# peterrum/dealii-multigrid

Measured on AMD Instinct MI355X. Metric: DoF/s per V-cycle, 3D octant p=4, higher is better.
Workload: dtype f64; 1 GPU; 3D octant (GeometryType quadrant) HMG-global p=4 FP64, NRefGlobal=8, SmootherDegree=3, coarse solver direct, f=1, zero Dirichlet (BASELINE.json configs[2]); n_dofs=137199985, n_cells=2127189, n_levels=9, parallelism=1 GPU, chebyshev_start_vector=deal.II's (i mod 11) - mean on the local numbering, fused_transfer_bricks=33509

## Files before the change

### dealii_multigrid_amd/__init__.py

```python
from __future__ import annotations

import ctypes as C
import os

import numpy as np

_LIB_PATH = os.environ.get("MGAMD_LIBRARY") or os.path.join(os.path.dirname(os.path.abspath(__file__)), "lib", "libmgamd.so")
F64, F32 = 8, 4
AMG_MIN_SHARDED_ROWS_DEFAULT = 20000
INVALID_DOF = 0xFFFFFFFF
ALL_DIRICHLET = 0x3F


class MgamdError(RuntimeError):
    pass


class NoDeviceError(MgamdError):
    pass


def _load():
    if not os.path.exists(_LIB_PATH):
        raise MgamdError(
# ... 350 lines not shown
    def cell_slots(self):
        grp, slot = np.zeros(self.info.n_cells, np.uint8), np.zeros(self.info.n_cells, np.uint32)
        _chk(_lib.mgamd_dofs_get_cell_slots(self._h, _ptr(grp), _ptr(slot)))
        return grp, slot

    def halo_plan(self):
        sz = (C.c_uint32 * 4)()
        _chk(_lib.mgamd_dofs_halo_sizes(self._h, sz))
        npeer, nsend, nsh, nc = (int(v) for v in sz)
        plan = dict(peers=np.zeros(npeer, np.int32), peer_offset=np.zeros(npeer + 1, np.uint32), pack_idx=np.zeros(nsend, np.uint32),
                    sh_tail=np.zeros(nsh, np.uint32), sh_ptr=np.zeros(nsh + 1, np.uint32), sh_src=np.zeros(nc, np.int32),
                    sh_owner_src=np.zeros(nsh, np.int32))
        if npeer:
            _chk(_lib.mgamd_dofs_halo_get(self._h, _ptr(plan["peers"]), _ptr(plan["peer_offset"]), _ptr(plan["pack_idx"]), _ptr(plan["sh_tail"]),
                                          _ptr(plan["sh_ptr"]), _ptr(plan["sh_src"]), _ptr(plan["sh_owner_src"])))
        return plan

    def __del__(self):
        if getattr(self, "_h", None) and _lib is not None:
            _lib.mgamd_dofs_destroy(self._h)
            self._h = None


def ls_copy_indices(active: DoFs, level_dofs: DoFs, level: int):
    n = C.c_uint64()
    _chk(_lib.mgamd_ls_copy_indices(active._h, level_dofs._h, level, C.byref(n), None, None))
    g, l = np.zeros(n.value, np.uint32), np.zeros(n.value, np.uint32)
    if n.value:
        _chk(_lib.mgamd_ls_copy_indices(active._h, level_dofs._h, level, C.byref(n), _ptr(g), _ptr(l)))
    return g, l


def transfer_tables(fine: DoFs, coarse: DoFs):
    npatch = (C.c_uint64 * 3)()
    nf = (C.c_uint32 * 3)()
    _chk(_lib.mgamd_transfer_tables_info(fine._h, coarse._h, npatch, nf))
    out = []
    nc3 = (coarse.degree + 1) ** 3
    for kind in range(3):
        n = npatch[kind]
        ci = np.zeros((n, nc3), np.uint32)
        cm = np.zeros(n, np.uint16)
        fi = np.zeros((n, nf[kind] ** 3), np.uint32)
        if n:
            _chk(_lib.mgamd_transfer_tables_get(fine._h, coarse._h, kind, _ptr(ci), _ptr(cm), _ptr(fi)))
        out.append((kind, int(nf[kind]), ci, cm, fi))
    return out


class Context:
    def __init__(self, device: int = 0):
        self._h = C.c_void_p()
        _chk(_lib.mgamd_ctx_create(device, C.byref(self._h)))

    def synchronize(self):
        _chk(_lib.mgamd_ctx_synchronize(self._h))

    def stream(self) -> int:
        s = C.c_void_p()
        _chk(_lib.mgamd_ctx_stream(self._h, C.byref(s)))
        return s.value

    def kernel_profile(self, enable: bool, brick_size: int = 0):
        _chk(_lib.mgamd_ctx_kernel_profile_brick(self._h, brick_size))
        _chk(_lib.mgamd_ctx_kernel_profile(self._h, 1 if enable else 0))

    def kernel_profile_read(self):
        ms, n, b = C.c_double(), C.c_uint64(), C.c_double()
        _chk(_lib.mgamd_ctx_kernel_profile_read(self._h, C.byref(ms), C.byref(n), C.byref(b)))
        return ms.value, n.value, b.value

    def kernel_profile_bytes_moved(self):
        b = C.c_double()
        _chk(_lib.mgamd_ctx_kernel_profile_bytes_moved(self._h, C.byref(b)))
        return b.value

    def __del__(self):
        if getattr(self, "_h", None) and _lib is not None:
            _lib.mgamd_ctx_destroy(self._h)
            self._h = None


class SimGroup:

    def __init__(self, n_ranks: int):
        self.n_ranks = n_ranks
        self._h = C.c_void_p()
        _chk(_lib.mgamd_sim_group_create(n_ranks, C.byref(self._h)))

    def comm(self, rank: int) -> "Communicator":
        h = C.c_void_p()
        _chk(_lib.mgamd_comm_sim_create(self._h, rank, C.byref(h)))
        return Communicator(h, self.n_ranks, rank, self)

    def __del__(self):
        if getattr(self, "_h", None) and _lib is not None:
            _lib.mgamd_sim_group_destroy(self._h)
            self._h = None


class Communicator:
    def __init__(self, handle, n_ranks, rank, keepalive=None):
        self._h, self.n_ranks, self.rank, self._keep = handle, n_ranks, rank, keepalive

    @staticmethod
    def rccl_unique_id() -> bytes:
        buf = C.create_string_buffer(128)
        _chk(_lib.mgamd_comm_rccl_unique_id(buf))
        return buf.raw

    @staticmethod
    def rccl(ctx: "Context", n_ranks: int, rank: int, unique_id: bytes) -> "Communicator":
        h = C.c_void_p()
        _chk(_lib.mgamd_comm_rccl_create(ctx._h, n_ranks, rank, C.c_char_p(unique_id), C.byref(h)))
        return Communicator(h, n_ranks, rank)

    def subset(self, group: int) -> "Communicator":
        if group == 1:
            return self
        h = C.c_void_p()
        _chk(_lib.mgamd_comm_subset(self._h, group, C.byref(h)))
        return Communicator(h, self.n_ranks // group, self.rank // group, self)

    def allreduce_sum(self, ctx: "Context", value: float) -> float:
        r = C.c_double()
        _chk(_lib.mgamd_comm_allreduce_sum(self._h, ctx._h, C.c_double(value), C.byref(r)))
        return r.value

    def __del__(self):
        if getattr(self, "_h", None) and _lib is not None:
            _lib.mgamd_comm_destroy(self._h)
            self._h = None


class Vector:

    def __init__(self, ctx: Context, n: int, number_type: int = F64, _handle=None):
        self.ctx = ctx
        self._h = C.c_void_p()
        if _handle is not None:
            self._h = _handle
        else:
            _chk(_lib.mgamd_vec_create(ctx._h, C.c_uint64(n), number_type, C.byref(self._h)))
        sz = C.c_uint64()
        _chk(_lib.mgamd_vec_size(self._h, C.byref(sz)))
        self.n = sz.value

    def from_host(self, a):
        a = np.ascontiguousarray(a, dtype=np.float64)
        assert a.size == self.n
        _chk(_lib.mgamd_vec_from_host(self._h, _ptr(a)))
        return self

    def to_host(self):
        a = np.zeros(self.n)
        _chk(_lib.mgamd_vec_to_host(self._h, _ptr(a)))
        return a

    def set(self, value: float):
        _chk(_lib.mgamd_vec_set(self._h, C.c_double(value)))

    def copy_from(self, other: "Vector"):
        _chk(_lib.mgamd_vec_copy(self._h, other._h))

    def sadd(self, s: float, a: float, x: "Vector"):
        _chk(_lib.mgamd_vec_sadd(self._h, C.c_double(s), C.c_double(a), x._h))

    def dot(self, other: "Vector") -> float:
        r = C.c_double()
        _chk(_lib.mgamd_vec_dot(self._h, other._h, C.byref(r)))
        return r.value

    def l2_norm(self) -> float:
        r = C.c_double()
        _chk(_lib.mgamd_vec_norm2(self._h, C.byref(r)))
        return r.value

    def __del__(self):
        if getattr(self, "_h", None) and _lib is not None:
            _lib.mgamd_vec_destroy(self._h)
            self._h = None


class Operator:

    def __init__(self, ctx: Context, dofs: DoFs, number_type: int = F64, comm: "Communicator" = None):
        self.ctx, self.dofs, self.number_type, self.comm = ctx, dofs, number_type, comm
        self._h = C.c_void_p()
        if comm is None:
            _chk(_lib.mgamd_level_op_create(ctx._h, dofs._h, number_type, C.byref(self._h)))
        else:
            _chk(_lib.mgamd_level_op_create_distributed(ctx._h, dofs._h, number_type, comm._h, C.byref(self._h)))

    def dot(self, x: "Vector", y: "Vector") -> float:
        r = C.c_double()
        _chk(_lib.mgamd_level_op_dot(self._h, x._h, y._h, C.byref(r)))
        return r.value

    def n_owned(self) -> int:
        n = C.c_uint64()
        _chk(_lib.mgamd_level_op_n_owned(self._h, C.byref(n)))
        return n.value

    def m(self) -> int:
        n = C.c_uint64()
        _chk(_lib.mgamd_level_op_m(self._h, C.byref(n)))
        return n.value

    def mass_coefficient(self) -> float:
        s = C.c_double()
        _chk(_lib.mgamd_level_op_mass_coefficient(self._h, C.byref(s)))
        return s.value

    def initialize_dof_vector(self) -> Vector:
        h = C.c_void_p()
        _chk(_lib.mgamd_level_op_init_vector(self._h, C.byref(h)))
        return Vector(self.ctx, 0, _handle=h)

    def vmult(self, dst: Vector, src: Vector):
        _chk(_lib.mgamd_level_op_vmult(self._h, dst._h, src._h))

    def vmult_mass(self, dst: Vector, src: Vector):
        _chk(_lib.mgamd_level_op_vmult_mass(self._h, dst._h, src._h))

    def vmult_interface_up(self, dst: Vector, src: Vector):
        _chk(_lib.mgamd_level_op_vmult_interface_up(self._h, dst._h, src._h))

    def exchange_add_tail(self, v: Vector):
        _chk(_lib.mgamd_level_op_exchange_add_tail(self._h, v._h))

    def vmult_interface_down(self, dst: Vector, src: Vector):
        _chk(_lib.mgamd_level_op_vmult_interface_down(self._h, dst._h, src._h))

    def compute_inverse_diagonal(self, diagonal: Vector):
        _chk(_lib.mgamd_level_op_inverse_diagonal(self._h, diagonal._h))

    def rhs(self, b: Vector, kind: int = 0):
        _chk(_lib.mgamd_level_op_rhs_kind(self._h, kind, b._h))

    def rhs_boundary_flux(self, b: Vector, q):
        q = _flux_array(q)
        _chk(_lib.mgamd_level_op_rhs_boundary_flux(self._h, _ptr(q), b._h))

    def distribute(self, x: Vector, kind: int = 0):
        _chk(_lib.mgamd_level_op_distribute(self._h, kind, x._h))

    def rhs_dirichlet(self, b: Vector, g: Vector, include_mass: bool = True):
        _chk(_lib.mgamd_level_op_rhs_dirichlet(self._h, g._h, 1 if include_mass else 0, b._h))

    def distribute_values(self, x: Vector, g: Vector):
        _chk(_lib.mgamd_level_op_distribute_values(self._h, x._h, g._h))

    def get_system_matrix(self) -> "SparseMatrix":
        if self.dofs.mass_coefficient() != self.mass_coefficient():
            raise MgamdError(f"get_system_matrix: the mass coefficient of the DoFs ({self.dofs.mass_coefficient()}) was changed after this "
                             f"operator was built with {self.mass_coefficient()}; the assembled matrix would be another operator's")
        return SparseMatrix(self.ctx, self.dofs)

    def __del__(self):
        if getattr(self, "_h", None) and _lib is not None:
            _lib.mgamd_level_op_destroy(self._h)
            self._h = None


class PreconditionChebyshev:
    def __init__(self, op: Operator, degree=3, smoothing_range=20.0, eig_cg_n_iterations=20):
        self.op = op
        self._h = C.c_void_p()
        _chk(_lib.mgamd_cheb_create(op._h, degree, C.c_double(smoothing_range), eig_cg_n_iterations, C.byref(self._h)))

    def vmult(self, dst: Vector, src: Vector):
        _chk(_lib.mgamd_cheb_vmult(self._h, dst._h, src._h))

    def step(self, dst: Vector, src: Vector):
        _chk(_lib.mgamd_cheb_step(self._h, dst._h, src._h))

    def eigenvalue_estimates(self):
        lo, hi = C.c_double(), C.c_double()
        _chk(_lib.mgamd_cheb_get_eigen_estimates(self._h, C.byref(lo), C.byref(hi)))
        return lo.value, hi.value

    def __del__(self):
        if getattr(self, "_h", None) and _lib is not None:
            _lib.mgamd_cheb_destroy(self._h)
            self._h = None


class MGTwoLevelTransfer:
    def __init__(self, fine: Operator, coarse: Operator):
        self.fine, self.coarse = fine, coarse
        self._h = C.c_void_p()
        _chk(_lib.mgamd_transfer2_create(fine._h, coarse._h, C.byref(self._h)))

    def prolongate_and_add(self, dst_fine: Vector, src_coarse: Vector):
        _chk(_lib.mgamd_transfer2_prolongate_and_add(self._h, dst_fine._h, src_coarse._h))

    def restrict_and_add(self, dst_coarse: Vector, src_fine: Vector):
        _chk(_lib.mgamd_transfer2_restrict_and_add(self._h, dst_coarse._h, src_fine._h))

    def n_fused_bricks(self):
        n = C.c_uint64()
        _chk(_lib.mgamd_transfer2_n_fused_bricks(self._h, C.byref(n)))
        return n.value

    def __del__(self):
        if getattr(self, "_h", None) and _lib is not None:
            _lib.mgamd_transfer2_destroy(self._h)
            self._h = None


STAGE_NAMES = ["pre_smoother_step", "residual_step", "restriction", "coarse_solve", "prolongation", "edge_prolongation",
               "post_smoother_step", "transfer_to_mg", "transfer_to_global"]
_STAGE_CB = C.CFUNCTYPE(None, C.c_int, C.c_int, C.c_uint, C.c_void_p)


class PreconditionMG:

    def __init__(self, ctx: Context, levels, transfers, smoothers, coarse_solver="direct", nested: "PreconditionMG" = None,
                 n_cycles: int = 1, local_smoothing: "DoFs" = None, sharded_amg: "DoFs" = None,
                 amg_min_sharded_rows: int = AMG_MIN_SHARDED_ROWS_DEFAULT):
        self.ctx, self.levels, self.transfers, self.smoothers, self.nested = ctx, levels, transfers, smoothers, nested
        self.sharded_amg = sharded_amg
        n = len(levels)
        L = (C.c_void_p * n)(*[l._h for l in levels])
        T = (C.c_void_p * n)(*[(t._h if t is not None else None) for t in transfers])
        S = (C.c_void_p * n)(*[(s._h if s is not None else None) for s in smoothers])
        self._h = C.c_void_p()
        if sharded_amg is not None:
            if local_smoothing is not None or nested is not None:
                raise MgamdError("sharded_amg excludes local smoothing and a nested multigrid")
            _chk(_lib.mgamd_mg_create_sharded_amg(ctx._h, n, L, T, S, coarse_solver.encode(), sharded_amg._h, n_cycles,
                                                  C.c_uint32(amg_min_sharded_rows), C.byref(self._h)))
        elif local_smoothing is not None:
            _chk(_lib.mgamd_mg_create_local_smoothing(ctx._h, n, L, T, S, local_smoothing._h, coarse_solver.encode(), C.byref(self._h)))
        else:
            _chk(_lib.mgamd_mg_create_nested(ctx._h, n, L, T, S, coarse_solver.encode(), nested._h if nested is not None else None, n_cycles,
                                             C.byref(self._h)))
        self._cb = None

    def set_collapse(self, enable: bool) -> int:
        l = C.c_uint()
        _chk(_lib.mgamd_mg_set_collapse(self._h, 1 if enable else 0, C.byref(l)))
        return l.value

    def coarse_solver_used(self) -> str:
        buf = C.create_string_buffer(32)
        _chk(_lib.mgamd_mg_coarse_solver_used(self._h, buf))
        return buf.value.decode()

    def coarse_iterations(self) -> int:
        n = C.c_uint64()
        _chk(_lib.mgamd_mg_coarse_iterations(self._h, C.byref(n)))
        return n.value

    def amg_layout(self):
        n, info = C.c_uint32(), (C.c_uint32 * (5 * 32))()
        _chk(_lib.mgamd_mg_amg_layout(self._h, C.byref(n), info, 32))
        return [dict(global_rows=info[5 * l], owned_rows=info[5 * l + 1], ghosts=info[5 * l + 2], peers=info[5 * l + 3],
                     replicated=bool(info[5 * l + 4])) for l in range(min(n.value, 32))]

    def vmult(self, z: Vector, r: Vector):
        _chk(_lib.mgamd_mg_vcycle(self._h, z._h, r._h))

    def connect_stages(self, fn):
        if fn is None:
            self._cb = None
            _chk(_lib.mgamd_mg_set_stage_callback(self._h, None, None))
            return
        self._cb = _STAGE_CB(lambda s, st, lv, u: fn(s, bool(st), lv))
        _chk(_lib.mgamd_mg_set_stage_callback(self._h, self._cb, None))

    def stage_timing(self, enable: bool):
        _chk(_lib.mgamd_mg_stage_timing(self._h, 1 if enable else 0))

    def stage_times(self):
        n = len(self.levels)
        ms = np.zeros((9, n))
        cnt = C.c_uint64()
        _chk(_lib.mgamd_mg_stage_times(self._h, _ptr(ms), n, C.byref(cnt)))
        return ms

    def time_vcycles(self, z: Vector, r: Vector, n: int, use_graph: bool = True) -> float:
        ms = C.c_double()
        _chk(_lib.mgamd_mg_time_vcycles(self._h, z._h, r._h, n, 1 if use_graph else 0, C.byref(ms)))
        return ms.value

    def __del__(self):
        if getattr(self, "_h", None) and _lib is not None:
            _lib.mgamd_mg_destroy(self._h)
            self._h = None


class SparseMatrix:

    def __init__(self, ctx: Context, dofs: DoFs):
        self.ctx, self.dofs = ctx, dofs
        self._h = C.c_void_p()
        _chk(_lib.mgamd_matrix_create(ctx._h, dofs._h, C.byref(self._h)))
        n, nnz, lanes = C.c_uint64(), C.c_uint64(), C.c_int()
        _chk(_lib.mgamd_matrix_info(self._h, C.byref(n), C.byref(nnz), C.byref(lanes)))
        self.n_rows, self.nnz, self.lanes = n.value, nnz.value, lanes.value

    def m(self) -> int:
        return self.n_rows

    def vmult(self, dst: Vector, src: Vector):
        _chk(_lib.mgamd_matrix_vmult(self._h, dst._h, src._h))

    def time_spmv(self, mode: int, lanes: int, reps: int = 50) -> float:
        ms = C.c_double()
        _chk(_lib.mgamd_debug_matrix_time_spmv(self._h, mode, lanes, reps, C.byref(ms)))
        return ms.value

    def __del__(self):
        if getattr(self, "_h", None) and _lib is not None:
            _lib.mgamd_matrix_destroy(self._h)
            self._h = None


class PreconditionAMG:

    def __init__(self, matrix: SparseMatrix, n_cycles: int = 1):
        self.matrix, self.n_cycles = matrix, n_cycles
        self._h = C.c_void_p()
        _chk(_lib.mgamd_amg_create(matrix._h, n_cycles, C.byref(self._h)))

    def vmult(self, z: Vector, r: Vector):
        _chk(_lib.mgamd_amg_vmult(self._h, z._h, r._h))

    def layout(self):
        n, rows = C.c_uint32(), (C.c_uint32 * 32)()
        _chk(_lib.mgamd_amg_layout(self._h, C.byref(n), rows, 32))
        return [rows[l] for l in range(min(n.value, 32))]

    def __del__(self):
        if getattr(self, "_h", None) and _lib is not None:
            _lib.mgamd_amg_destroy(self._h)
            self._h = None


def solve_cg(A, preconditioner, x: Vector, b: Vector, reltol=1e-4, abstol=1e-20, maxiter=10000):
    it, res = C.c_uint(), C.c_double()
    ph = preconditioner._h if preconditioner is not None else None
    if isinstance(A, SparseMatrix):
        if preconditioner is not None and not isinstance(preconditioner, PreconditionAMG):
            raise MgamdError("solve_cg: a SparseMatrix takes a PreconditionAMG (or None)")
        _chk(_lib.mgamd_solve_cg_matrix(A._h, ph, x._h, b._h, C.c_double(reltol), C.c_double(abstol), maxiter, C.byref(it), C.byref(res)))
        return it.value, res.value
    if isinstance(preconditioner, PreconditionAMG):
        raise MgamdError("solve_cg: a PreconditionAMG goes with the SparseMatrix it was built on")
    _chk(_lib.mgamd_solve_cg(A._h, ph, x._h, b._h, C.c_double(reltol), C.c_double(abstol), maxiter, C.byref(it), C.byref(res)))
    return it.value, res.value


class TimeStepper:

    def __init__(self, op: Operator, mg: "PreconditionMG", theta: float, dt: float):
        self.op, self.mg = op, mg
        self._h = C.c_void_p()
        _chk(_lib.mgamd_time_stepper_create(op._h, mg._h if mg is not None else None, C.c_double(theta), C.c_double(dt), C.byref(self._h)))

    @staticmethod
    def mass_coefficient(theta: float, dt: float) -> float:
        return 1.0 / (theta * dt)

    def step(self, u: Vector, f_old: Vector = None, f_new: Vector = None, reltol=1e-4, abstol=1e-20, maxiter=10000, g_old: Vector = None,
             g_new: Vector = None, load: Vector = None):
        it, res = C.c_uint(), C.c_double()
        h = lambda v: v._h if v is not None else None
        if g_old is None and g_new is None and load is None:
            _chk(_lib.mgamd_time_stepper_step(self._h, u._h, h(f_old), h(f_new), C.c_double(reltol), C.c_double(abstol), maxiter,
                                              C.byref(it), C.byref(res)))
        else:
            _chk(_lib.mgamd_time_stepper_step_data(self._h, u._h, h(f_old), h(f_new), h(g_old), h(g_new), h(load), C.c_double(reltol),
                                                   C.c_double(abstol), maxiter, C.byref(it), C.byref(res)))
        return it.value, res.value

    def time(self) -> float:
        t = C.c_double()
        _chk(_lib.mgamd_time_stepper_time(self._h, C.byref(t), None))
        return t.value

    def n_steps(self) -> int:
        n = C.c_uint64()
        _chk(_lib.mgamd_time_stepper_time(self._h, None, C.byref(n)))
        return n.value

    def __del__(self):
        if getattr(self, "_h", None) and _lib is not None:
            _lib.mgamd_time_stepper_destroy(self._h)
            self._h = None


class AmgHostHierarchy:

    def __init__(self, dofs: DoFs):
        self._h = C.c_void_p()
        _chk(_lib.mgamd_debug_amg_host_create(dofs._h, C.byref(self._h)))
        n = C.c_uint32()
        _chk(_lib.mgamd_debug_amg_host_n_levels(self._h, C.byref(n)))
        self.n_levels = n.value

    def level(self, l: int):
        rows, nnz_a, cols_p, nnz_p, na, lam = C.c_uint32(), C.c_uint64(), C.c_uint32(), C.c_uint64(), C.c_uint32(), C.c_double()
        _chk(_lib.mgamd_debug_amg_host_level_info(self._h, C.c_uint32(l), C.byref(rows), C.byref(nnz_a), C.byref(cols_p), C.byref(nnz_p),
                                                 C.byref(na), C.byref(lam)))
        n, coarsest = rows.value, l + 1 == self.n_levels
        A = (np.zeros(n + 1, np.uint32), np.zeros(nnz_a.value, np.uint32), np.zeros(nnz_a.value))
        P = (np.zeros(n + 1, np.uint32), np.zeros(nnz_p.value, np.uint32), np.zeros(nnz_p.value))
        agg = np.zeros(n, np.int32)
        _chk(_lib.mgamd_debug_amg_host_level_get(self._h, C.c_uint32(l), *[_ptr(a) for a in A], *([None] * 3 if coarsest else [_ptr(a) for a in P]),
                                                None if coarsest else _ptr(agg)))
        return dict(A=A, P=None if coarsest else P, n_cols_P=cols_p.value, agg=None if coarsest else agg, n_aggregates=na.value,
                    lambda_max=lam.value)

    def __del__(self):
        if getattr(self, "_h", None) and _lib is not None:
            _lib.mgamd_debug_amg_host_destroy(self._h)
            self._h = None


class AmgShardPlans:

    def __init__(self, partition: "Partition", level: int, degree: int, max_brick: int = -1,
                 min_sharded_rows: int = AMG_MIN_SHARDED_ROWS_DEFAULT):
        self._h = C.c_void_p()
        _chk(_lib.mgamd_debug_amg_shard_create(partition._h, level, degree, max_brick, C.c_uint32(min_sharded_rows), C.byref(self._h)))
        n, ns = C.c_uint32(), C.c_uint32()
        _chk(_lib.mgamd_debug_amg_shard_n_levels(self._h, C.byref(n), C.byref(ns)))
        self.n_levels, self.n_sharded_levels, self.n_ranks = n.value, ns.value, partition.n_ranks

    def level(self, rank: int, l: int):
        info = (C.c_uint32 * 12)()
        _chk(_lib.mgamd_debug_amg_shard_level_info(self._h, rank, C.c_uint32(l), info))
        rep, ng, nr, nm, ni, ngh, nrecv, npeer, nza, nzp, nzr, rrows = (int(v) for v in info)
        out = dict(replicated=bool(rep), n_global=ng, n_rows=nr, n_mirror=nm, n_interior=ni, n_ghost=ngh, n_recv=nrecv, A=None, P=None, R=None)
        if rep:
            return out
        u32 = lambda n: np.zeros(n, np.uint32)
        out.update(rows=u32(nr), ghost=u32(nrecv), peers=np.zeros(npeer, np.int32), peer_offset=u32(npeer + 1), send_count=u32(npeer),
                   recv_count=u32(npeer), send_idx=u32(nrecv), A=(u32(nr + 1), u32(nza), np.zeros(nza)), P=(u32(nr + 1), u32(nzp), np.zeros(nzp)),
                   R=(u32(rrows + 1), u32(nzr), np.zeros(nzr)))
        _chk(_lib.mgamd_debug_amg_shard_level_get(self._h, rank, C.c_uint32(l), *[_ptr(out[k]) for k in ("rows", "ghost", "peers", "peer_offset",
                                                                                                      "send_count", "recv_count", "send_idx")],
                                                 *[_ptr(a) for a in out["A"]], *[_ptr(a) for a in out["P"]], *[_ptr(a) for a in out["R"]]))
        return out

    def __del__(self):
        if getattr(self, "_h", None) and _lib is not None:
            _lib.mgamd_debug_amg_shard_destroy(self._h)
            self._h = None


SPMV_PLAIN, SPMV_ADD, SPMV_RESID, SPMV_CHEB, SPMV_DOT = 0, 1, 2, 3, 4


def debug_csr_spmv(ctx: "Context", number_type, mode, lanes, ptr, col, val, x, y, b=None, xold=None, xold_is_y=False, dinv=None, f1=0.0,
                   f2=0.0):
    ptr, col = np.ascontiguousarray(ptr, np.uint32), np.ascontiguousarray(col, np.uint32)
    val, x, y = (np.ascontiguousarray(a, np.float64) for a in (val, x, y))
    y = y.copy()
    opt = [None if a is None else np.ascontiguousarray(a, np.float64) for a in (b, xold, dinv)]
    n_rows = len(ptr) - 1
    assert len(y) == n_rows and len(col) == len(val) == ptr[-1]
    used = C.c_int()
    _chk(_lib.mgamd_debug_csr_spmv(ctx._h, number_type, mode, lanes, C.c_uint32(n_rows), C.c_uint32(len(x)), _ptr(ptr), _ptr(col), _ptr(val),
                                   _ptr(x), _ptr(y), *[None if a is None else _ptr(a) for a in opt[:2]], 1 if xold_is_y else 0,
                                   None if opt[2] is None else _ptr(opt[2]), C.c_double(f1), C.c_double(f2), C.byref(used)))
    return y, used.value


def debug_csr_spmv_ex(ctx: "Context", mode, lanes, ptr, col, val, x, y, b=None, xold=None, xold_is_y=False, dinv=None, f1=0.0, f2=0.0,
                      max_blocks=0, number_type=F64):
    ptr, col = np.ascontiguousarray(ptr, np.uint32), np.ascontiguousarray(col, np.uint32)
    val, x, y = (np.ascontiguousarray(a, np.float64) for a in (val, x, y))
    y = y.copy()
    opt = [None if a is None else np.ascontiguousarray(a, np.float64) for a in (b, xold, dinv)]
    n_rows = len(ptr) - 1
    assert len(y) == n_rows and len(col) == len(val) == ptr[-1]
    used, blocks, dot = C.c_int(), C.c_int(), C.c_double()
    _chk(_lib.mgamd_debug_csr_spmv_ex(ctx._h, number_type, mode, lanes, C.c_uint32(n_rows), C.c_uint32(len(x)), _ptr(ptr), _ptr(col),
                                      _ptr(val), _ptr(x), _ptr(y), *[None if a is None else _ptr(a) for a in opt[:2]],
                                      1 if xold_is_y else 0, None if opt[2] is None else _ptr(opt[2]), C.c_double(f1), C.c_double(f2),
                                      max_blocks, C.byref(used), C.byref(blocks), C.byref(dot)))
    return y, used.value, blocks.value, dot.value


def csr_spmv_lanes_long(n_rows: int, nnz: int) -> int:
    lanes = C.c_int()
    _chk(_lib.mgamd_debug_csr_spmv_lanes_long(C.c_uint32(n_rows), C.c_uint64(nnz), C.byref(lanes)))
    return lanes.value


def amg_shard_match_rows(global_dofs: "DoFs", local_dofs: "DoFs"):
    rows = np.zeros(local_dofs.n_dofs, np.uint32)
    _chk(_lib.mgamd_debug_amg_shard_match_rows(global_dofs._h, local_dofs._h, _ptr(rows)))
    return rows


def csr_row_pointers(row_counts):
    counts = np.ascontiguousarray(row_counts, np.uint64)
    ptr = np.zeros(len(counts) + 1, np.uint32)
    _chk(_lib.mgamd_debug_csr_row_pointers(C.c_uint32(len(counts)), _ptr(counts), _ptr(ptr)))
    return ptr


# ... 187 lines not shown
```

### dealii_multigrid_amd/csrc/c_api_device.hip

```cpp
#include "runtime.hpp"
#include "kernels_amg.hpp"
#include <cstdio>

using namespace mgamd;

#define REQUIRE(cond)                                    \
  if (!(cond))                                           \
  throw std::invalid_argument("null or invalid argument: " #cond)

extern "C" {

int
mgamd_ctx_create(int device, mgamd_ctx **out)
{
  MGAMD_TRY
  REQUIRE(out);
  auto *c = new mgamd_ctx;
  try
    {
      c->ctx = std::make_unique<Ctx>(device);
    }
  catch (...)
    {
      delete c;
// ... 238 lines not shown
}

int
mgamd_sim_group_create(unsigned n_ranks, mgamd_sim_group **out)
{
  MGAMD_TRY
  REQUIRE(out && n_ranks > 0);
  auto *g  = new mgamd_sim_group;
  g->group = std::make_shared<SimGroup>((int)n_ranks);
  *out     = g;
  MGAMD_CATCH
}

int
mgamd_sim_group_destroy(mgamd_sim_group *g)
{
  delete g;
  return MGAMD_OK;
}

int
mgamd_comm_sim_create(mgamd_sim_group *g, unsigned rank, mgamd_comm **out)
{
  MGAMD_TRY
  REQUIRE(g && out && (int)rank < g->group->n);
  auto *c = new mgamd_comm;
  c->comm = std::make_shared<SimComm>(g->group, (int)rank);
  *out    = c;
  MGAMD_CATCH
}

int
mgamd_comm_subset(mgamd_comm *base, unsigned group, mgamd_comm **out)
{
  MGAMD_TRY
  if (!base || !base->comm || !out || group == 0)
    throw std::invalid_argument("bad argument");
  auto *c = new mgamd_comm;
  try
    {
      c->comm = std::make_shared<SubsetComm>(base->comm, (int)group);
    }
  catch (...)
    {
      delete c;
      throw;
    }
  *out = c;
  MGAMD_CATCH
}

int
mgamd_comm_destroy(mgamd_comm *c)
{
  delete c;
  return MGAMD_OK;
}

int
mgamd_comm_allreduce_sum(mgamd_comm *c, mgamd_ctx *ctx, double value, double *result)
{
  MGAMD_TRY
  REQUIRE(c && ctx && result);
  *result = c->comm->allreduce_sum_host(value, ctx->ctx->stream);
  MGAMD_CATCH
}

int
mgamd_level_op_destroy(mgamd_level_op *op)
{
  delete op;
  return MGAMD_OK;
}

int
mgamd_level_op_m(const mgamd_level_op *op, uint64_t *n)
{
  MGAMD_TRY
  REQUIRE(op && n);
  *n = op->op->n_dofs();
  MGAMD_CATCH
}

int
mgamd_level_op_mass_coefficient(const mgamd_level_op *op, double *sigma)
{
  MGAMD_TRY
  REQUIRE(op && sigma);
  *sigma = op->op->sigma;
  MGAMD_CATCH
}

int
mgamd_level_op_init_vector(const mgamd_level_op *op, mgamd_vec **out)
{
  MGAMD_TRY
  REQUIRE(op && out);
  *out = vec_create(op->op->ctx, op->op->n_dofs(), op->op->type);
  MGAMD_CATCH
}

int
mgamd_level_op_vmult(mgamd_level_op *op, mgamd_vec *dst, const mgamd_vec *src)
{
  MGAMD_TRY
  REQUIRE(op && dst && src);
  op->op->vmult(*dst, *src);
  MGAMD_CATCH
}

int
mgamd_level_op_vmult_mass(mgamd_level_op *op, mgamd_vec *dst, const mgamd_vec *src)
{
  MGAMD_TRY
  REQUIRE(op && dst && src);
  op->op->vmult_mass(*dst, *src);
  MGAMD_CATCH
}

int
mgamd_level_op_inverse_diagonal(mgamd_level_op *op, mgamd_vec *diagonal)
{
  MGAMD_TRY
  REQUIRE(op && diagonal);
  if (diagonal->type != op->op->type)
    throw std::invalid_argument("vector number type does not match the operator's");
  op->op->compute_inverse_diagonal(*diagonal);
  MGAMD_CATCH
}

int
mgamd_level_op_rhs(mgamd_level_op *op, mgamd_vec *rhs)
{
  MGAMD_TRY
  REQUIRE(op && rhs);
  op->op->rhs(*rhs);
  MGAMD_CATCH
}

int
mgamd_level_op_rhs_kind(mgamd_level_op *op, int kind, mgamd_vec *rhs)
{
  MGAMD_TRY
  REQUIRE(op && rhs);
  if (kind != 0 && kind != 1)
    throw std::invalid_argument("SimulationType kind must be 0 (Constant) or 1 (Gaussian)");
  op->op->rhs(*rhs, kind);
  MGAMD_CATCH
}

int
mgamd_level_op_rhs_boundary_flux(mgamd_level_op *op, const double q[6], mgamd_vec *rhs)
{
  MGAMD_TRY
  REQUIRE(op && q && rhs);
  op->op->rhs_boundary_flux(*rhs, q);
  MGAMD_CATCH
}

int
mgamd_level_op_distribute(mgamd_level_op *op, int kind, mgamd_vec *x)
{
  MGAMD_TRY
  REQUIRE(op && x);
  if (kind != 0 && kind != 1)
    throw std::invalid_argument("SimulationType kind must be 0 (Constant) or 1 (Gaussian)");
  op->op->distribute(*x, kind);
  MGAMD_CATCH
}

int
mgamd_level_op_rhs_dirichlet(mgamd_level_op *op, const mgamd_vec *g, int include_mass, mgamd_vec *rhs)
{
  MGAMD_TRY
  REQUIRE(op && g && rhs);
  op->op->rhs_dirichlet(*rhs, *g, include_mass != 0);
  MGAMD_CATCH
}

int
mgamd_level_op_distribute_values(mgamd_level_op *op, mgamd_vec *x, const mgamd_vec *g)
{
  MGAMD_TRY
  REQUIRE(op && x && g);
  op->op->distribute_values(*x, *g);
  MGAMD_CATCH
}

int
mgamd_level_op_debug_stamps(mgamd_level_op *op, unsigned long long *out, uint64_t max_count, uint64_t *count)
{
  MGAMD_TRY
  REQUIRE(op && out && count);
  *count = op->op->read_debug_stamps(out, max_count);
  MGAMD_CATCH
}

int
mgamd_cheb_create(mgamd_level_op *op, unsigned degree, double smoothing_range, unsigned eig_cg_n_iterations, mgamd_cheb **out)
{
  MGAMD_TRY
  REQUIRE(op && out);
  auto *h = new mgamd_cheb;
  try
    {
      h->c.reset(make_chebyshev(op->op.get(), degree, smoothing_range, eig_cg_n_iterations));
    }
  catch (...)
    {
      delete h;
      throw;
    }
  *out = h;
  MGAMD_CATCH
}

int
mgamd_cheb_destroy(mgamd_cheb *c)
{
  delete c;
  return MGAMD_OK;
}

int
mgamd_cheb_vmult(mgamd_cheb *c, mgamd_vec *dst, const mgamd_vec *src)
{
  MGAMD_TRY
  REQUIRE(c && dst && src);
  c->c->vmult(*dst, *src);
  MGAMD_CATCH
}

int
mgamd_cheb_step(mgamd_cheb *c, mgamd_vec *dst, const mgamd_vec *src)
{
  MGAMD_TRY
  REQUIRE(c && dst && src);
  c->c->step(*dst, *src);
  MGAMD_CATCH
}

int
mgamd_cheb_get_eigen_estimates(const mgamd_cheb *c, double *min_eigenvalue, double *max_eigenvalue)
{
  MGAMD_TRY
  REQUIRE(c);
  if (min_eigenvalue)
    *min_eigenvalue = c->c->min_eig;
  if (max_eigenvalue)
    *max_eigenvalue = c->c->max_eig;
  MGAMD_CATCH
}

int
mgamd_transfer2_create(mgamd_level_op *fine, mgamd_level_op *coarse, mgamd_transfer2 **out)
{
  MGAMD_TRY
  REQUIRE(fine && coarse && out);
  auto *h = new mgamd_transfer2;
  try
    {
      h->t.reset(make_transfer2(fine->op.get(), coarse->op.get()));
    }
  catch (...)
    {
      delete h;
      throw;
    }
  *out = h;
  MGAMD_CATCH
}

int
mgamd_transfer2_destroy(mgamd_transfer2 *t)
{
  delete t;
  return MGAMD_OK;
}

int
mgamd_transfer2_prolongate_and_add(mgamd_transfer2 *t, mgamd_vec *dst_fine, const mgamd_vec *src_coarse)
{
  MGAMD_TRY
  REQUIRE(t && dst_fine && src_coarse);
  t->t->prolongate_and_add(*dst_fine, *src_coarse);
  MGAMD_CATCH
}

int
mgamd_transfer2_restrict_and_add(mgamd_transfer2 *t, mgamd_vec *dst_coarse, const mgamd_vec *src_fine)
{
  MGAMD_TRY
  REQUIRE(t && dst_coarse && src_fine);
  t->t->restrict_and_add(*dst_coarse, *src_fine);
  MGAMD_CATCH
}

int
mgamd_transfer2_n_fused_bricks(const mgamd_transfer2 *t, uint64_t *n)
{
  MGAMD_TRY
  REQUIRE(t && n);
  *n = t->t->n_fused_bricks_total();
  MGAMD_CATCH
}

int
mgamd_mg_create(mgamd_ctx *ctx, unsigned n_levels, mgamd_level_op *const *levels, mgamd_transfer2 *const *transfers,
                mgamd_cheb *const *smoothers, const char *coarse_solver, mgamd_mg **out)
{
  MGAMD_TRY
  REQUIRE(ctx && levels && out && n_levels > 0 && (n_levels == 1 || (transfers && smoothers)));
  std::vector<LevelOperatorBase *> L(n_levels, nullptr);
  std::vector<Transfer2Base *>     Tr(n_levels, nullptr);
  std::vector<ChebyshevBase *>     Sm(n_levels, nullptr);
  for (unsigned l = 0; l < n_levels; ++l)
    {
      REQUIRE(levels[l]);
      L[l] = levels[l]->op.get();
      if (transfers && transfers[l])
        Tr[l] = transfers[l]->t.get();
      if (smoothers && smoothers[l])
        Sm[l] = smoothers[l]->c.get();
    }
  auto *h = new mgamd_mg;
  try
    {
      h->mg.reset(make_multigrid(ctx->ctx.get(), n_levels, L.data(), Tr.data(), Sm.data(), coarse_solver ? coarse_solver : "direct"));
    }
  catch (...)
    {
      delete h;
      throw;
    }
  *out = h;
  MGAMD_CATCH
}

int
mgamd_mg_create_nested(mgamd_ctx *ctx, unsigned n_levels, mgamd_level_op *const *levels, mgamd_transfer2 *const *transfers,
                       mgamd_cheb *const *smoothers, const char *coarse_solver, mgamd_mg *coarse_mg, unsigned n_cycles, mgamd_mg **out)
{
  MGAMD_TRY
  REQUIRE(ctx && levels && out && n_levels > 0 && (n_levels == 1 || (transfers && smoothers)));
  std::vector<LevelOperatorBase *> L(n_levels, nullptr);
  std::vector<Transfer2Base *>     Tr(n_levels, nullptr);
  std::vector<ChebyshevBase *>     Sm(n_levels, nullptr);
  for (unsigned l = 0; l < n_levels; ++l)
    {
      REQUIRE(levels[l]);
      L[l] = levels[l]->op.get();
      if (transfers && transfers[l])
        Tr[l] = transfers[l]->t.get();
      if (smoothers && smoothers[l])
        Sm[l] = smoothers[l]->c.get();
    }
  auto *h = new mgamd_mg;
  try
    {
      h->mg.reset(make_multigrid(ctx->ctx.get(), n_levels, L.data(), Tr.data(), Sm.data(), coarse_solver ? coarse_solver : "amg",
                                 coarse_mg ? coarse_mg->mg.get() : nullptr, n_cycles));
    }
  catch (...)
    {
      delete h;
      throw;
    }
  *out = h;
  MGAMD_CATCH
}

int
mgamd_mg_create_sharded_amg(mgamd_ctx *ctx, unsigned n_levels, mgamd_level_op *const *levels, mgamd_transfer2 *const *transfers,
                            mgamd_cheb *const *smoothers, const char *coarse_solver, const mgamd_dofs *global_coarse_dofs, unsigned n_cycles,
                            uint32_t min_sharded_rows, mgamd_mg **out)
{
  MGAMD_TRY
  REQUIRE(ctx && levels && out && global_coarse_dofs && n_levels > 0 && (n_levels == 1 || (transfers && smoothers)));
  if (global_coarse_dofs->halo)
    throw std::invalid_argument("mgamd_mg_create_sharded_amg: global_coarse_dofs must be the GLOBAL level (mgamd_dofs_create)");
  std::vector<LevelOperatorBase *> L(n_levels, nullptr);
  std::vector<Transfer2Base *>     Tr(n_levels, nullptr);
  std::vector<ChebyshevBase *>     Sm(n_levels, nullptr);
  for (unsigned l = 0; l < n_levels; ++l)
    {
      REQUIRE(levels[l]);
      L[l] = levels[l]->op.get();
      if (transfers && transfers[l])
        Tr[l] = transfers[l]->t.get();
      if (smoothers && smoothers[l])
        Sm[l] = smoothers[l]->c.get();
    }
  auto *h = new mgamd_mg;
  try
    {
      h->mg.reset(make_multigrid(ctx->ctx.get(), n_levels, L.data(), Tr.data(), Sm.data(), coarse_solver ? coarse_solver : "amg", nullptr,
                                 n_cycles, global_coarse_dofs->tables.get(), min_sharded_rows));
    }
  catch (...)
    {
      delete h;
      throw;
    }
  *out = h;
  MGAMD_CATCH
}

int
mgamd_mg_coarse_iterations(const mgamd_mg *mg, uint64_t *n_iterations)
{
  MGAMD_TRY
  REQUIRE(mg && n_iterations);
  *n_iterations = mg->mg->coarse_cg_iterations();
  MGAMD_CATCH
}

int
mgamd_mg_amg_layout(const mgamd_mg *mg, uint32_t *n_levels, uint32_t *info, uint32_t max_levels)
{
  MGAMD_TRY
  REQUIRE(mg && n_levels);
  std::vector<uint32_t> v;
  mg->mg->amg_layout(v);
  *n_levels = (uint32_t)(v.size() / 5);
  if (info)
    std::copy(v.begin(), v.begin() + 5 * std::min<size_t>(v.size() / 5, max_levels), info);
  MGAMD_CATCH
}

int
mgamd_mg_create_local_smoothing(mgamd_ctx *ctx, unsigned n_levels, mgamd_level_op *const *levels, mgamd_transfer2 *const *transfers,
                                mgamd_cheb *const *smoothers, const mgamd_dofs *active_mesh_dofs, const char *coarse_solver, mgamd_mg **out)
{
  MGAMD_TRY
  REQUIRE(ctx && levels && out && active_mesh_dofs && n_levels > 0 && (n_levels == 1 || (transfers && smoothers)));
  std::vector<LevelOperatorBase *> L(n_levels, nullptr);
  std::vector<Transfer2Base *>     Tr(n_levels, nullptr);
  std::vector<ChebyshevBase *>     Sm(n_levels, nullptr);
  for (unsigned l = 0; l < n_levels; ++l)
    {
      REQUIRE(levels[l]);
      L[l] = levels[l]->op.get();
      if (transfers && transfers[l])
        Tr[l] = transfers[l]->t.get();
      if (smoothers && smoothers[l])
        Sm[l] = smoothers[l]->c.get();
    }
  auto *h = new mgamd_mg;
  try
    {
      h->mg.reset(make_multigrid(ctx->ctx.get(), n_levels, L.data(), Tr.data(), Sm.data(), coarse_solver ? coarse_solver : "amg"));
      h->mg->setup_local_smoothing(*active_mesh_dofs->tables);
    }
  catch (...)
    {
      delete h;
      throw;
    }
  *out = h;
  MGAMD_CATCH
}

int
mgamd_level_op_exchange_add_tail(mgamd_level_op *op, mgamd_vec *v)
{
  MGAMD_TRY
  REQUIRE(op && v);
  op->op->exchange_add_tail(*v);
  MGAMD_CATCH
}

int
mgamd_level_op_vmult_interface_up(mgamd_level_op *op, mgamd_vec *dst, const mgamd_vec *src)
{
  MGAMD_TRY
  REQUIRE(op && dst && src);
  op->op->vmult_interface_up(*dst, *src);
  MGAMD_CATCH
}

int
mgamd_level_op_vmult_interface_down(mgamd_level_op *op, mgamd_vec *dst, const mgamd_vec *src)
{
  MGAMD_TRY
  REQUIRE(op && dst && src);
  op->op->vmult_interface_down(*dst, *src);
  MGAMD_CATCH
}

int
mgamd_mg_set_collapse(mgamd_mg *mg, int enable, unsigned *collapse_level)
{
  MGAMD_TRY
  REQUIRE(mg);
  const unsigned l = mg->mg->set_collapse(enable != 0);
  if (collapse_level)
    *collapse_level = l;
  MGAMD_CATCH
}

int
mgamd_mg_coarse_solver_used(const mgamd_mg *mg, char name[32])
{
  MGAMD_TRY
  REQUIRE(mg && name);
  std::snprintf(name, 32, "%s", mg->mg->coarse_used.c_str());
  MGAMD_CATCH
}

int
mgamd_mg_destroy(mgamd_mg *mg)
{
  delete mg;
  return MGAMD_OK;
}

int
mgamd_mg_vcycle(mgamd_mg *mg, mgamd_vec *z, const mgamd_vec *r)
{
  MGAMD_TRY
  REQUIRE(mg && z && r);
  mg->mg->vcycle(*z, *r);
  MGAMD_CATCH
}

int
mgamd_mg_set_stage_callback(mgamd_mg *mg, mgamd_stage_callback cb, void *user)
{
  MGAMD_TRY
  REQUIRE(mg);
  mg->mg->cb      = cb;
  mg->mg->cb_user = user;
  MGAMD_CATCH
}

int
mgamd_mg_stage_timing(mgamd_mg *mg, int enable)
{
  MGAMD_TRY
  if (!mg)
    throw std::invalid_argument("null argument");
  mg->mg->set_stage_timing(enable != 0);
  MGAMD_CATCH
}

int
mgamd_mg_stage_times(mgamd_mg *mg, double *ms, unsigned n_levels, uint64_t *n_records)
{
  MGAMD_TRY
  if (!mg || !ms)
    throw std::invalid_argument("null argument");
  if (n_levels != mg->mg->n_levels())
    throw std::invalid_argument("stage_times: ms must hold 9 x n_levels entries");
  const size_t n = mg->mg->read_stage_times(ms);
  if (n_records)
    *n_records = n;
  MGAMD_CATCH
}

int
mgamd_mg_time_vcycles(mgamd_mg *mg, mgamd_vec *z, const mgamd_vec *r, unsigned n, int use_graph, double *ms_per_cycle)
{
  MGAMD_TRY
  REQUIRE(mg && z && r && ms_per_cycle);
  *ms_per_cycle = mg->mg->time_vcycles(*z, *r, n, use_graph != 0);
  MGAMD_CATCH
}

int
mgamd_solve_cg(mgamd_level_op *A, mgamd_mg *preconditioner, mgamd_vec *x, const mgamd_vec *b, double reltol, double abstol,
               unsigned maxiter, unsigned *n_iterations, double *residual_norm)
{
  MGAMD_TRY
  REQUIRE(A && x && b);
  unsigned it  = 0;
  double   res = 0;
  solve_cg(*A->op, preconditioner ? preconditioner->mg.get() : nullptr, *x, *b, reltol, abstol, maxiter, it, res);
  if (n_iterations)
    *n_iterations = it;
  if (residual_norm)
    *residual_norm = res;
  MGAMD_CATCH
}

int
mgamd_time_stepper_create(mgamd_level_op *A, mgamd_mg *preconditioner, double theta, double dt, mgamd_time_stepper **out)
{
  MGAMD_TRY
  REQUIRE(A && out);
  auto ts = std::make_unique<mgamd_time_stepper>();
  ts->ts.reset(make_theta_stepper(*A->op, preconditioner ? preconditioner->mg.get() : nullptr, theta, dt));
  *out = ts.release();
  MGAMD_CATCH
}

int
mgamd_time_stepper_step(mgamd_time_stepper *ts, mgamd_vec *u, const mgamd_vec *f_old, const mgamd_vec *f_new, double reltol, double abstol,
                        unsigned maxiter, unsigned *n_iterations, double *residual_norm)
{
  MGAMD_TRY
  REQUIRE(ts && u);
  unsigned it  = 0;
  double   res = 0;
  ts->ts->step(*u, f_old, f_new, reltol, abstol, maxiter, it, res);
  if (n_iterations)
    *n_iterations = it;
// ... 322 lines not shown
```

### dealii_multigrid_amd/csrc/kernels_transfer.hpp

```cpp
#pragma once
#include "kernels_common.hpp"

namespace mgamd
{
  template <int PC, int NF>
  struct TransferGeo
  {
    static constexpr int NC    = PC + 1;
    static constexpr int NC3   = NC * NC * NC;
    static constexpr int NF3   = NF * NF * NF;
    static constexpr int LINES = NF * NF;
    static constexpr int SPW   = LINES >= 256 ? 1 : 256 / LINES;
    static constexpr int BLOCK = ((SPW * LINES + 63) / 64) * 64;
  };

  template <typename T, int PC, int NF>
  struct TransferArgs
  {
    const uint32_t *coarse_idx;
    const uint16_t *coarse_mask;
    const uint32_t *fine_idx;
    uint32_t        n_patches;
    Mats<PC, T>     m;
    T               E[NF * (PC + 1)];
    const T        *src;
    T              *dst;
  };
  static_assert(sizeof(TransferArgs<double, MAX_KERNEL_DEGREE, 2 * MAX_KERNEL_DEGREE + 1>) <= KERNARG_LIMIT,
                "TransferArgs exceeds the kernel-argument segment");

  template <typename T, int PC, int NF>
  __device__ __forceinline__ void
  fine_rmw(const TransferArgs<T, PC, NF> &args, const T *__restrict__ buf, int p0, int np, int tid)
  {
    using G           = TransferGeo<PC, NF>;
    constexpr int ITF = (G::SPW * G::NF3 + G::BLOCK - 1) / G::BLOCK;
    uint32_t      gi[ITF];
    T             val[ITF];
#pragma unroll
    for (int it = 0; it < ITF; ++it)
      {
        const int idx = tid + it * G::BLOCK;
        gi[it]        = idx < np * G::NF3 ? args.fine_idx[(size_t)p0 * G::NF3 + idx] : DEV_INVALID;
      }
#pragma unroll
    for (int it = 0; it < ITF; ++it)
      val[it] = args.dst[gi[it] != DEV_INVALID ? gi[it] : 0];
#pragma unroll
    for (int it = 0; it < ITF; ++it)
      if (gi[it] != DEV_INVALID)
        args.dst[gi[it]] = val[it] + buf[tid + it * G::BLOCK];
  }

  template <typename T, int PC, int NF, bool IDENTITY>
  __global__ void
  __launch_bounds__((TransferGeo<PC, NF>::BLOCK)) prolongate_kernel(const TransferArgs<T, PC, NF> args)
  {
    using G = TransferGeo<PC, NF>;
    extern __shared__ __align__(16) unsigned char smem_raw[];
    T *bufA = reinterpret_cast<T *>(smem_raw);
    T *bufB = bufA + G::SPW * G::NF3;

    const int tid    = threadIdx.x;
    const int p0     = blockIdx.x * G::SPW;
    const int np     = min((int)G::SPW, (int)args.n_patches - p0);
    const int sl     = tid / G::LINES;
    const int ln     = tid % G::LINES;
    const int u = ln % NF, v = ln / NF;
    const bool act = tid < G::SPW * G::LINES && sl < np;

    {
      constexpr int ITC = (G::SPW * G::NC3 + G::BLOCK - 1) / G::BLOCK;
      uint32_t      gi[ITC];
      T             val[ITC];
#pragma unroll
      for (int it = 0; it < ITC; ++it)
        {
          const int idx = tid + it * G::BLOCK;
          gi[it]        = idx < np * G::NC3 ? args.coarse_idx[(size_t)p0 * G::NC3 + idx] : DEV_INVALID;
        }
#pragma unroll
      for (int it = 0; it < ITC; ++it)
        val[it] = args.src[gi[it] != DEV_INVALID ? gi[it] : 0];
#pragma unroll
      for (int it = 0; it < ITC; ++it)
        {
          const int idx = tid + it * G::BLOCK;
          if (idx < np * G::NC3)
            bufB[(idx / G::NC3) * G::NF3 + idx % G::NC3] = gi[it] != DEV_INVALID ? val[it] : T(0);
        }
    }
    __syncthreads();
    uint32_t mask = 0;
    if (act)
      mask = args.coarse_mask[p0 + sl];
    const bool any_hanging = __syncthreads_or((int)(mask >> 3)) != 0;
    if (any_hanging)
      {
        T        *view = bufB + sl * (G::NF3 - G::NC3);
        const bool la  = act && u < G::NC && v < G::NC;
        hanging_passes<T, PC>(view, args.m, sl, u, v, la, la ? mask : 0u, false);
      }
    if (IDENTITY)
      {
        fine_rmw<T, PC, NF>(args, bufB, p0, np, tid);
        return;
      }
    if (act && u < G::NC && v < G::NC)
      {
        T in[G::NC];
#pragma unroll
        for (int b = 0; b < G::NC; ++b)
          in[b] = bufB[sl * G::NF3 + (v * G::NC + u) * G::NC + b];
#pragma unroll
        for (int a = 0; a < NF; ++a)
          {
            T s = T(0);
#pragma unroll
            for (int b = 0; b < G::NC; ++b)
              s += T(args.E[a * G::NC + b]) * in[b];
            bufA[sl * G::NF3 + (v * G::NC + u) * NF + a] = s;
          }
      }
    __syncthreads();
    if (act && v < G::NC)
      {
        T in[G::NC];
#pragma unroll
        for (int b = 0; b < G::NC; ++b)
          in[b] = bufA[sl * G::NF3 + (v * G::NC + b) * NF + u];
#pragma unroll
        for (int a = 0; a < NF; ++a)
          {
            T s = T(0);
#pragma unroll
            for (int b = 0; b < G::NC; ++b)
              s += T(args.E[a * G::NC + b]) * in[b];
            bufB[sl * G::NF3 + (v * NF + a) * NF + u] = s;
          }
      }
    __syncthreads();
    if (act)
      {
        T in[G::NC];
#pragma unroll
        for (int b = 0; b < G::NC; ++b)
          in[b] = bufB[sl * G::NF3 + (b * NF + v) * NF + u];
#pragma unroll
        for (int a = 0; a < NF; ++a)
          {
            T s = T(0);
#pragma unroll
            for (int b = 0; b < G::NC; ++b)
              s += T(args.E[a * G::NC + b]) * in[b];
            bufA[sl * G::NF3 + (a * NF + v) * NF + u] = s;
          }
      }
    __syncthreads();
    fine_rmw<T, PC, NF>(args, bufA, p0, np, tid);
  }

  template <typename T, int PC, int NF, bool IDENTITY>
  __global__ void
  __launch_bounds__((TransferGeo<PC, NF>::BLOCK)) restrict_kernel(const TransferArgs<T, PC, NF> args)
  {
    using G = TransferGeo<PC, NF>;
    extern __shared__ __align__(16) unsigned char smem_raw[];
    T *bufA = reinterpret_cast<T *>(smem_raw);
    T *bufB = bufA + G::SPW * G::NF3;

    const int tid    = threadIdx.x;
    const int p0     = blockIdx.x * G::SPW;
    const int np     = min((int)G::SPW, (int)args.n_patches - p0);
    const int sl     = tid / G::LINES;
    const int ln     = tid % G::LINES;
    const int u = ln % NF, v = ln / NF;
    const bool act = tid < G::SPW * G::LINES && sl < np;

    {
      constexpr int ITF = (G::SPW * G::NF3 + G::BLOCK - 1) / G::BLOCK;
      uint32_t      gi[ITF];
      T             val[ITF];
#pragma unroll
      for (int it = 0; it < ITF; ++it)
        {
          const int idx = tid + it * G::BLOCK;
          gi[it]        = idx < np * G::NF3 ? args.fine_idx[(size_t)p0 * G::NF3 + idx] : DEV_INVALID;
        }
#pragma unroll
      for (int it = 0; it < ITF; ++it)
        val[it] = args.src[gi[it] != DEV_INVALID ? gi[it] : 0];
#pragma unroll
      for (int it = 0; it < ITF; ++it)
        {
          const int idx = tid + it * G::BLOCK;
          if (idx < G::SPW * G::NF3)
            bufA[idx] = gi[it] != DEV_INVALID ? val[it] : T(0);
        }
    }
    __syncthreads();
    if (!IDENTITY)
      {
        if (act)
          {
            T in[NF];
#pragma unroll
            for (int a = 0; a < NF; ++a)
              in[a] = bufA[sl * G::NF3 + (a * NF + v) * NF + u];
#pragma unroll
            for (int b = 0; b < G::NC; ++b)
              {
                T s = T(0);
#pragma unroll
                for (int a = 0; a < NF; ++a)
                  s += T(args.E[a * G::NC + b]) * in[a];
                bufB[sl * G::NF3 + (b * NF + v) * NF + u] = s;
              }
          }
        __syncthreads();
        if (act && v < G::NC)
          {
            T in[NF];
#pragma unroll
            for (int a = 0; a < NF; ++a)
              in[a] = bufB[sl * G::NF3 + (v * NF + a) * NF + u];
#pragma unroll
            for (int b = 0; b < G::NC; ++b)
              {
                T s = T(0);
#pragma unroll
                for (int a = 0; a < NF; ++a)
                  s += T(args.E[a * G::NC + b]) * in[a];
                bufA[sl * G::NF3 + (v * G::NC + b) * NF + u] = s;
              }
          }
        __syncthreads();
        if (act && u < G::NC && v < G::NC)
          {
            T in[NF];
#pragma unroll
            for (int a = 0; a < NF; ++a)
              in[a] = bufA[sl * G::NF3 + (v * G::NC + u) * NF + a];
#pragma unroll
            for (int b = 0; b < G::NC; ++b)
              {
                T s = T(0);
#pragma unroll
                for (int a = 0; a < NF; ++a)
                  s += T(args.E[a * G::NC + b]) * in[a];
                bufB[sl * G::NF3 + (v * G::NC + u) * G::NC + b] = s;
              }
          }
        __syncthreads();
      }
    T *res = IDENTITY ? bufA : bufB;
    uint32_t mask = 0;
    if (act)
      mask = args.coarse_mask[p0 + sl];
    const bool any_hanging = __syncthreads_or((int)(mask >> 3)) != 0;
    if (any_hanging)
      {
        T         *view = res + sl * (G::NF3 - G::NC3);
        const bool la   = act && u < G::NC && v < G::NC;
        hanging_passes<T, PC>(view, args.m, sl, u, v, la, la ? mask : 0u, true);
      }
    {
      constexpr int ITC = (G::SPW * G::NC3 + G::BLOCK - 1) / G::BLOCK;
      uint32_t      gi[ITC];
#pragma unroll
      for (int it = 0; it < ITC; ++it)
        {
          const int idx = tid + it * G::BLOCK;
          gi[it]        = idx < np * G::NC3 ? args.coarse_idx[(size_t)p0 * G::NC3 + idx] : DEV_INVALID;
        }
#pragma unroll
      for (int it = 0; it < ITC; ++it)
        if (gi[it] != DEV_INVALID)
          {
            const int idx = tid + it * G::BLOCK;
            atomic_add(&args.dst[gi[it]], res[(idx / G::NC3) * G::NF3 + idx % G::NC3]);
          }
    }
  }

  template <typename T>
  struct PatchP1Args
  {
    const uint32_t *uniq_ptr;
    const uint32_t *uniq_idx;
    const uint16_t *loc;
    const uint16_t *coarse_mask;
    const uint32_t *fine_idx_t;
    uint32_t        n_patches, max_uniq;
    Mats<1, T>      m;
    const T        *src;
    T              *dst;
  };
  static_assert(sizeof(PatchP1Args<double>) <= KERNARG_LIMIT, "PatchP1Args exceeds the kernel-argument segment");
  constexpr int PATCH_P1_BLOCK = 256;
  constexpr int PATCH_P1_ITERS = 8;

  template <typename T>
  __global__ void
  __launch_bounds__(PATCH_P1_BLOCK) patch_p1_prolongate_kernel(const PatchP1Args<T> a)
  {
    extern __shared__ __align__(16) unsigned char smem_raw[];
    T             *U    = reinterpret_cast<T *>(smem_raw);
    const int      tid  = threadIdx.x;
    const uint32_t wg   = blockIdx.x;
    const uint32_t pch  = wg * PATCH_P1_BLOCK + tid;
    const bool     act  = pch < a.n_patches;
    const uint32_t p0   = a.uniq_ptr[wg];
    const int      nu   = (int)(a.uniq_ptr[wg + 1] - p0);
    const uint4    lw   = reinterpret_cast<const uint4 *>(a.loc)[act ? pch : 0];
    const uint32_t mask = act ? a.coarse_mask[pch] : 0u;
    uint32_t       fi[27];
#pragma unroll
    for (int t = 0; t < 27; ++t)
      fi[t] = act ? a.fine_idx_t[(size_t)t * a.n_patches + pch] : DEV_INVALID;
    T gv[PATCH_P1_ITERS];
#pragma unroll
    for (int k = 0; k < PATCH_P1_ITERS; ++k)
      {
        const int j = tid + k * PATCH_P1_BLOCK;
        gv[k]       = nu > 0 ? a.src[a.uniq_idx[p0 + (j < nu ? j : nu - 1)]] : T(0);
      }
#pragma unroll
    for (int k = 0; k < PATCH_P1_ITERS; ++k)
      {
        const int j = tid + k * PATCH_P1_BLOCK;
        if (j < nu)
          U[j] = gv[k];
      }
    __syncthreads();
    const uint32_t lw4[4] = {lw.x, lw.y, lw.z, lw.w};
    T              c[8];
#pragma unroll
    for (int i = 0; i < 8; ++i)
      {
        const uint32_t l = (lw4[i / 2] >> (16 * (i % 2))) & 0xFFFFu;
        c[i]             = (act && l != 0xFFFFu) ? U[l] : T(0);
      }
    if (mask >> 3)
      hanging_in_registers_p1<T, false>(c, mask, a.m);
    T gx[12], gy[18];
#pragma unroll
    for (int q = 0; q < 4; ++q)
      {
        gx[3 * q + 0] = c[2 * q];
        gx[3 * q + 1] = T(0.5) * (c[2 * q] + c[2 * q + 1]);
        gx[3 * q + 2] = c[2 * q + 1];
      }
#pragma unroll
    for (int z = 0; z < 2; ++z)
#pragma unroll
      for (int X = 0; X < 3; ++X)
        {
          const T y0 = gx[X + 3 * (0 + 2 * z)], y1 = gx[X + 3 * (1 + 2 * z)];
          gy[X + 3 * (0 + 3 * z)] = y0;
          gy[X + 3 * (1 + 3 * z)] = T(0.5) * (y0 + y1);
          gy[X + 3 * (2 + 3 * z)] = y1;
        }
    T oldv[27];
#pragma unroll
    for (int t = 0; t < 27; ++t)
      oldv[t] = a.dst[fi[t] != DEV_INVALID ? fi[t] : 0];
#pragma unroll
    for (int XY = 0; XY < 9; ++XY)
      {
        const T z0 = gy[XY], z1 = gy[XY + 9];
        const T f[3] = {z0, T(0.5) * (z0 + z1), z1};
#pragma unroll
        for (int Z = 0; Z < 3; ++Z)
          if (fi[XY + 9 * Z] != DEV_INVALID)
            a.dst[fi[XY + 9 * Z]] = oldv[XY + 9 * Z] + f[Z];
      }
  }

  template <typename T>
  __global__ void
  __launch_bounds__(PATCH_P1_BLOCK) patch_p1_restrict_kernel(const PatchP1Args<T> a)
  {
    extern __shared__ __align__(16) unsigned char smem_raw[];
    T             *Acc  = reinterpret_cast<T *>(smem_raw);
    const int      tid  = threadIdx.x;
    const uint32_t wg   = blockIdx.x;
    const uint32_t pch  = wg * PATCH_P1_BLOCK + tid;
    const bool     act  = pch < a.n_patches;
    const uint32_t p0   = a.uniq_ptr[wg];
    const int      nu   = (int)(a.uniq_ptr[wg + 1] - p0);
    const uint4    lw   = reinterpret_cast<const uint4 *>(a.loc)[act ? pch : 0];
    const uint32_t mask = act ? a.coarse_mask[pch] : 0u;
    uint32_t       fi[27];
#pragma unroll
    for (int t = 0; t < 27; ++t)
      fi[t] = act ? a.fine_idx_t[(size_t)t * a.n_patches + pch] : DEV_INVALID;
    T r[27];
#pragma unroll
    for (int t = 0; t < 27; ++t)
      r[t] = a.src[fi[t] != DEV_INVALID ? fi[t] : 0];
#pragma unroll
    for (int t = 0; t < 27; ++t)
      if (fi[t] == DEV_INVALID)
        r[t] = T(0);
    for (int j = tid; j < nu; j += PATCH_P1_BLOCK)
      Acc[j] = T(0);
    T gy[18], gx[12], c[8];
#pragma unroll
    for (int XY = 0; XY < 9; ++XY)
      {
        gy[XY]     = r[XY] + T(0.5) * r[XY + 9];
        gy[XY + 9] = T(0.5) * r[XY + 9] + r[XY + 18];
      }
#pragma unroll
    for (int z = 0; z < 2; ++z)
#pragma unroll
      for (int X = 0; X < 3; ++X)
        {
          const T y0 = gy[X + 3 * (0 + 3 * z)], y1 = gy[X + 3 * (1 + 3 * z)], y2 = gy[X + 3 * (2 + 3 * z)];
          gx[X + 3 * (0 + 2 * z)] = y0 + T(0.5) * y1;
          gx[X + 3 * (1 + 2 * z)] = T(0.5) * y1 + y2;
        }
#pragma unroll
    for (int q = 0; q < 4; ++q)
      {
        c[2 * q]     = gx[3 * q] + T(0.5) * gx[3 * q + 1];
        c[2 * q + 1] = T(0.5) * gx[3 * q + 1] + gx[3 * q + 2];
      }
    if (mask >> 3)
      hanging_in_registers_p1<T, true>(c, mask, a.m);
    __syncthreads();
    const uint32_t lw4[4] = {lw.x, lw.y, lw.z, lw.w};
    if (act)
      {
#pragma unroll
        for (int i = 0; i < 8; ++i)
          {
            const uint32_t l = (lw4[i / 2] >> (16 * (i % 2))) & 0xFFFFu;
            if (l != 0xFFFFu)
              atomic_add(&Acc[l], c[i]);
          }
      }
    __syncthreads();
    for (int j = tid; j < nu; j += PATCH_P1_BLOCK)
      atomic_add(&a.dst[a.uniq_idx[p0 + j]], Acc[j]);
  }

  template <int P, int B>
  struct BrickTransferGeo
  {
    static constexpr int NF    = P * B + 1;
    static constexpr int BC    = B / 2;
    static constexpr int NC    = P * BC + 1;
    static constexpr int NF3   = NF * NF * NF;
    static constexpr int NC3   = NC * NC * NC;
    static constexpr int BLOCK = 256;
    static constexpr int LDS = NF3;
  };

  template <typename T, int P>
  struct BrickTransferArgs
  {
    const uint32_t *slot;
    const uint32_t *interior_base;
    const uint16_t *shell_pos;
    const uint32_t *coarse_idx;
    const uint32_t *own_shell;
    uint32_t        n_bricks;
    T               E[(2 * P + 1) * (P + 1)];
    const T        *src;
    T              *dst;
  };
  static_assert(sizeof(BrickTransferArgs<double, MAX_KERNEL_DEGREE>) <= KERNARG_LIMIT, "BrickTransferArgs exceeds the kernel-argument segment");

  template <typename T, int P, int B>
  __global__ void
  __launch_bounds__(256, 4) brick_prolongate_kernel(const BrickTransferArgs<T, P> args)
  {
    using G  = BrickTransferGeo<P, B>;
    using LG = Geo<P, B>;
    extern __shared__ __align__(16) unsigned char smem_raw[];
    T *buf = reinterpret_cast<T *>(smem_raw);
    constexpr int NC = G::NC, NF = G::NF, BLOCK = G::BLOCK;
    const int      tid   = threadIdx.x;
    const uint32_t brick = xcd_contiguous(blockIdx.x, gridDim.x);
    const uint32_t slot  = args.slot[brick];

    constexpr int  NI_P  = LG::NI > 0 ? LG::NI : 1;
    constexpr int  NIN_P = LG::N_INT > 0 ? LG::N_INT : 1;
    constexpr int  ITI_P = (NIN_P + BLOCK - 1) / BLOCK;
    constexpr int  ITS_P = (LG::N_SHELL + BLOCK - 1) / BLOCK;
    const uint32_t ibase = LG::N_INT > 0 ? args.interior_base[slot] : 0u;
    T              ival[ITI_P];
    uint32_t       sgi_p[ITS_P];
    T              sval_p[ITS_P];
    if (LG::N_INT > 0)
      {
#pragma unroll
        for (int it = 0; it < ITI_P; ++it)
          {
            const int i = tid + it * BLOCK;
            ival[it]    = NT_LOAD(&args.dst[ibase + (i < NIN_P ? i : 0)]);
          }
      }
#pragma unroll
    for (int it = 0; it < ITS_P; ++it)
      {
        const int s = tid + it * BLOCK;
        sgi_p[it]   = s < LG::N_SHELL ? NT_LOAD(&args.own_shell[(size_t)brick * LG::N_SHELL + s]) : DEV_INVALID;
      }
#pragma unroll
    for (int it = 0; it < ITS_P; ++it)
      sval_p[it] = args.dst[sgi_p[it] != DEV_INVALID ? sgi_p[it] : 0];

    {
      constexpr int ITC = (G::NC3 + BLOCK - 1) / BLOCK;
      uint32_t      gi[ITC];
      T             val[ITC];
#pragma unroll
      for (int it = 0; it < ITC; ++it)
        {
          const int idx = tid + it * BLOCK;
          gi[it]        = idx < G::NC3 ? NT_LOAD(&args.coarse_idx[(size_t)brick * G::NC3 + idx]) : DEV_INVALID;
        }
#pragma unroll
      for (int it = 0; it < ITC; ++it)
        val[it] = args.src[gi[it] != DEV_INVALID ? gi[it] : 0];
#pragma unroll
      for (int it = 0; it < ITC; ++it)
        {
          const int idx = tid + it * BLOCK;
          if (idx < G::NC3)
            {
              const int x = idx % NC, y = (idx / NC) % NC, z = idx / (NC * NC);
              buf[(z * NF + y) * NF + x] = gi[it] != DEV_INVALID ? val[it] : T(0);
            }
        }
    }
    __syncthreads();
    T in[NC], out[NF];
    for (int l = tid; l < NC * NC; l += BLOCK)
      {
        const int base = (l / NC) * NF + l % NC;
#pragma unroll
        for (int i = 0; i < NC; ++i)
          in[i] = buf[base + i * NF * NF];
        line_embed<T, P, G::BC>(args.E, in, out);
#pragma unroll
        for (int i = 0; i < NF; ++i)
          buf[base + i * NF * NF] = out[i];
      }
    __syncthreads();
    for (int l = tid; l < NC * NF; l += BLOCK)
      {
        const int base = (l / NC) * NF * NF + l % NC;
#pragma unroll
        for (int i = 0; i < NC; ++i)
          in[i] = buf[base + i * NF];
        line_embed<T, P, G::BC>(args.E, in, out);
#pragma unroll
        for (int i = 0; i < NF; ++i)
          buf[base + i * NF] = out[i];
      }
    __syncthreads();
    for (int l = tid; l < NF * NF; l += BLOCK)
      {
        const int base = l * NF;
#pragma unroll
        for (int i = 0; i < NC; ++i)
          in[i] = buf[base + i];
        line_embed<T, P, G::BC>(args.E, in, out);
#pragma unroll
        for (int i = 0; i < NF; ++i)
          buf[base + i] = out[i];
      }
    __syncthreads();
    if (LG::N_INT > 0)
      {
#pragma unroll
        for (int it = 0; it < ITI_P; ++it)
          {
            const int i = tid + it * BLOCK;
            if (i < NIN_P)
              {
                const int x = i % NI_P, y = (i / NI_P) % NI_P, z = i / (NI_P * NI_P);
                NT_STORE(ival[it] + buf[((z + 1) * NF + (y + 1)) * NF + x + 1], &args.dst[ibase + i]);
              }
          }
      }
#pragma unroll
    for (int it = 0; it < ITS_P; ++it)
      if (sgi_p[it] != DEV_INVALID)
        args.dst[sgi_p[it]] = sval_p[it] + buf[args.shell_pos[tid + it * BLOCK]];
  }

  template <typename T, int P, int B>
  __global__ void
  __launch_bounds__(256) brick_restrict_kernel(const BrickTransferArgs<T, P> args)
  {
    using G  = BrickTransferGeo<P, B>;
    using LG = Geo<P, B>;
    extern __shared__ __align__(16) unsigned char smem_raw[];
    T *buf = reinterpret_cast<T *>(smem_raw);
    constexpr int NC = G::NC, NF = G::NF, BLOCK = G::BLOCK;
    const int      tid   = threadIdx.x;
    const uint32_t brick = xcd_contiguous(blockIdx.x, gridDim.x);
    const uint32_t slot  = args.slot[brick];

    if (LG::N_INT > 0)
      {
        constexpr int  NI_  = LG::NI > 0 ? LG::NI : 1;
        constexpr int  NIN_ = LG::N_INT > 0 ? LG::N_INT : 1;
        constexpr int  ITI  = (NIN_ + BLOCK - 1) / BLOCK;
        const uint32_t base = args.interior_base[slot];
        T              val[ITI];
#pragma unroll
        for (int it = 0; it < ITI; ++it)
          {
            const int i = tid + it * BLOCK;
            val[it]     = NT_LOAD(&args.src[base + (i < NIN_ ? i : 0)]);
          }
#pragma unroll
        for (int it = 0; it < ITI; ++it)
          {
            const int i = tid + it * BLOCK;
            if (i < NIN_)
              {
                const int x = i % NI_, y = (i / NI_) % NI_, z = i / (NI_ * NI_);
                buf[((z + 1) * NF + (y + 1)) * NF + x + 1] = val[it];
              }
          }
      }
    {
      constexpr int ITS = (LG::N_SHELL + BLOCK - 1) / BLOCK;
      uint32_t      gi[ITS];
      T             val[ITS];
#pragma unroll
      for (int it = 0; it < ITS; ++it)
        {
          const int s = tid + it * BLOCK;
          gi[it]      = s < LG::N_SHELL ? NT_LOAD(&args.own_shell[(size_t)brick * LG::N_SHELL + s]) : DEV_INVALID;
        }
#pragma unroll
      for (int it = 0; it < ITS; ++it)
        val[it] = args.src[gi[it] != DEV_INVALID ? gi[it] : 0];
#pragma unroll
      for (int it = 0; it < ITS; ++it)
        if (tid + it * BLOCK < LG::N_SHELL)
          buf[args.shell_pos[tid + it * BLOCK]] = gi[it] != DEV_INVALID ? val[it] : T(0);
    }
    constexpr int ITC_R = (G::NC3 + BLOCK - 1) / BLOCK;
    uint32_t      cgi[ITC_R];
    T             cold[ITC_R];
    bool          cinner[ITC_R];
#pragma unroll
    for (int it = 0; it < ITC_R; ++it)
      {
        const int idx = tid + it * BLOCK;
        cgi[it]       = idx < G::NC3 ? NT_LOAD(&args.coarse_idx[(size_t)brick * G::NC3 + idx]) : DEV_INVALID;
        const int x = idx % NC, y = (idx / NC) % NC, z = idx / (NC * NC);
        cinner[it] = x > 0 && y > 0 && z > 0 && x < NC - 1 && y < NC - 1 && z < NC - 1;
      }
#pragma unroll
    for (int it = 0; it < ITC_R; ++it)
      cold[it] = args.dst[(cgi[it] != DEV_INVALID && cinner[it]) ? cgi[it] : 0];
    __syncthreads();
    T in[NF], out[NC];
    for (int l = tid; l < NF * NF; l += BLOCK)
      {
        const int base = l * NF;
#pragma unroll
        for (int i = 0; i < NF; ++i)
          in[i] = buf[base + i];
        line_embed_T<T, P, G::BC>(args.E, in, out);
#pragma unroll
        for (int i = 0; i < NC; ++i)
          buf[base + i] = out[i];
      }
    __syncthreads();
    for (int l = tid; l < NC * NF; l += BLOCK)
      {
        const int base = (l / NC) * NF * NF + l % NC;
#pragma unroll
        for (int i = 0; i < NF; ++i)
          in[i] = buf[base + i * NF];
        line_embed_T<T, P, G::BC>(args.E, in, out);
#pragma unroll
        for (int i = 0; i < NC; ++i)
          buf[base + i * NF] = out[i];
      }
    __syncthreads();
    for (int l = tid; l < NC * NC; l += BLOCK)
      {
        const int base = (l / NC) * NF + l % NC;
#pragma unroll
        for (int i = 0; i < NF; ++i)
          in[i] = buf[base + i * NF * NF];
        line_embed_T<T, P, G::BC>(args.E, in, out);
#pragma unroll
        for (int i = 0; i < NC; ++i)
          buf[base + i * NF * NF] = out[i];
      }
    __syncthreads();
#pragma unroll
    for (int it = 0; it < ITC_R; ++it)
      if (cgi[it] != DEV_INVALID)
        {
          const int idx = tid + it * BLOCK;
          const int x = idx % NC, y = (idx / NC) % NC, z = idx / (NC * NC);
          const T   v = buf[(z * NF + y) * NF + x];
          if (cinner[it])
            args.dst[cgi[it]] = cold[it] + v;
          else
            atomic_add(&args.dst[cgi[it]], v);
        }
  }

  template <typename T, int P, int B>
  __global__ void
  __launch_bounds__(256, 3) brick_restrict_persistent_kernel(const BrickTransferArgs<T, P> args)
  {
    using G  = BrickTransferGeo<P, B>;
    using LG = Geo<P, B>;
    static_assert(LG::N_INT > 0, "bricks with interior nodes");
    extern __shared__ __align__(16) unsigned char smem_raw[];
    T *buf = reinterpret_cast<T *>(smem_raw);
    constexpr int NC = G::NC, NF = G::NF, BLOCK = G::BLOCK;
    constexpr int NI = LG::NI, NIN = LG::N_INT;
    constexpr int ITI = (NIN + BLOCK - 1) / BLOCK, ITS = (LG::N_SHELL + BLOCK - 1) / BLOCK, ITC = (G::NC3 + BLOCK - 1) / BLOCK;
    const int      tid = threadIdx.x;
    const uint32_t n = args.n_bricks, w = blockIdx.x, stride = gridDim.x;
    if (w >= n)
      return;
    int  spos[ITS], cpos[ITC];
    bool cinner[ITC];
#pragma unroll
    for (int it = 0; it < ITS; ++it)
      spos[it] = tid + it * BLOCK < LG::N_SHELL ? (int)args.shell_pos[tid + it * BLOCK] : -1;
#pragma unroll
    for (int it = 0; it < ITC; ++it)
      {
        const int idx = tid + it * BLOCK;
        const int x = idx % NC, y = (idx / NC) % NC, z = idx / (NC * NC);
        cinner[it] = x > 0 && y > 0 && z > 0 && x < NC - 1 && y < NC - 1 && z < NC - 1;
        cpos[it]   = idx < G::NC3 ? (z * NF + y) * NF + x : -1;
      }
    auto load_tables = [&](uint32_t v, uint32_t &base, uint32_t(&gi)[ITS], uint32_t(&cgi)[ITC]) {
      const uint32_t brick = xcd_contiguous(v, n);
      base                 = args.interior_base[args.slot[brick]];
#pragma unroll
      for (int it = 0; it < ITS; ++it)
        gi[it] = spos[it] >= 0 ? NT_LOAD(&args.own_shell[(size_t)brick * LG::N_SHELL + tid + it * BLOCK]) : DEV_INVALID;
#pragma unroll
      for (int it = 0; it < ITC; ++it)
        cgi[it] = cpos[it] >= 0 ? NT_LOAD(&args.coarse_idx[(size_t)brick * G::NC3 + tid + it * BLOCK]) : DEV_INVALID;
    };
    auto load_values = [&](uint32_t base, const uint32_t(&gi)[ITS], const uint32_t(&cgi)[ITC], T(&val)[ITI], T(&sval)[ITS], T(&cold)[ITC]) {
#pragma unroll
      for (int it = 0; it < ITI; ++it)
        val[it] = NT_LOAD(&args.src[base + (uint32_t)(tid + it * BLOCK < NIN ? tid + it * BLOCK : 0)]);
#pragma unroll
      for (int it = 0; it < ITS; ++it)
        sval[it] = args.src[gi[it] != DEV_INVALID ? gi[it] : 0];
#pragma unroll
      for (int it = 0; it < ITC; ++it)
        cold[it] = args.dst[(cgi[it] != DEV_INVALID && cinner[it]) ? cgi[it] : 0];
    };
    uint32_t base, gi[ITS], cgi[ITC];
    T        val[ITI], sval[ITS], cold[ITC];
    load_tables(w, base, gi, cgi);
    load_values(base, gi, cgi, val, sval, cold);
    for (uint32_t v = w;;)
      {
        const uint32_t vn       = v + stride;
        const bool     has_next = vn < n;
        {
          int x = tid % NI + 1, y = (tid / NI) % NI + 1, z = tid / (NI * NI) + 1;
#pragma unroll
          for (int it = 0; it < ITI; ++it)
            {
              if ((it + 1) * BLOCK <= NIN || tid + it * BLOCK < NIN)
                buf[(z * NF + y) * NF + x] = val[it];
              constexpr int DZ = BLOCK / (NI * NI), DY = (BLOCK % (NI * NI)) / NI, DX = BLOCK % NI;
              x += DX;
              if (x > NI)
                {
                  x -= NI;
                  ++y;
                }
              y += DY;
              if (y > NI)
                {
                  y -= NI;
                  ++z;
                }
              z += DZ;
            }
        }
#pragma unroll
        for (int it = 0; it < ITS; ++it)
          if (spos[it] >= 0)
            buf[spos[it]] = gi[it] != DEV_INVALID ? sval[it] : T(0);
        uint32_t basen = base, gin[ITS], cgn[ITC];
        if (has_next)
          load_tables(vn, basen, gin, cgn);
        __syncthreads();
        T in[NF], out[NC];
        for (int l = tid; l < NF * NF; l += BLOCK)
          {
            const int b0 = l * NF;
#pragma unroll
            for (int i = 0; i < NF; ++i)
              in[i] = buf[b0 + i];
            line_embed_T<T, P, G::BC>(args.E, in, out);
#pragma unroll
            for (int i = 0; i < NC; ++i)
              buf[b0 + i] = out[i];
          }
        __syncthreads();
        for (int l = tid; l < NC * NF; l += BLOCK)
          {
            const int b0 = (l / NC) * NF * NF + l % NC;
#pragma unroll
            for (int i = 0; i < NF; ++i)
              in[i] = buf[b0 + i * NF];
            line_embed_T<T, P, G::BC>(args.E, in, out);
#pragma unroll
            for (int i = 0; i < NC; ++i)
              buf[b0 + i * NF] = out[i];
          }
        __syncthreads();
        for (int l = tid; l < NC * NC; l += BLOCK)
          {
            const int b0 = (l / NC) * NF + l % NC;
#pragma unroll
            for (int i = 0; i < NF; ++i)
              in[i] = buf[b0 + i * NF * NF];
            line_embed_T<T, P, G::BC>(args.E, in, out);
#pragma unroll
            for (int i = 0; i < NC; ++i)
              buf[b0 + i * NF * NF] = out[i];
          }
        __syncthreads();
        T valn[ITI], svaln[ITS], coldn[ITC];
        if (has_next)
          load_values(basen, gin, cgn, valn, svaln, coldn);
#pragma unroll
        for (int it = 0; it < ITC; ++it)
          if (cgi[it] != DEV_INVALID)
            {
              const T r = buf[cpos[it]];
              if (cinner[it])
                args.dst[cgi[it]] = cold[it] + r;
              else
                atomic_add(&args.dst[cgi[it]], r);
            }
        if (!has_next)
          break;
        v    = vn;
        base = basen;
#pragma unroll
        for (int it = 0; it < ITS; ++it)
          {
            gi[it]   = gin[it];
            sval[it] = svaln[it];
          }
#pragma unroll
        for (int it = 0; it < ITC; ++it)
          {
            cgi[it]  = cgn[it];
            cold[it] = coldn[it];
          }
#pragma unroll
        for (int it = 0; it < ITI; ++it)
          val[it] = valn[it];
        __syncthreads();
      }
  }

}
```

### dealii_multigrid_amd/csrc/runtime.hip

```cpp
#include "runtime.hpp"
#include "level_operator.hpp"
#include "amg.hpp"
#include "amg_shard.hpp"

#include <chrono>
#include <cmath>
#include <mutex>
#include <set>
#include <unordered_map>
#include <cstring>
#include <type_traits>

namespace mgamd
{
  Ctx::Ctx(int dev)
    : device(dev)
  {
    int        count = 0;
    hipError_t e     = hipGetDeviceCount(&count);
    if (e != hipSuccess || count == 0)
      throw NoDeviceError("no HIP device available: this library has no CPU fallback");
    if (dev < 0 || dev >= count)
      throw std::invalid_argument("device index out of range");
    HIP_CHECK(hipSetDevice(dev));
// ... 425 lines not shown
              hipLaunchKernelGGL(vec_sadd_kernel<T>, g, 256, 0, ctx->stream, d.p, T(beta), T(1), z.p, n);
            }
        }
      if (!alphas.empty())
        {
          betas.resize(alphas.size(), 0.0);
          max_eig = lanczos_max_eigenvalue(alphas, betas, &min_eig);
        }
      else
        min_eig = max_eig = 1.0;
      max_eig *= 1.2;
      const double a = smoothing_range > 1.0 ? max_eig / smoothing_range : std::min(0.9 * max_eig, min_eig);
      delta          = 0.5 * (max_eig - a);
      theta          = 0.5 * (max_eig + a);
      ctx->sync();
    }

    void
    vmult_raw(T *S, T *Tb, const T *b)
    {
      Ctx         *ctx = lop->ctx;
      const size_t n   = lop->n_dofs();
      T           *cur = (degree % 2 == 1) ? S : Tb;
      T           *oth = (cur == S) ? Tb : S;
      const bool passes = degree >= 2 && std::fabs(delta) >= 1e-40;
      if (!passes)
        hipLaunchKernelGGL(vec_scaled_product_kernel<T>, grid_for(n), 256, 0, ctx->stream, cur, T(1.0 / theta), dinv.p, b, n);
      if (passes)
        {
          double rhok = delta / theta, sigma = theta / delta;
          for (unsigned j = 0; j + 1 < degree; ++j)
            {
              const double rhokp = 1.0 / (2.0 * sigma - rhok);
              const double f1 = rhokp * rhok, f2 = 2.0 * rhokp / delta;
              rhok = rhokp;
              if (j < 2)
                lop->cheb_raw(oth, j == 0 ? nullptr : cur, nullptr, b, dinv.p, f1, f2, (int)j + 1, 1.0 / theta);
              else
                lop->cheb_raw(oth, cur, oth, b, dinv.p, f1, f2);
              std::swap(cur, oth);
            }
        }
      if (cur != S)
        hipLaunchKernelGGL((vec_copy_kernel<T, T>), grid_for(n), 256, 0, ctx->stream, S, cur, n);
    }

    T *
    step_raw(T *X, T *O, const T *b, const FusedTransferHost<T> *prolongate = nullptr, double *out_wide = nullptr)
    {
      const bool wide_in_pass = out_wide && degree >= 2 && std::fabs(delta) >= 1e-40 && sizeof(T) == 4;
      T *cur = X, *oth = O;
      if (prolongate)
        lop->cheb_prolongate_raw(oth, cur, b, dinv.p, 1.0 / theta, *prolongate);
      else
        lop->cheb_raw(oth, cur, nullptr, b, dinv.p, 0.0, 1.0 / theta);
      std::swap(cur, oth);
      if (degree >= 2 && std::fabs(delta) >= 1e-40)
        {
          double rhok = delta / theta, sigma = theta / delta;
          for (unsigned j = 0; j + 1 < degree; ++j)
            {
              const double rhokp = 1.0 / (2.0 * sigma - rhok);
              const double f1 = rhokp * rhok, f2 = 2.0 * rhokp / delta;
              rhok = rhokp;
              const bool last = j + 2 == degree;
              lop->cheb_raw(oth, cur, oth, b, dinv.p, f1, f2, 0, 0.0, (last && wide_in_pass) ? out_wide : nullptr);
              std::swap(cur, oth);
            }
        }
      if (out_wide && !wide_in_pass)
        hipLaunchKernelGGL((vec_copy_kernel<double, T>), grid_for(lop->n_dofs()), 256, 0, lop->ctx->stream, out_wide, cur, lop->n_dofs());
      return out_wide ? nullptr : cur;
    }

    void
    vmult(mgamd_vec &dst, const mgamd_vec &src) override
    {
      if (dst.n != lop->n_dofs() || src.n != lop->n_dofs() || dst.data == src.data)
        throw std::invalid_argument("PreconditionChebyshev::vmult: bad vectors");
      vmult_raw(dst.as<T>(), tmp.p, src.as<T>());
    }
    void
    step(mgamd_vec &dst, const mgamd_vec &src) override
    {
      if (dst.n != lop->n_dofs() || src.n != lop->n_dofs() || dst.data == src.data)
        throw std::invalid_argument("PreconditionChebyshev::step: bad vectors");
      T *res = step_raw(dst.as<T>(), tmp.p, src.as<T>());
      if (res != dst.as<T>())
        hipLaunchKernelGGL((vec_copy_kernel<T, T>), grid_for(dst.n), 256, 0, lop->ctx->stream, dst.as<T>(), res, dst.n);
    }
  };

  ChebyshevBase *
  make_chebyshev(LevelOperatorBase *op, unsigned degree, double smoothing_range, unsigned eig_cg_n_iterations)
  {
    if (degree < 1)
      throw std::invalid_argument("SmootherDegree must be >= 1");
    if (op->type == MGAMD_F64)
      return new Chebyshev<double>(static_cast<LevelOperator<double> *>(op), degree, smoothing_range, eig_cg_n_iterations);
    return new Chebyshev<float>(static_cast<LevelOperator<float> *>(op), degree, smoothing_range, eig_cg_n_iterations);
  }

  template <typename T>
  struct Transfer2 : Transfer2Base
  {
    struct GroupD
    {
      int                 kind = 0, nf = 2;
      size_t              n_patches = 0;
      DBuf<uint32_t>      coarse_idx, fine_idx, fine_idx_restrict;
      DBuf<uint16_t>      coarse_mask;
      std::vector<double> E;
      DBuf<uint32_t> p1_uniq_ptr, p1_uniq_idx, p1_fine_t, p1_fine_t_restrict;
      DBuf<uint16_t> p1_loc;
      uint32_t       p1_max_uniq = 0;
      void
      build_p1(const std::vector<uint32_t> &cidx, const std::vector<uint32_t> &fidx, const std::vector<uint32_t> *fidx_restrict)
      {
        const size_t          np = n_patches, nwg = (np + PATCH_P1_BLOCK - 1) / PATCH_P1_BLOCK;
        std::vector<uint32_t> ptr(nwg + 1, 0), idx, tmp;
        std::vector<uint16_t> l(np * 8, 0xFFFFu);
        for (size_t w = 0; w < nwg; ++w)
          {
            const size_t a = w * PATCH_P1_BLOCK, b = std::min(np, a + PATCH_P1_BLOCK);
            tmp.clear();
            for (size_t i = a * 8; i < b * 8; ++i)
              if (cidx[i] != INVALID_DOF)
                tmp.push_back(cidx[i]);
            std::sort(tmp.begin(), tmp.end());
            tmp.erase(std::unique(tmp.begin(), tmp.end()), tmp.end());
            for (size_t i = a * 8; i < b * 8; ++i)
              if (cidx[i] != INVALID_DOF)
                l[i] = (uint16_t)(std::lower_bound(tmp.begin(), tmp.end(), cidx[i]) - tmp.begin());
            idx.insert(idx.end(), tmp.begin(), tmp.end());
            ptr[w + 1]  = (uint32_t)idx.size();
            p1_max_uniq = std::max<uint32_t>(p1_max_uniq, (uint32_t)tmp.size());
          }
        if (idx.empty())
          idx.push_back(0);
        auto transpose = [&](const std::vector<uint32_t> &f) {
          std::vector<uint32_t> t(f.size());
          for (size_t q = 0; q < np; ++q)
            for (int k = 0; k < 27; ++k)
              t[(size_t)k * np + q] = f[q * 27 + k];
          return t;
        };
        p1_uniq_ptr.upload(ptr);
        p1_uniq_idx.upload(idx);
        p1_loc.upload(l);
        p1_fine_t.upload(transpose(fidx));
        if (fidx_restrict)
          p1_fine_t_restrict.upload(transpose(*fidx_restrict));
      }
    };
    struct BrickD
    {
      int            B = 2, fine_group = 0;
      size_t         n_bricks = 0;
      size_t         n_unfused = 0;
      bool           fused = false;
      DBuf<uint32_t> slot, coarse_idx, own_shell, own_shell_restrict;
    };
    FusedTransferHost<T> fused;
    DBuf<uint32_t>       fused_flags;
    DBuf<uint32_t>       fused_coarse_idx;
    DBuf<uint8_t>        fused_tail_flags;
    DBuf<uint32_t>       fused_tail_chunks;
    size_t               n_fused_bricks = 0;
    bool
    fused_ready() const
    {
      return fused.group >= 0 && n_fused_bricks > 0;
    }
    uint64_t
    n_fused_bricks_total() const override
    {
      return fused_ready() ? n_fused_bricks : 0;
    }
    GroupD                               grp[3];
    std::vector<std::unique_ptr<BrickD>> bricks;
    LevelOperator<T>                    *fop = nullptr, *cop = nullptr;
    int                                  pc = 1, pf = 1;
    Ctx                                 *ctx = nullptr;
    FE1D                                 fec;

    Transfer2(LevelOperator<T> *f, LevelOperator<T> *c)
      : fec(c->tables->p)
    {
      fine   = f;
      coarse = c;
      fop    = f;
      cop    = c;
      ctx    = f->ctx;
      int fuse_group = -1;
      if (!getenv("MGAMD_NO_FUSED_TRANSFER") && !f->tables->has_robin() && f->tables->tria != c->tables->tria && f->tables->p == c->tables->p &&
          !f->tables->ls_level && !c->tables->ls_level && fused_transfer_supported(f->tables->p))
        for (size_t gi = 0; gi < f->tables->groups.size(); ++gi)
          {
            const SlotGroup &g = f->tables->groups[gi];
            if (persistent_lattice(g.N) && !g.constrained_group && g.n_slots() > 0)
              fuse_group = (int)gi;
          }
      TransferTables tt(*f->tables, *c->tables, true, fuse_group);
      const uint32_t copy_lo = f->tables->n_interior + f->tables->n_tail_owned, copy_hi = f->tables->n_interior + f->tables->n_tail;
      auto           owned_only = [&](std::vector<uint32_t> v) {
        for (uint32_t &i : v)
          if (i != INVALID_DOF && i >= copy_lo && i < copy_hi)
            i = INVALID_DOF;
        return v;
      };
      for (const BrickTransferGroup &bg : tt.bricks)
        {
          auto d        = std::make_unique<BrickD>();
          d->B          = bg.B;
          d->fine_group = bg.fine_group;
          d->n_bricks   = bg.n_bricks();
          d->n_unfused  = bg.fused ? bg.n_unfused : bg.n_bricks();
          d->fused      = bg.fused;
          if (bg.fused && bg.n_bricks() > bg.n_unfused)
            {
              const SlotGroup &fg  = f->tables->groups[bg.fine_group];
              const size_t     ns  = fg.n_slots(), nsh = (size_t)fg.n_shell, nc3 = (size_t)bg.Nc * bg.Nc * bg.Nc;
              if (2 * ((nsh + 255) / 256) > 15)
                throw std::runtime_error("fused transfer: shell too large for the flag word");
              std::vector<uint32_t> fl(ns * 256, 0);
              std::vector<uint32_t> ci(ns * nc3, INVALID_DOF);
              for (size_t q = bg.n_unfused; q < bg.n_bricks(); ++q)
                {
                  const size_t sl = bg.slot[q];
                  for (size_t t = 0; t < 256; ++t)
                    fl[sl * 256 + t] = 0x8000u;
                  for (size_t t = 0; t < nsh; ++t)
                    fl[sl * 256 + t % 256] |= (uint32_t)(bg.shell_flags[q * nsh + t] & 3u) << (2 * (t / 256));
                  std::copy(bg.coarse_idx.begin() + q * nc3, bg.coarse_idx.begin() + (q + 1) * nc3, ci.begin() + sl * nc3);
                  for (size_t t = 0; t < nc3; ++t)
                    if (bg.coarse_idx[q * nc3 + t] == INVALID_DOF)
                      fl[sl * 256 + t % 256] |= 1u << (16 + t / 256);
                }
              fused_flags.upload(fl);
              fused_coarse_idx.upload(ci);
              fused_tail_flags.upload(tt.tail_owned_by_fused);
              fused.group      = bg.fine_group;
              fused.flags      = fused_flags.p;
              fused.coarse_idx = fused_coarse_idx.p;
              fused.nc3        = (uint32_t)nc3;
              fused.E          = fec.embedding(1, f->tables->p);
              fused.tail_flags = fused_tail_flags.p;
              n_fused_bricks   = bg.n_bricks() - bg.n_unfused;
              if (!f->halo && !f->tables->n_edge)
                {
                  std::vector<uint32_t> runs = tt.residual_tail_runs, chunks;
                  if (f->tables->n_dofs > f->tables->n_interior + f->tables->n_tail)
                    {
                      runs.push_back(f->tables->n_tail);
                      runs.push_back(f->tables->n_dofs - f->tables->n_interior);
                    }
                  for (size_t k = 0; k + 1 < runs.size(); k += 2)
                    for (uint32_t b0 = runs[k]; b0 < runs[k + 1]; b0 += TAIL_CHUNK)
                      {
                        chunks.push_back(b0);
                        chunks.push_back(std::min(runs[k + 1], b0 + TAIL_CHUNK));
                      }
                  fused.n_tail_chunks = (uint32_t)(chunks.size() / 2);
                  if (chunks.empty())
                    chunks.push_back(0);
                  fused_tail_chunks.upload(chunks);
                  fused.tail_chunks = fused_tail_chunks.p;
                }
            }
          d->slot.upload(bg.slot);
          d->coarse_idx.upload(bg.coarse_idx);
          d->own_shell.upload(bg.own_shell);
          if (copy_hi > copy_lo)
            d->own_shell_restrict.upload(owned_only(bg.own_shell));
          bricks.push_back(std::move(d));
        }
      pc = tt.pc;
      pf = tt.pf;
      for (int k = 0; k < 3; ++k)
        {
          grp[k].kind      = k;
          grp[k].nf        = tt.groups[k].nf;
          grp[k].n_patches = tt.groups[k].n_patches();
          if (grp[k].n_patches)
            {
              grp[k].coarse_idx.upload(tt.groups[k].coarse_idx);
              grp[k].coarse_mask.upload(tt.groups[k].coarse_mask);
              grp[k].fine_idx.upload(tt.groups[k].fine_idx);
              if (copy_hi > copy_lo)
                grp[k].fine_idx_restrict.upload(owned_only(tt.groups[k].fine_idx));
              if (k == 1 && tt.pc == 1 && grp[k].nf == 3)
                {
                  if (copy_hi > copy_lo)
                    {
                      const std::vector<uint32_t> fr = owned_only(tt.groups[k].fine_idx);
                      grp[k].build_p1(tt.groups[k].coarse_idx, tt.groups[k].fine_idx, &fr);
                    }
                  else
                    grp[k].build_p1(tt.groups[k].coarse_idx, tt.groups[k].fine_idx, nullptr);
                }
            }
          grp[k].E = fec.embedding(k, pf);
        }
    }

    template <int PC, int NF, bool IDENTITY>
    void
    launch(const GroupD &g, const T *src, T *dst, bool prolongate)
    {
      using G = TransferGeo<PC, NF>;
      TransferArgs<T, PC, NF> a;
      a.coarse_idx  = g.coarse_idx.p;
      a.coarse_mask = g.coarse_mask.p;
      a.fine_idx    = (!prolongate && g.fine_idx_restrict.p) ? g.fine_idx_restrict.p : g.fine_idx.p;
      a.n_patches   = (uint32_t)g.n_patches;
      const int n   = PC + 1;
      for (int i = 0; i < n * n; ++i)
        {
          a.m.M[i] = a.m.K[i] = 0.0;
          a.m.I0[i]           = fec.I[0][i];
          a.m.I1[i]           = fec.I[1][i];
        }
      if ((int)g.E.size() != NF * n)
        throw std::runtime_error("transfer: embedding size mismatch");
      for (int i = 0; i < NF * n; ++i)
        a.E[i] = g.E[i];
      a.src            = src;
      a.dst            = dst;
      const size_t lds = 2 * (size_t)G::SPW * G::NF3 * sizeof(T);
      const int    grid = (int)((g.n_patches + G::SPW - 1) / G::SPW);
      if (prolongate)
        launch_lds(ctx, ctx->stream, prolongate_kernel<T, PC, NF, IDENTITY>, grid, G::BLOCK, lds, a);
      else
        launch_lds(ctx, ctx->stream, restrict_kernel<T, PC, NF, IDENTITY>, grid, G::BLOCK, lds, a);
      HIP_CHECK(hipGetLastError());
    }

    void
    launch_p1(const GroupD &g, const T *src, T *dst, bool prolongate)
    {
      PatchP1Args<T> a;
      a.uniq_ptr    = g.p1_uniq_ptr.p;
      a.uniq_idx    = g.p1_uniq_idx.p;
      a.loc         = g.p1_loc.p;
      a.coarse_mask = g.coarse_mask.p;
      a.fine_idx_t  = (!prolongate && g.p1_fine_t_restrict.p) ? g.p1_fine_t_restrict.p : g.p1_fine_t.p;
      a.n_patches   = (uint32_t)g.n_patches;
      a.max_uniq    = g.p1_max_uniq;
      for (int i = 0; i < 4; ++i)
        {
          a.m.M[i] = a.m.K[i] = 0.0;
          a.m.I0[i]           = fec.I[0][i];
          a.m.I1[i]           = fec.I[1][i];
        }
      a.src = src;
      a.dst = dst;
      const int    grid = (int)((g.n_patches + PATCH_P1_BLOCK - 1) / PATCH_P1_BLOCK);
      const size_t lds  = (size_t)std::max<uint32_t>(g.p1_max_uniq, 1) * sizeof(T);
      if (prolongate)
        hipLaunchKernelGGL(patch_p1_prolongate_kernel<T>, grid, PATCH_P1_BLOCK, lds, ctx->stream, a);
      else
        hipLaunchKernelGGL(patch_p1_restrict_kernel<T>, grid, PATCH_P1_BLOCK, lds, ctx->stream, a);
      HIP_CHECK(hipGetLastError());
    }

    template <int P, int B>
    void
    launch_brick(const BrickD &b, const T *src, T *dst, bool prolongate, size_t n_launch)
    {
      if (n_launch == 0)
        return;
      using G = BrickTransferGeo<P, B>;
      BrickTransferArgs<T, P> a;
      const GroupDev<T>      &fg = *fop->groups[b.fine_group];
      a.slot          = b.slot.p;
      a.interior_base = fg.interior_base.p;
      a.shell_pos     = fg.shell_pos.p;
      a.coarse_idx    = b.coarse_idx.p;
      a.own_shell     = (!prolongate && b.own_shell_restrict.p) ? b.own_shell_restrict.p : b.own_shell.p;
      a.n_bricks      = (uint32_t)n_launch;
      const std::vector<double> E = fec.embedding(1, P);
      for (int i = 0; i < (2 * P + 1) * (P + 1); ++i)
        a.E[i] = E[i];
      a.src            = src;
      a.dst            = dst;
      const size_t lds = (size_t)G::LDS * sizeof(T);
      if (prolongate)
        launch_lds(ctx, ctx->stream, brick_prolongate_kernel<T, P, B>, (int)n_launch, G::BLOCK, lds, a);
      else if constexpr (persistent_lattice(G::NF))
        launch_persistent(ctx, ctx->stream, brick_restrict_persistent_kernel<T, P, B>, (int)n_launch, 3, G::BLOCK, lds, a);
      else
        launch_lds(ctx, ctx->stream, brick_restrict_kernel<T, P, B>, (int)n_launch, G::BLOCK, lds, a);
      HIP_CHECK(hipGetLastError());
    }

    void
    run(const T *src, T *dst, bool prolongate, bool skip_fused = false)
    {
      for (auto &b : bricks)
        {
          const size_t nb = skip_fused ? b->n_unfused : b->n_bricks;
          if (!dispatch_degree(pc, [&](auto P) {
                if (!dispatch_brick_size<P(), 2, 4, 8, 16>(b->B, [&](auto B) { launch_brick<P(), B()>(*b, src, dst, prolongate, nb); }))
                  throw std::runtime_error("brick transfer: unsupported brick size");
              }))
            throw std::runtime_error("brick transfer: degree not instantiated");
        }
      for (int k = 0; k < 3; ++k)
        {
          const GroupD &g = grp[k];
          if (!g.n_patches)
            continue;
          const int key = pc * 100 + g.nf;
          if (k == 0)
            {
              if (!dispatch_degree(pc, [&](auto P) { launch<P(), P() + 1, true>(g, src, dst, prolongate); }))
                throw std::runtime_error("transfer: degree not instantiated");
            }
          else
            switch (key)
              {
                case 103:
                  if (g.p1_uniq_ptr.p)
                    launch_p1(g, src, dst, prolongate);
                  else
                    launch<1, 3, false>(g, src, dst, prolongate);
                  break;
                case 104:
                  launch<1, 4, false>(g, src, dst, prolongate);
                  break;
                case 205:
                  launch<2, 5, false>(g, src, dst, prolongate);
                  break;
                case 206:
                  launch<2, 6, false>(g, src, dst, prolongate);
                  break;
                case 307:
                  launch<3, 7, false>(g, src, dst, prolongate);
                  break;
                case 308:
                  launch<3, 8, false>(g, src, dst, prolongate);
                  break;
                case 409:
                  launch<4, 9, false>(g, src, dst, prolongate);
                  break;
                case 511:
                  launch<5, 11, false>(g, src, dst, prolongate);
                  break;
                case 613:
                  launch<6, 13, false>(g, src, dst, prolongate);
                  break;
                case 715:
                  launch<7, 15, false>(g, src, dst, prolongate);
                  break;
                default:
                  throw std::runtime_error("transfer: (coarse degree, fine patch) combination not instantiated");
              }
        }
    }

    void
    residual_restrict_raw(T *dst_coarse, T *t, const T *b, const T *x)
    {
      FusedTransferHost<T> f = fused;
      f.coarse               = dst_coarse;
      Epilogue<T> e{t, x, nullptr, b, nullptr, T(0), T(0), T(0)};
      fop->template apply<MODE_RESIDUAL_RESTRICT>(x, e, false, 0, 0, &f);
    }
    void
    restrict_unfused_raw(T *dst_coarse, const T *src_fine)
    {
      run(src_fine, dst_coarse, false, true);
      finish_restriction(dst_coarse);
    }
    void
    prolongate_unfused_raw(T *dst_fine, const T *src_coarse)
    {
      run(src_coarse, dst_fine, true, true);
      if (fop->halo)
        fop->import_from_owner_raw(dst_fine + fop->tables->n_interior);
    }
    void
    prolongate_raw(T *dst_fine, const T *src_coarse)
    {
      run(src_coarse, dst_fine, true);
      if (fop->halo)
        fop->import_from_owner_raw(dst_fine + fop->tables->n_interior);
    }
    void
    restrict_raw(T *dst_coarse, const T *src_fine)
    {
      run(src_fine, dst_coarse, false);
      finish_restriction(dst_coarse);
    }
    void
    finish_restriction(T *dst_coarse)
    {
      if (auto *sc = dynamic_cast<SubsetComm *>(cop->comm.get()))
        {
          auto     *sf = dynamic_cast<SubsetComm *>(fop->comm.get());
          const int gf = sf ? sf->group : (fop->comm ? 1 : sc->group);
          if (gf != sc->group)
            {
              if (gf != 1)
                throw std::runtime_error("restriction between two rank-subset tiers of different group sizes is not supported");
              sc->replica_sum(dst_coarse, cop->n_dofs(), (int)sizeof(T), ctx->stream);
            }
        }
      if (cop->halo)
        cop->exchange_add_raw(dst_coarse + cop->tables->n_interior);
      else if (fop->comm)
        fop->comm->allreduce_sum(dst_coarse, cop->n_dofs(), (int)sizeof(T), ctx->stream);
    }
    void
    prolongate_and_add(mgamd_vec &dst, const mgamd_vec &src) override
    {
      if (dst.n != fine->n_dofs() || src.n != coarse->n_dofs())
        throw std::invalid_argument("prolongate_and_add: vector size mismatch");
      prolongate_raw(dst.as<T>(), src.as<T>());
    }
    void
    restrict_and_add(mgamd_vec &dst, const mgamd_vec &src) override
    {
      if (dst.n != coarse->n_dofs() || src.n != fine->n_dofs())
        throw std::invalid_argument("restrict_and_add: vector size mismatch");
      restrict_raw(dst.as<T>(), src.as<T>());
    }
  };

  Transfer2Base *
  make_transfer2(LevelOperatorBase *fine, LevelOperatorBase *coarse)
  {
    if (fine->type != coarse->type)
      throw std::invalid_argument("transfer: level number types differ");
    if (fine->type == MGAMD_F64)
      return new Transfer2<double>(static_cast<LevelOperator<double> *>(fine), static_cast<LevelOperator<double> *>(coarse));
    return new Transfer2<float>(static_cast<LevelOperator<float> *>(fine), static_cast<LevelOperator<float> *>(coarse));
  }

  int
  csr_spmv_lanes(uint32_t n_rows, size_t nnz)
  {
    const double avg = n_rows ? (double)nnz / n_rows : 0.0;
    return avg <= 6 ? 4 : (avg <= 24 ? 8 : (avg <= 64 ? 16 : 32));
  }
  int
  csr_spmv_lanes_long(uint32_t n_rows, size_t nnz)
  {
    const double avg       = n_rows ? (double)nnz / n_rows : 0.0;
    const char  *e         = getenv("MGAMD_SPMV_WAVE_MIN_MEAN_ROW");
    const double threshold = e ? atof(e) : CSR_SPMV_WAVE_MIN_MEAN_ROW;
    return avg > threshold ? 64 : csr_spmv_lanes(n_rows, nnz);
  }

  template <typename F>
  void
  dispatch_spmv(int mode, int lanes, F &&f)
  {
    auto with_lanes = [&](auto mode_tag) {
      switch (lanes)
        {
          case 4:
            f(mode_tag, std::integral_constant<int, 4>());
            break;
          case 8:
            f(mode_tag, std::integral_constant<int, 8>());
            break;
          case 16:
            f(mode_tag, std::integral_constant<int, 16>());
            break;
          case 32:
            f(mode_tag, std::integral_constant<int, 32>());
            break;
          case 64:
            f(mode_tag, std::integral_constant<int, 64>());
            break;
          default:
            throw std::invalid_argument("csr_spmv: lanes must be 4, 8, 16, 32 or 64");
        }
    };
    switch (mode)
      {
        case SPMV_PLAIN:
          with_lanes(std::integral_constant<int, SPMV_PLAIN>());
          break;
        case SPMV_ADD:
          with_lanes(std::integral_constant<int, SPMV_ADD>());
          break;
        case SPMV_RESID:
          with_lanes(std::integral_constant<int, SPMV_RESID>());
          break;
        case SPMV_CHEB:
          with_lanes(std::integral_constant<int, SPMV_CHEB>());
          break;
        case SPMV_DOT:
          with_lanes(std::integral_constant<int, SPMV_DOT>());
          break;
        default:
          throw std::invalid_argument("csr_spmv: unknown mode");
      }
  }

  template <typename T>
  int
  launch_csr_spmv(hipStream_t stream, int mode, int lanes, uint32_t n_rows, const uint32_t *ptr, const uint32_t *col, const T *val, const T *x,
                  T *y, const T *b, const T *xold, const T *dinv, double f1, double f2, double *partial, int max_blocks)
  {
    if (!n_rows)
      return 0;
    if (mode == SPMV_DOT && !partial)
      throw std::invalid_argument("csr_spmv: SPMV_DOT needs the buffer of the block partials");
    int grid = 0;
    dispatch_spmv(mode, lanes, [&](auto mode_tag, auto lanes_tag) {
      constexpr int MODE  = decltype(mode_tag)::value;
      constexpr int LANES = decltype(lanes_tag)::value;
      if constexpr ((MODE == SPMV_DOT || LANES == 64) && !std::is_same<T, double>::value)
        throw std::invalid_argument("csr_spmv: SPMV_DOT and 64 lanes per row are FP64 only");
      else
        {
          size_t g = std::min<size_t>(((size_t)n_rows * LANES + 255) / 256, MODE == SPMV_DOT ? 1024 : 4096);
          if (max_blocks > 0)
            g = std::min<size_t>(g, (size_t)max_blocks);
          grid = (int)g;
          if constexpr (LANES == 64)
            hipLaunchKernelGGL((csr_spmv_wave_kernel<T, MODE>), grid, 256, 0, stream, n_rows, ptr, col, val, x, y, b, xold, dinv, T(f1), T(f2),
                               partial);
          else
            hipLaunchKernelGGL((csr_spmv_kernel<T, MODE, LANES>), grid, 256, 0, stream, n_rows, ptr, col, val, x, y, b, xold, dinv, T(f1),
                               T(f2), partial);
        }
    });
    HIP_CHECK(hipGetLastError());
    return grid;
  }
  template int
  launch_csr_spmv<double>(hipStream_t, int, int, uint32_t, const uint32_t *, const uint32_t *, const double *, const double *, double *,
                          const double *, const double *, const double *, double, double, double *, int);
  template int
  launch_csr_spmv<float>(hipStream_t, int, int, uint32_t, const uint32_t *, const uint32_t *, const float *, const float *, float *,
                         const float *, const float *, const float *, double, double, double *, int);

  template <typename T>
  void
  launch_csr_spmv_range(hipStream_t stream, int mode, int lanes, uint32_t row_begin, uint32_t row_end, const uint32_t *ptr, const uint32_t *col,
                        const T *val, const T *x, T *y, const T *b, const T *xold, const T *dinv, double f1, double f2)
  {
    if (row_end <= row_begin)
      return;
    if (mode == SPMV_DOT || lanes == 64)
      throw std::invalid_argument("csr_spmv: a range of rows has neither SPMV_DOT nor 64 lanes per row");
    const uint32_t n_rows = row_end - row_begin;
    dispatch_spmv(mode, lanes, [&](auto mode_tag, auto lanes_tag) {
      constexpr int MODE  = decltype(mode_tag)::value;
      constexpr int LANES = decltype(lanes_tag)::value;
      if constexpr (MODE != SPMV_DOT && LANES != 64)
        {
          const int grid = (int)std::min<size_t>(((size_t)n_rows * LANES + 255) / 256, 4096);
          hipLaunchKernelGGL((csr_spmv_range_kernel<T, MODE, LANES>), grid, 256, 0, stream, row_begin, row_end, ptr, col, val, x, y, b, xold,
                             dinv, T(f1), T(f2));
        }
    });
    HIP_CHECK(hipGetLastError());
  }

  template <typename T>
  struct AmgCycle
  {
    struct Mat
    {
      DBuf<uint32_t> ptr, col;
      DBuf<T>        val;
      uint32_t       n_rows = 0, n_cols = 0;
      int            lanes  = 8;
      void
      upload(const CSR &A)
      {
        n_rows = A.n_rows;
        n_cols = A.n_cols;
        ptr.upload(A.ptr);
        col.upload(A.col.empty() ? std::vector<uint32_t>(1, 0) : A.col);
        std::vector<T> v(std::max<size_t>(A.val.size(), 1), T(0));
        std::copy(A.val.begin(), A.val.end(), v.begin());
        val.upload(v);
      }
    };
    struct Lvl
    {
      std::shared_ptr<Mat>  A;
      Mat                   P, R;
      DBuf<T>               dinv, x, b, r, t, send;
      DBuf<uint32_t>        send_idx;
      double                theta = 1, delta = 0;
      uint32_t              n = 0, n_int = 0, n_recv = 0, n_global = 0, n_owned = 0, n_ghost = 0;
      bool                  replicated = true;
      std::vector<int>      peers;
      std::vector<uint32_t> peer_offset;
    };
    Ctx                              *ctx = nullptr;
    LevelOperator<T>                 *op0 = nullptr;
    std::shared_ptr<Comm>             comm;
    std::vector<std::unique_ptr<Lvl>> lv;
    DBuf<double>                      coarse_inv;
    unsigned                          degree  = 2;
    bool                              overlap = true;
    bool                              long_rows = false;
    std::shared_ptr<Mat>              shared0;
    DBuf<uint32_t> in_amg, in_geo, out_amg, out_geo;
    uint32_t       n_in = 0, n_out = 0;

    int
    lanes_for(const CSR &M) const
    {
      return long_rows ? csr_spmv_lanes_long(M.n_rows, M.nnz()) : csr_spmv_lanes(M.n_rows, M.nnz());
    }
    AmgHierarchyHost
    build_hierarchy(CSR A0)
    {
      if (const char *e = getenv("MGAMD_AMG_SMOOTHER_DEGREE"))
        degree = std::max(1, atoi(e));
      AmgHierarchyHost H = build_smoothed_aggregation(std::move(A0));
      if (H.levels.back().A.n_rows > 4096)
        throw std::runtime_error("AMG: coarsening stalled at " + std::to_string(H.levels.back().A.n_rows) + " rows");
      coarse_inv.upload(H.coarse_inv);
      return H;
    }
    void
    add_level(const AmgLevelHost &G, const AmgShardLevel *P, bool last)
    {
      const bool whole = !P || P->replicated;
      auto       L     = std::make_unique<Lvl>();
      L->n_global = L->n = L->n_int = L->n_owned = G.A.n_rows;
      if (P)
        {
          L->replicated  = P->replicated;
          L->n_global    = P->n_global;
          L->n           = P->n_rows;
          L->n_int       = P->replicated ? P->n_rows : P->launch_interior();
          L->n_recv      = P->n_recv;
          L->n_owned     = P->n_owned();
          L->n_ghost     = P->n_ghost;
          L->peers       = P->peers;
          L->peer_offset = P->peer_offset;
        }
      if (lv.empty() && shared0)
        L->A = shared0;
      else
        {
          L->A = std::make_shared<Mat>();
          L->A->upload(whole ? G.A : P->A);
          L->A->lanes = lanes_for(G.A);
        }
      if (!last)
        {
          L->P.upload(whole ? G.P : P->P);
          L->R.upload(whole ? G.R : P->R);
          L->P.lanes = lanes_for(G.P);
          L->R.lanes = lanes_for(G.R);
        }
      std::vector<T> d(std::max<uint32_t>(L->n, 1), T(1));
      for (uint32_t i = 0; i < L->n; ++i)
        d[i] = (T)G.dinv[whole ? i : P->rows[i]];
// ... 1227 lines not shown
```

### dealii_multigrid_amd/csrc/runtime.hpp

```cpp
#pragma once
#include "api_common.hpp"
#include "comm.hpp"

#include <hip/hip_runtime.h>

#include <functional>
#include <map>
#include <sstream>

namespace mgamd
{
#define HIP_CHECK(expr)                                                                                       \
  do                                                                                                          \
    {                                                                                                         \
      hipError_t e_ = (expr);                                                                                 \
      if (e_ != hipSuccess)                                                                                   \
        {                                                                                                     \
          std::ostringstream os_;                                                                             \
          os_ << "HIP error " << hipGetErrorString(e_) << " at " << __FILE__ << ":" << __LINE__ << ": " #expr; \
          throw std::runtime_error(os_.str());                                                                \
        }                                                                                                     \
    }                                                                                                         \
  while (0)

  struct Ctx
  {
    int         device = 0;
    hipStream_t stream = nullptr;
    int         n_cu   = 256;
    double     *d_partial = nullptr;
    double     *d_result  = nullptr;
    double     *h_result  = nullptr;
    double     *d_cg      = nullptr;
    bool                                           profile = false;
    int                                            prof_brick = 0;
    std::vector<std::pair<hipEvent_t, hipEvent_t>> prof_events;
    size_t                                         prof_used  = 0;
    double                                         prof_bytes = 0.0;
    double                                         prof_bytes_moved = 0.0;
    double                                         prof_ms_accum = 0.0;
    uint64_t                                       prof_n_accum  = 0;

    hipStream_t             side = nullptr;
    std::vector<hipEvent_t> sync_events;
    size_t                  sync_next = 0;

    explicit Ctx(int dev);
    ~Ctx();
    void
    sync()
    {
      HIP_CHECK(hipStreamSynchronize(stream));
    }
    void
    order_after(hipStream_t to, hipStream_t from)
    {
      hipEvent_t e = sync_events[sync_next];
      sync_next    = (sync_next + 1) % sync_events.size();
      HIP_CHECK(hipEventRecord(e, from));
      HIP_CHECK(hipStreamWaitEvent(to, e, 0));
    }
    void
    harvest_profile();
  };

  template <typename T>
  struct DBuf
  {
    T     *p = nullptr;
    size_t n = 0;
    DBuf() = default;
    DBuf(const DBuf &) = delete;
    DBuf &
    operator=(const DBuf &) = delete;
    ~DBuf()
    {
      if (p)
        (void)hipFree(p);
    }
    void
    alloc(size_t count)
    {
      if (p)
        (void)hipFree(p);
      p = nullptr;
      n = count;
      if (count)
        HIP_CHECK(hipMalloc((void **)&p, count * sizeof(T)));
    }
    void
    upload(const std::vector<T> &h)
    {
      alloc(h.size());
      if (n)
        HIP_CHECK(hipMemcpy(p, h.data(), n * sizeof(T), hipMemcpyHostToDevice));
    }
    void
    zero(hipStream_t s)
    {
      if (n)
        HIP_CHECK(hipMemsetAsync(p, 0, n * sizeof(T), s));
    }
  };
}

struct mgamd_ctx
{
  std::unique_ptr<mgamd::Ctx> ctx;
};

struct mgamd_vec
{
  mgamd::Ctx *ctx  = nullptr;
  size_t      n    = 0;
  int         type = MGAMD_F64;
  void       *data = nullptr;
  ~mgamd_vec();
  template <typename T>
  T *
  as()
  {
    check<T>();
    return static_cast<T *>(data);
  }
  template <typename T>
  const T *
  as() const
  {
    check<T>();
    return static_cast<const T *>(data);
  }
  template <typename T>
  void
  check() const
  {
    if ((int)sizeof(T) != type)
      throw std::invalid_argument("vector number type does not match the operator's");
  }
};

namespace mgamd
{
  mgamd_vec *
  vec_create(Ctx *ctx, size_t n, int type);

  void
  vec_set(mgamd_vec &v, double value);
  void
  vec_copy(mgamd_vec &dst, const mgamd_vec &src);
  void
  vec_sadd(mgamd_vec &y, double s, double a, const mgamd_vec &x);
  double
  vec_dot(const mgamd_vec &x, const mgamd_vec &y);

  struct LevelOperatorBase
  {
    Ctx                         *ctx  = nullptr;
    int                          type = MGAMD_F64;
    std::shared_ptr<LevelTables> tables;
    std::shared_ptr<Tria>        tria;
    std::shared_ptr<Comm>        comm;
    std::shared_ptr<HaloPlan>    halo_plan;
    double sigma = 0.0;
    void
    refuse_singular(const char *who) const
    {
      if (tables->dirichlet_faces == 0 && sigma == 0.0 && !tables->has_robin())
        throw std::invalid_argument(std::string(who) + ": refused, the operator is singular: dirichlet_faces mask 0 (no Dirichlet face) with "
                                    "mass coefficient sigma = 0 and no convective face has the constants in its kernel, and no mean-value "
                                    "projection is built");
    }
    virtual ~LevelOperatorBase() = default;
    virtual double
    dot(const mgamd_vec &x, const mgamd_vec &y) = 0;
    virtual void
    exchange_add_tail(mgamd_vec &v) = 0;
    uint64_t
    n_dofs_owned() const
    {
      return (uint64_t)tables->n_interior + tables->n_tail_owned + tables->n_dirichlet_owned + tables->n_hanging_owned;
    }
    uint32_t
    n_dofs() const
    {
      return tables->n_dofs;
    }
    size_t
    n_dot() const
    {
      return comm ? (size_t)tables->n_interior + tables->n_tail_owned : (size_t)n_dofs();
    }
    virtual void
    vmult(mgamd_vec &dst, const mgamd_vec &src) = 0;
    virtual void
    vmult_mass(mgamd_vec &dst, const mgamd_vec &src) = 0;
    virtual void
    compute_inverse_diagonal(mgamd_vec &d) = 0;
    virtual void
    vmult_interface_up(mgamd_vec &dst, const mgamd_vec &src) = 0;
    virtual void
    vmult_interface_down(mgamd_vec &dst, const mgamd_vec &src) = 0;
    virtual size_t
    read_debug_stamps(unsigned long long *out, size_t max_count) = 0;
    void
    rhs(mgamd_vec &b, int kind = 0);
    void
    rhs_boundary_flux(mgamd_vec &b, const double q[6]);
    void
    distribute(mgamd_vec &x, int kind);
    virtual void
    rhs_dirichlet(mgamd_vec &rhs, const mgamd_vec &g, bool include_mass) = 0;
    virtual void
    distribute_values(mgamd_vec &x, const mgamd_vec &g) = 0;

  private:
    virtual void
    distribute_values_core(mgamd_vec &x, const mgamd_vec &g) = 0;
    void
    upload_load(mgamd_vec &b, const std::vector<double> &h);
  };

  struct ChebyshevBase
  {
    virtual ~ChebyshevBase() = default;
    LevelOperatorBase *op = nullptr;
    unsigned           degree = 3;
    double             min_eig = 0, max_eig = 0, theta = 1, delta = 0;
    virtual void
    vmult(mgamd_vec &dst, const mgamd_vec &src) = 0;
    virtual void
    step(mgamd_vec &dst, const mgamd_vec &src) = 0;
  };

  struct Transfer2Base
  {
    virtual ~Transfer2Base() = default;
    LevelOperatorBase *fine = nullptr, *coarse = nullptr;
    virtual void
    prolongate_and_add(mgamd_vec &dst_fine, const mgamd_vec &src_coarse) = 0;
    virtual void
    restrict_and_add(mgamd_vec &dst_coarse, const mgamd_vec &src_fine) = 0;
    virtual uint64_t
    n_fused_bricks_total() const = 0;
  };

  struct MultigridBase
  {
    virtual ~MultigridBase() = default;
    Ctx                 *ctx = nullptr;
    mgamd_stage_callback cb  = nullptr;
    void                *cb_user = nullptr;
    virtual void
    vcycle(mgamd_vec &z, const mgamd_vec &r) = 0;
    virtual double
    time_vcycles(mgamd_vec &z, const mgamd_vec &r, unsigned n, bool use_graph) = 0;
    virtual unsigned
    n_levels() const = 0;
    virtual void
    setup_local_smoothing(const LevelTables &active) = 0;
    virtual unsigned
    set_collapse(bool on) = 0;
    std::string coarse_used;
    int         number_type = MGAMD_F64;
    virtual LevelOperatorBase *
    finest_operator() const = 0;
    virtual const LevelTables *
    outer_tables() const = 0;
    virtual void
    vcycle_level_raw(void *z, const void *r) = 0;
    virtual void
    amg_layout(std::vector<uint32_t> &out) const = 0;
    virtual uint64_t
    coarse_cg_iterations() const = 0;

    struct StageRecord
    {
      int        stage;
      unsigned   level;
      hipEvent_t e0, e1;
    };
    bool                     stage_timing = false;
    std::vector<StageRecord> stage_records;
    size_t                   stage_used = 0;
    void
    set_stage_timing(bool on)
    {
      ctx->sync();
      stage_timing = on;
      stage_used   = 0;
    }
    size_t
    read_stage_times(double *ms)
    {
      ctx->sync();
      for (size_t i = 0; i < stage_used; ++i)
        {
          float t = 0;
          HIP_CHECK(hipEventElapsedTime(&t, stage_records[i].e0, stage_records[i].e1));
          ms[(size_t)stage_records[i].stage * n_levels() + stage_records[i].level] += t;
        }
      const size_t n = stage_used;
      stage_used     = 0;
      return n;
    }
    void
    release_stage_records()
    {
      for (auto &r : stage_records)
        {
          (void)hipEventDestroy(r.e0);
          (void)hipEventDestroy(r.e1);
        }
      stage_records.clear();
    }
  };

  LevelOperatorBase *
  make_level_operator(Ctx *ctx, const mgamd_dofs *dofs, int type, std::shared_ptr<Comm> comm = nullptr);
  ChebyshevBase *
  make_chebyshev(LevelOperatorBase *op, unsigned degree, double smoothing_range, unsigned eig_cg_n_iterations);
  Transfer2Base *
  make_transfer2(LevelOperatorBase *fine, LevelOperatorBase *coarse);
  MultigridBase *
  make_multigrid(Ctx *ctx, unsigned n_levels, LevelOperatorBase *const *levels, Transfer2Base *const *transfers,
                 ChebyshevBase *const *smoothers, const std::string &coarse_solver, MultigridBase *nested = nullptr,
                 unsigned n_cycles = 1, const LevelTables *amg_global = nullptr, uint32_t amg_min_sharded_rows = 0);
  void
  solve_cg(LevelOperatorBase &A, MultigridBase *M, mgamd_vec &x, const mgamd_vec &b, double reltol, double abstol, unsigned maxiter,
           unsigned &n_iterations, double &residual);
  struct ThetaStepperBase
  {
    virtual ~ThetaStepperBase() = default;
    double   theta = 1, dt = 0, t = 0;
    uint64_t n_steps = 0;
    virtual void
    step(mgamd_vec &u, const mgamd_vec *f_old, const mgamd_vec *f_new, double reltol, double abstol, unsigned maxiter, unsigned &n_iterations,
         double &residual) = 0;
    virtual void
    step_data(mgamd_vec &u, const mgamd_vec *f_old, const mgamd_vec *f_new, const mgamd_vec *g_old, const mgamd_vec *g_new, const mgamd_vec *load,
              double reltol, double abstol, unsigned maxiter, unsigned &n_iterations, double &residual) = 0;
  };
  ThetaStepperBase *
  make_theta_stepper(LevelOperatorBase &A, MultigridBase *M, double theta, double dt);
  int
  csr_spmv_lanes(uint32_t n_rows, size_t nnz);
  constexpr double CSR_SPMV_WAVE_MIN_MEAN_ROW = 144.0;
  int
  csr_spmv_lanes_long(uint32_t n_rows, size_t nnz);
  template <typename T>
  int
  launch_csr_spmv(hipStream_t stream, int mode, int lanes, uint32_t n_rows, const uint32_t *ptr, const uint32_t *col, const T *val, const T *x,
                  T *y, const T *b, const T *xold, const T *dinv, double f1, double f2, double *partial = nullptr, int max_blocks = 0);

  struct AssembledMatrixBase
  {
    virtual ~AssembledMatrixBase() = default;
    Ctx     *ctx    = nullptr;
    uint32_t n_rows = 0;
    uint64_t nnz    = 0;
    int      lanes  = 0;
    virtual void
    vmult(mgamd_vec &dst, const mgamd_vec &src) = 0;
    virtual double
    time_spmv(int mode, int lanes, unsigned reps) = 0;
  };
  struct AmgPreconditionerBase
  {
    virtual ~AmgPreconditionerBase() = default;
    virtual void
    vmult(mgamd_vec &z, const mgamd_vec &r) = 0;
    virtual void
    layout(std::vector<uint32_t> &rows_per_level) const = 0;
  };
  std::shared_ptr<AssembledMatrixBase>
  make_assembled_matrix(Ctx *ctx, const mgamd_dofs *dofs);
  AmgPreconditionerBase *
  make_amg_preconditioner(const std::shared_ptr<AssembledMatrixBase> &A, unsigned n_cycles);
  void
  solve_cg_matrix(AssembledMatrixBase &A, AmgPreconditionerBase *M, mgamd_vec &x, const mgamd_vec &b, double reltol, double abstol,
                  unsigned maxiter, unsigned &n_iterations, double &residual);
}

struct mgamd_level_op
{
  std::unique_ptr<mgamd::LevelOperatorBase> op;
};
struct mgamd_cheb
{
  std::unique_ptr<mgamd::ChebyshevBase> c;
};
struct mgamd_transfer2
{
  std::unique_ptr<mgamd::Transfer2Base> t;
};
struct mgamd_mg
{
  std::unique_ptr<mgamd::MultigridBase> mg;
};
struct mgamd_time_stepper
{
  std::unique_ptr<mgamd::ThetaStepperBase> ts;
};
struct mgamd_matrix
{
  std::shared_ptr<mgamd::AssembledMatrixBase> A;
};
struct mgamd_amg
{
  std::unique_ptr<mgamd::AmgPreconditionerBase> P;
};
```

### include/mgamd.h

```cpp
#ifndef MGAMD_H
#define MGAMD_H

#include <stddef.h>
#include <stdint.h>

#ifdef __cplusplus
extern "C" {
#endif

#define MGAMD_OK 0
#define MGAMD_ERR 1
#define MGAMD_ERR_NO_DEVICE 2
#define MGAMD_ERR_INVALID 3

#define MGAMD_INVALID_DOF 0xFFFFFFFFu

typedef struct mgamd_ctx       mgamd_ctx;
typedef struct mgamd_tria      mgamd_tria;
typedef struct mgamd_dofs      mgamd_dofs;
typedef struct mgamd_vec       mgamd_vec;
typedef struct mgamd_level_op  mgamd_level_op;
typedef struct mgamd_cheb      mgamd_cheb;
typedef struct mgamd_transfer2 mgamd_transfer2;
typedef struct mgamd_mg        mgamd_mg;
typedef struct mgamd_matrix    mgamd_matrix;
typedef struct mgamd_amg       mgamd_amg;
typedef struct mgamd_partition mgamd_partition;
typedef struct mgamd_comm      mgamd_comm;
typedef struct mgamd_sim_group mgamd_sim_group;

const char *mgamd_last_error(void);
const char *mgamd_version(void);


int mgamd_tria_create(const char *geometry, unsigned n_ref_global, unsigned n_ref_local, mgamd_tria **out);
int mgamd_tria_create_from_leaves(uint64_t n_leaves, const uint8_t *level, const uint32_t *i, const uint32_t *j, const uint32_t *k,
                                  mgamd_tria **out);
int mgamd_tria_coarsen(const mgamd_tria *fine, mgamd_tria **out);
int mgamd_tria_destroy(mgamd_tria *t);
int mgamd_tria_info(const mgamd_tria *t, uint64_t *n_cells, uint32_t *n_levels, uint64_t *n_cells_hn);
int mgamd_tria_get_cells(const mgamd_tria *t, uint8_t *level, uint32_t *i, uint32_t *j, uint32_t *k, uint16_t *mask);

int mgamd_tria_set_coefficient(mgamd_tria *t, const double *a);
int mgamd_tria_get_coefficient(const mgamd_tria *t, double *a);
int mgamd_tria_has_coefficient(const mgamd_tria *t, int *has);

int mgamd_tria_set_dirichlet_faces(mgamd_tria *t, unsigned mask);
int mgamd_tria_get_dirichlet_faces(const mgamd_tria *t, unsigned *mask);
int mgamd_tria_set_robin_coefficients(mgamd_tria *t, const double beta[6]);
int mgamd_tria_get_robin_coefficients(const mgamd_tria *t, double beta[6]);

typedef struct
{
  uint32_t degree;
  uint64_t n_cells;
  uint32_t n_dofs;
  uint32_t n_interior;
  uint32_t n_tail;
  uint32_t n_dirichlet;
  uint32_t n_hanging;
  uint32_t n_groups;
  uint32_t group_B[8];
  uint64_t group_slots[8];
  uint32_t n_tail_owned, n_dirichlet_owned, n_hanging_owned;
  uint32_t n_peers;
  uint32_t n_halo_send;
  uint32_t n_edge;
  uint64_t group_halo_slots[8];
} mgamd_dofs_info_t;

int mgamd_dofs_create(const mgamd_tria *t, int degree, int max_brick, mgamd_dofs **out);
int mgamd_dofs_destroy(mgamd_dofs *d);
int mgamd_dofs_info(const mgamd_dofs *d, mgamd_dofs_info_t *info);
int mgamd_dofs_get_cell_slots(const mgamd_dofs *d, uint8_t *group, uint32_t *slot);
int mgamd_dofs_get_keys(const mgamd_dofs *d, int32_t *keys);
int mgamd_dofs_get_cell_dofs(const mgamd_dofs *d, uint32_t *out);
int mgamd_dofs_rhs_constant(const mgamd_dofs *d, double *out);
int mgamd_dofs_rhs(const mgamd_dofs *d, int kind, double *out);
int mgamd_dofs_distribute(const mgamd_dofs *d, int kind, double *x);
int mgamd_dofs_dirichlet_faces(const mgamd_dofs *d, unsigned *mask);
int mgamd_dofs_rhs_boundary_flux(const mgamd_dofs *d, const double q[6], double *out);
int mgamd_dofs_robin_coefficients(const mgamd_dofs *d, double beta[6]);
int mgamd_dofs_robin_faces(const mgamd_dofs *d, uint64_t *n_faces, uint32_t *idx, uint8_t *flags, double *scale);
int mgamd_dofs_rhs_dirichlet(const mgamd_dofs *d, const double *g, int include_mass, double *out);
int mgamd_dofs_distribute_values(const mgamd_dofs *d, const double *g, double *x);
int mgamd_dofs_dirichlet_face_values(const mgamd_dofs *d, const double v[6], double *g);
int mgamd_dofs_dirichlet_cells(const mgamd_dofs *d, uint64_t *n_cells, uint32_t *idx, uint16_t *mask, double *scale);
int mgamd_dofs_node_positions(const mgamd_dofs *d, double *xyz);
int mgamd_dofs_set_mass_coefficient(mgamd_dofs *d, double sigma);
int mgamd_dofs_mass_coefficient(const mgamd_dofs *d, double *sigma);
int mgamd_dofs_coefficient_range(const mgamd_dofs *d, double *min, double *max);

int mgamd_dofs_matrix(const mgamd_dofs *d, uint64_t *nnz, uint32_t *row_ptr, uint32_t *col, double *val);
int mgamd_dofs_amg_setup_info(const mgamd_dofs *d, uint32_t *n_levels, uint32_t *rows, uint64_t *nnz, uint32_t max_levels);

int mgamd_tria_level_mesh(const mgamd_tria *fine, unsigned level, mgamd_tria **out);
int mgamd_dofs_create_level(const mgamd_tria *level_mesh, int degree, int max_brick, mgamd_dofs **out);
int mgamd_ls_copy_indices(const mgamd_dofs *active_mesh_dofs, const mgamd_dofs *level_dofs, unsigned level, uint64_t *count,
                          uint32_t *global_idx, uint32_t *level_idx);

int mgamd_partition_create(const mgamd_tria *const *trias, unsigned n_levels, unsigned n_ranks, double hanging_weight,
                           mgamd_partition **out);
int mgamd_partition_create_ex(const mgamd_tria *const *trias, unsigned n_levels, unsigned n_ranks, double hanging_weight,
                              uint64_t min_root_cells, mgamd_partition **out);
int mgamd_partition_create_tiered(const mgamd_tria *const *trias, unsigned n_levels, unsigned n_ranks, double hanging_weight,
                                  uint64_t min_root_cells, unsigned group, uint64_t min_sub_root_cells, mgamd_partition **out);
int mgamd_partition_tiers(const mgamd_partition *p, unsigned *sub_root_level, unsigned *group);
int mgamd_partition_destroy(mgamd_partition *p);
int mgamd_partition_statistics(const mgamd_partition *p, double stats[5]);
int mgamd_partition_info(const mgamd_partition *p, unsigned *root_level, unsigned *n_ranks);
int mgamd_partition_get_owner(const mgamd_partition *p, unsigned level, uint16_t *owner);
int mgamd_dofs_create_local(const mgamd_partition *p, unsigned level, unsigned rank, int degree, int max_brick, mgamd_dofs **out);

int mgamd_dofs_halo_sizes(const mgamd_dofs *d, uint32_t sizes[4]);
int mgamd_dofs_halo_get(const mgamd_dofs *d, int32_t *peers, uint32_t *peer_offset, uint32_t *pack_idx, uint32_t *sh_tail,
                        uint32_t *sh_ptr, int32_t *sh_src, int32_t *sh_owner_src);

int mgamd_transfer_tables_info(const mgamd_dofs *fine, const mgamd_dofs *coarse, uint64_t n_patches[3], uint32_t nf[3]);
int mgamd_transfer_tables_get(const mgamd_dofs *fine, const mgamd_dofs *coarse, int kind, uint32_t *coarse_idx,
                              uint16_t *coarse_mask, uint32_t *fine_idx);


#define MGAMD_DIRECT_COARSE_MAX_DOFS 4096u

int mgamd_level_plan(const char *type, unsigned n_meshes, unsigned degree, unsigned max_levels, unsigned *n_levels, unsigned *mesh_index,
                     unsigned *degrees, int *local_smoothing);

#define MGAMD_COARSE_PLAIN 0
#define MGAMD_COARSE_NESTED 1
#define MGAMD_COARSE_SHARDED_AMG 2
int mgamd_coarse_plan(const char *coarse_name, uint64_t n_level0_dofs_global, int level0_distributed, int sharded_amg_requested, int *plan);

int mgamd_partition_defaults(unsigned n_ranks, unsigned p_low, unsigned *group, uint64_t *min_root_cells, uint64_t *min_sub_root_cells);

int mgamd_ctx_create(int device, mgamd_ctx **out);
int mgamd_ctx_destroy(mgamd_ctx *ctx);
int mgamd_ctx_synchronize(mgamd_ctx *ctx);
int mgamd_ctx_stream(mgamd_ctx *ctx, void **stream);

int mgamd_comm_rccl_unique_id(char id[128]);
int mgamd_comm_rccl_create(mgamd_ctx *ctx, unsigned n_ranks, unsigned rank, const char id[128], mgamd_comm **out);
int mgamd_sim_group_create(unsigned n_ranks, mgamd_sim_group **out);
int mgamd_sim_group_destroy(mgamd_sim_group *g);
int mgamd_comm_sim_create(mgamd_sim_group *g, unsigned rank, mgamd_comm **out);
int mgamd_comm_subset(mgamd_comm *base, unsigned group, mgamd_comm **out);
int mgamd_comm_destroy(mgamd_comm *c);
int mgamd_comm_allreduce_sum(mgamd_comm *c, mgamd_ctx *ctx, double value, double *result);

#define MGAMD_F64 8
#define MGAMD_F32 4

int mgamd_vec_create(mgamd_ctx *ctx, uint64_t n, int number_type, mgamd_vec **out);
int mgamd_vec_destroy(mgamd_vec *v);
int mgamd_vec_size(const mgamd_vec *v, uint64_t *n);
int mgamd_vec_from_host(mgamd_vec *v, const double *src);
int mgamd_vec_to_host(const mgamd_vec *v, double *dst);
int mgamd_vec_set(mgamd_vec *v, double value);
int mgamd_vec_copy(mgamd_vec *dst, const mgamd_vec *src);
int mgamd_vec_axpy(mgamd_vec *y, double a, const mgamd_vec *x);
int mgamd_vec_sadd(mgamd_vec *y, double s, double a, const mgamd_vec *x);
int mgamd_vec_dot(const mgamd_vec *x, const mgamd_vec *y, double *result);
int mgamd_vec_norm2(const mgamd_vec *x, double *result);

int mgamd_level_op_create(mgamd_ctx *ctx, const mgamd_dofs *dofs, int number_type, mgamd_level_op **out);
int mgamd_level_op_create_distributed(mgamd_ctx *ctx, const mgamd_dofs *dofs, int number_type, mgamd_comm *comm, mgamd_level_op **out);
int mgamd_level_op_destroy(mgamd_level_op *op);
int mgamd_level_op_dot(mgamd_level_op *op, const mgamd_vec *x, const mgamd_vec *y, double *result);
int mgamd_level_op_exchange_add_tail(mgamd_level_op *op, mgamd_vec *v);
int mgamd_level_op_n_owned(const mgamd_level_op *op, uint64_t *n);
int mgamd_level_op_m(const mgamd_level_op *op, uint64_t *n);
int mgamd_level_op_mass_coefficient(const mgamd_level_op *op, double *sigma);
int mgamd_level_op_init_vector(const mgamd_level_op *op, mgamd_vec **out);
int mgamd_level_op_vmult(mgamd_level_op *op, mgamd_vec *dst, const mgamd_vec *src);
int mgamd_level_op_vmult_mass(mgamd_level_op *op, mgamd_vec *dst, const mgamd_vec *src);
int mgamd_level_op_inverse_diagonal(mgamd_level_op *op, mgamd_vec *diagonal);
int mgamd_level_op_rhs(mgamd_level_op *op, mgamd_vec *rhs);
int mgamd_level_op_rhs_kind(mgamd_level_op *op, int kind, mgamd_vec *rhs);
int mgamd_level_op_rhs_boundary_flux(mgamd_level_op *op, const double q[6], mgamd_vec *rhs);
int mgamd_level_op_distribute(mgamd_level_op *op, int kind, mgamd_vec *x);
int mgamd_level_op_rhs_dirichlet(mgamd_level_op *op, const mgamd_vec *g, int include_mass, mgamd_vec *rhs);
int mgamd_level_op_distribute_values(mgamd_level_op *op, mgamd_vec *x, const mgamd_vec *g);

int mgamd_cheb_create(mgamd_level_op *op, unsigned degree, double smoothing_range, unsigned eig_cg_n_iterations,
                      mgamd_cheb **out);
int mgamd_cheb_destroy(mgamd_cheb *c);
int mgamd_cheb_vmult(mgamd_cheb *c, mgamd_vec *dst, const mgamd_vec *src);
int mgamd_cheb_step(mgamd_cheb *c, mgamd_vec *dst, const mgamd_vec *src);
int mgamd_cheb_get_eigen_estimates(const mgamd_cheb *c, double *min_eigenvalue, double *max_eigenvalue);

int mgamd_transfer2_create(mgamd_level_op *fine, mgamd_level_op *coarse, mgamd_transfer2 **out);
int mgamd_transfer2_destroy(mgamd_transfer2 *t);
int mgamd_transfer2_prolongate_and_add(mgamd_transfer2 *t, mgamd_vec *dst_fine, const mgamd_vec *src_coarse);
int mgamd_transfer2_restrict_and_add(mgamd_transfer2 *t, mgamd_vec *dst_coarse, const mgamd_vec *src_fine);
int mgamd_transfer2_n_fused_bricks(const mgamd_transfer2 *t, uint64_t *n);

int mgamd_mg_create(mgamd_ctx *ctx, unsigned n_levels, mgamd_level_op *const *levels, mgamd_transfer2 *const *transfers,
                    mgamd_cheb *const *smoothers, const char *coarse_solver, mgamd_mg **out);
int mgamd_mg_create_nested(mgamd_ctx *ctx, unsigned n_levels, mgamd_level_op *const *levels, mgamd_transfer2 *const *transfers,
                           mgamd_cheb *const *smoothers, const char *coarse_solver, mgamd_mg *coarse_mg, unsigned n_cycles,
                           mgamd_mg **out);
int mgamd_mg_coarse_solver_used(const mgamd_mg *mg, char name[32]);
#define MGAMD_AMG_MIN_SHARDED_ROWS_DEFAULT 20000u
int mgamd_mg_create_sharded_amg(mgamd_ctx *ctx, unsigned n_levels, mgamd_level_op *const *levels, mgamd_transfer2 *const *transfers,
                                mgamd_cheb *const *smoothers, const char *coarse_solver, const mgamd_dofs *global_coarse_dofs,
                                unsigned n_cycles, uint32_t min_sharded_rows, mgamd_mg **out);
int mgamd_mg_coarse_iterations(const mgamd_mg *mg, uint64_t *n_iterations);
int mgamd_mg_amg_layout(const mgamd_mg *mg, uint32_t *n_levels, uint32_t *info, uint32_t max_levels);
int mgamd_mg_create_local_smoothing(mgamd_ctx *ctx, unsigned n_levels, mgamd_level_op *const *levels, mgamd_transfer2 *const *transfers,
                                    mgamd_cheb *const *smoothers, const mgamd_dofs *active_mesh_dofs, const char *coarse_solver,
                                    mgamd_mg **out);
int mgamd_level_op_vmult_interface_up(mgamd_level_op *op, mgamd_vec *dst, const mgamd_vec *src);
int mgamd_level_op_vmult_interface_down(mgamd_level_op *op, mgamd_vec *dst, const mgamd_vec *src);
int mgamd_mg_set_collapse(mgamd_mg *mg, int enable, unsigned *collapse_level);
int mgamd_mg_destroy(mgamd_mg *mg);
int mgamd_mg_vcycle(mgamd_mg *mg, mgamd_vec *z, const mgamd_vec *r);
typedef void (*mgamd_stage_callback)(int stage, int start, unsigned level, void *user);
int mgamd_mg_set_stage_callback(mgamd_mg *mg, mgamd_stage_callback cb, void *user);
int mgamd_mg_stage_timing(mgamd_mg *mg, int enable);
int mgamd_mg_stage_times(mgamd_mg *mg, double *ms, unsigned n_levels, uint64_t *n_records);
int mgamd_mg_time_vcycles(mgamd_mg *mg, mgamd_vec *z, const mgamd_vec *r, unsigned n, int use_graph, double *ms_per_cycle);

int mgamd_solve_cg(mgamd_level_op *A, mgamd_mg *preconditioner, mgamd_vec *x, const mgamd_vec *b, double reltol, double abstol,
                   unsigned maxiter, unsigned *n_iterations, double *residual_norm);

typedef struct mgamd_time_stepper mgamd_time_stepper;
int mgamd_time_stepper_create(mgamd_level_op *A, mgamd_mg *preconditioner, double theta, double dt, mgamd_time_stepper **out);
int mgamd_time_stepper_step(mgamd_time_stepper *ts, mgamd_vec *u, const mgamd_vec *f_old, const mgamd_vec *f_new, double reltol,
                            double abstol, unsigned maxiter, unsigned *n_iterations, double *residual_norm);
int mgamd_time_stepper_step_data(mgamd_time_stepper *ts, mgamd_vec *u, const mgamd_vec *f_old, const mgamd_vec *f_new,
                                 const mgamd_vec *g_old, const mgamd_vec *g_new, const mgamd_vec *load, double reltol, double abstol,
                                 unsigned maxiter, unsigned *n_iterations, double *residual_norm);
int  mgamd_time_stepper_time(const mgamd_time_stepper *ts, double *t, uint64_t *n_steps);
void mgamd_time_stepper_destroy(mgamd_time_stepper *ts);

int mgamd_matrix_create(mgamd_ctx *ctx, const mgamd_dofs *dofs, mgamd_matrix **out);
int mgamd_matrix_destroy(mgamd_matrix *A);
int mgamd_matrix_info(const mgamd_matrix *A, uint64_t *n_rows, uint64_t *nnz, int *lanes);
int mgamd_matrix_vmult(mgamd_matrix *A, mgamd_vec *dst, const mgamd_vec *src);
int mgamd_amg_create(mgamd_matrix *A, unsigned n_cycles, mgamd_amg **out);
int mgamd_amg_destroy(mgamd_amg *P);
int mgamd_amg_vmult(mgamd_amg *P, mgamd_vec *z, const mgamd_vec *r);
int mgamd_amg_layout(const mgamd_amg *P, uint32_t *n_levels, uint32_t *rows, uint32_t max_levels);
int mgamd_solve_cg_matrix(mgamd_matrix *A, mgamd_amg *preconditioner, mgamd_vec *x, const mgamd_vec *b, double reltol, double abstol,
                          unsigned maxiter, unsigned *n_iterations, double *residual_norm);

#ifdef __cplusplus
}
#endif
#endif
```

Before: 15.57 billion DoF/s.

## Merge transfer kernel launches into planned multi-member stages per level

Turns the per-variant prolongation and restriction kernels (identity patch, general patch, P1 patch, bricks) into device body functions. A stage kernel dispatches to them by block-index ranges, and a launch plan is precomputed once per direction and fused mode. Small groups share one merged launch, while large brick groups and persistent bricks keep their own launches. The aim is fewer kernel launches and less tail idle time across the transfer stages. The cost is a fixed 256-thread block for patch kernels, which can lower occupancy for small patch sizes, and larger kernel argument structs. A launch-plan query API is also exposed.

```diff
diff --git a/dealii_multigrid_amd/__init__.py b/dealii_multigrid_amd/__init__.py
--- a/dealii_multigrid_amd/__init__.py
+++ b/dealii_multigrid_amd/__init__.py
@@ -676,6 +676,16 @@
         n = C.c_uint64()
         _chk(_lib.mgamd_transfer2_n_fused_bricks(self._h, C.byref(n)))
         return n.value
+
+    MEMBERS = ("identity", "patch", "patch_p1", "bricks", "bricks17")
+
+    def launch_plan(self, prolongate: bool, skip_fused: bool = False):
+        n, cap = C.c_uint32(), 8
+        buf = (C.c_uint32 * (cap * len(self.MEMBERS)))()
+        _chk(_lib.mgamd_transfer2_launch_plan(self._h, C.c_int(int(prolongate)), C.c_int(int(skip_fused)), C.byref(n), buf, C.c_uint32(cap)))
+        assert n.value <= cap
+        k = len(self.MEMBERS)
+        return [{m: buf[l * k + i] for i, m in enumerate(self.MEMBERS) if buf[l * k + i]} for l in range(n.value)]
 
     def __del__(self):
         if getattr(self, "_h", None) and _lib is not None:
diff --git a/dealii_multigrid_amd/csrc/c_api_device.hip b/dealii_multigrid_amd/csrc/c_api_device.hip
--- a/dealii_multigrid_amd/csrc/c_api_device.hip
+++ b/dealii_multigrid_amd/csrc/c_api_device.hip
@@ -564,6 +564,16 @@
   MGAMD_TRY
   REQUIRE(t && n);
   *n = t->t->n_fused_bricks_total();
+  MGAMD_CATCH
+}
+
+int
+mgamd_transfer2_launch_plan(const mgamd_transfer2 *t, int prolongate, int skip_fused, uint32_t *n_launches, uint32_t *members,
+                            uint32_t max_launches)
+{
+  MGAMD_TRY
+  REQUIRE(t && n_launches);
+  *n_launches = t->t->launch_plan(prolongate != 0, skip_fused != 0, members, members ? max_launches : 0);
   MGAMD_CATCH
 }
 
diff --git a/dealii_multigrid_amd/csrc/kernels_transfer.hpp b/dealii_multigrid_amd/csrc/kernels_transfer.hpp
--- a/dealii_multigrid_amd/csrc/kernels_transfer.hpp
+++ b/dealii_multigrid_amd/csrc/kernels_transfer.hpp
@@ -11,27 +11,21 @@
     static constexpr int NF3   = NF * NF * NF;
     static constexpr int LINES = NF * NF;
     static constexpr int SPW   = LINES >= 256 ? 1 : 256 / LINES;
-    static constexpr int BLOCK = ((SPW * LINES + 63) / 64) * 64;
+    static constexpr int BLOCK = 256;
+    static_assert(SPW * LINES <= BLOCK, "a patch line per thread");
   };
 
-  template <typename T, int PC, int NF>
-  struct TransferArgs
+  struct PatchTables
   {
     const uint32_t *coarse_idx;
     const uint16_t *coarse_mask;
     const uint32_t *fine_idx;
     uint32_t        n_patches;
-    Mats<PC, T>     m;
-    T               E[NF * (PC + 1)];
-    const T        *src;
-    T              *dst;
   };
-  static_assert(sizeof(TransferArgs<double, MAX_KERNEL_DEGREE, 2 * MAX_KERNEL_DEGREE + 1>) <= KERNARG_LIMIT,
-                "TransferArgs exceeds the kernel-argument segment");
 
   template <typename T, int PC, int NF>
   __device__ __forceinline__ void
-  fine_rmw(const TransferArgs<T, PC, NF> &args, const T *__restrict__ buf, int p0, int np, int tid)
+  fine_rmw(const PatchTables &t, T *dst, const T *__restrict__ buf, int p0, int np, int tid)
   {
     using G           = TransferGeo<PC, NF>;
     constexpr int ITF = (G::SPW * G::NF3 + G::BLOCK - 1) / G::BLOCK;
@@ -41,29 +35,29 @@
     for (int it = 0; it < ITF; ++it)
       {
         const int idx = tid + it * G::BLOCK;
-        gi[it]        = idx < np * G::NF3 ? args.fine_idx[(size_t)p0 * G::NF3 + idx] : DEV_INVALID;
+        gi[it]        = idx < np * G::NF3 ? t.fine_idx[(size_t)p0 * G::NF3 + idx] : DEV_INVALID;
       }
 #pragma unroll
     for (int it = 0; it < ITF; ++it)
-      val[it] = args.dst[gi[it] != DEV_INVALID ? gi[it] : 0];
+      val[it] = dst[gi[it] != DEV_INVALID ? gi[it] : 0];
 #pragma unroll
     for (int it = 0; it < ITF; ++it)
       if (gi[it] != DEV_INVALID)
-        args.dst[gi[it]] = val[it] + buf[tid + it * G::BLOCK];
-  }
-
-  template <typename T, int PC, int NF, bool IDENTITY>
-  __global__ void
-  __launch_bounds__((TransferGeo<PC, NF>::BLOCK)) prolongate_kernel(const TransferArgs<T, PC, NF> args)
+        dst[gi[it]] = val[it] + buf[tid + it * G::BLOCK];
+  }
+
+
+  template <typename T, int PC, int NF, bool IDENTITY, typename A>
+  __device__ __forceinline__ void
+  prolongate_body(const A &args, const PatchTables &t, const uint32_t block, unsigned char *smem_raw)
   {
     using G = TransferGeo<PC, NF>;
-    extern __shared__ __align__(16) unsigned char smem_raw[];
     T *bufA = reinterpret_cast<T *>(smem_raw);
     T *bufB = bufA + G::SPW * G::NF3;
 
     const int tid    = threadIdx.x;
-    const int p0     = blockIdx.x * G::SPW;
-    const int np     = min((int)G::SPW, (int)args.n_patches - p0);
+    const int p0     = (int)block * G::SPW;
+    const int np     = min((int)G::SPW, (int)t.n_patches - p0);
     const int sl     = tid / G::LINES;
     const int ln     = tid % G::LINES;
     const int u = ln % NF, v = ln / NF;
@@ -77,7 +71,7 @@
       for (int it = 0; it < ITC; ++it)
         {
           const int idx = tid + it * G::BLOCK;
-          gi[it]        = idx < np * G::NC3 ? args.coarse_idx[(size_t)p0 * G::NC3 + idx] : DEV_INVALID;
+          gi[it]        = idx < np * G::NC3 ? t.coarse_idx[(size_t)p0 * G::NC3 + idx] : DEV_INVALID;
         }
 #pragma unroll
       for (int it = 0; it < ITC; ++it)
@@ -93,7 +87,7 @@
     __syncthreads();
     uint32_t mask = 0;
     if (act)
-      mask = args.coarse_mask[p0 + sl];
+      mask = t.coarse_mask[p0 + sl];
     const bool any_hanging = __syncthreads_or((int)(mask >> 3)) != 0;
     if (any_hanging)
       {
@@ -103,7 +97,7 @@
       }
     if (IDENTITY)
       {
-        fine_rmw<T, PC, NF>(args, bufB, p0, np, tid);
+        fine_rmw<T, PC, NF>(t, args.dst, bufB, p0, np, tid);
         return;
       }
     if (act && u < G::NC && v < G::NC)
@@ -157,21 +151,20 @@
           }
       }
     __syncthreads();
-    fine_rmw<T, PC, NF>(args, bufA, p0, np, tid);
-  }
-
-  template <typename T, int PC, int NF, bool IDENTITY>
-  __global__ void
-  __launch_bounds__((TransferGeo<PC, NF>::BLOCK)) restrict_kernel(const TransferArgs<T, PC, NF> args)
+    fine_rmw<T, PC, NF>(t, args.dst, bufA, p0, np, tid);
+  }
+
+  template <typename T, int PC, int NF, bool IDENTITY, typename A>
+  __device__ __forceinline__ void
+  restrict_body(const A &args, const PatchTables &t, const uint32_t block, unsigned char *smem_raw)
   {
     using G = TransferGeo<PC, NF>;
-    extern __shared__ __align__(16) unsigned char smem_raw[];
     T *bufA = reinterpret_cast<T *>(smem_raw);
     T *bufB = bufA + G::SPW * G::NF3;
 
     const int tid    = threadIdx.x;
-    const int p0     = blockIdx.x * G::SPW;
-    const int np     = min((int)G::SPW, (int)args.n_patches - p0);
+    const int p0     = (int)block * G::SPW;
+    const int np     = min((int)G::SPW, (int)t.n_patches - p0);
     const int sl     = tid / G::LINES;
     const int ln     = tid % G::LINES;
     const int u = ln % NF, v = ln / NF;
@@ -185,7 +178,7 @@
       for (int it = 0; it < ITF; ++it)
         {
           const int idx = tid + it * G::BLOCK;
-          gi[it]        = idx < np * G::NF3 ? args.fine_idx[(size_t)p0 * G::NF3 + idx] : DEV_INVALID;
+          gi[it]        = idx < np * G::NF3 ? t.fine_idx[(size_t)p0 * G::NF3 + idx] : DEV_INVALID;
         }
 #pragma unroll
       for (int it = 0; it < ITF; ++it)
@@ -256,7 +249,7 @@
     T *res = IDENTITY ? bufA : bufB;
     uint32_t mask = 0;
     if (act)
-      mask = args.coarse_mask[p0 + sl];
+      mask = t.coarse_mask[p0 + sl];
     const bool any_hanging = __syncthreads_or((int)(mask >> 3)) != 0;
     if (any_hanging)
       {
@@ -271,7 +264,7 @@
       for (int it = 0; it < ITC; ++it)
         {
           const int idx = tid + it * G::BLOCK;
-          gi[it]        = idx < np * G::NC3 ? args.coarse_idx[(size_t)p0 * G::NC3 + idx] : DEV_INVALID;
+          gi[it]        = idx < np * G::NC3 ? t.coarse_idx[(size_t)p0 * G::NC3 + idx] : DEV_INVALID;
         }
 #pragma unroll
       for (int it = 0; it < ITC; ++it)
@@ -283,47 +276,40 @@
     }
   }
 
-  template <typename T>
-  struct PatchP1Args
+  struct PatchP1Tables
   {
     const uint32_t *uniq_ptr;
     const uint32_t *uniq_idx;
     const uint16_t *loc;
     const uint16_t *coarse_mask;
     const uint32_t *fine_idx_t;
-    uint32_t        n_patches, max_uniq;
-    Mats<1, T>      m;
-    const T        *src;
-    T              *dst;
+    uint32_t        n_patches;
   };
-  static_assert(sizeof(PatchP1Args<double>) <= KERNARG_LIMIT, "PatchP1Args exceeds the kernel-argument segment");
   constexpr int PATCH_P1_BLOCK = 256;
   constexpr int PATCH_P1_ITERS = 8;
 
-  template <typename T>
-  __global__ void
-  __launch_bounds__(PATCH_P1_BLOCK) patch_p1_prolongate_kernel(const PatchP1Args<T> a)
-  {
-    extern __shared__ __align__(16) unsigned char smem_raw[];
+  template <typename T, typename A>
+  __device__ __forceinline__ void
+  patch_p1_prolongate_body(const A &a, const PatchP1Tables &g, const uint32_t wg, unsigned char *smem_raw)
+  {
     T             *U    = reinterpret_cast<T *>(smem_raw);
     const int      tid  = threadIdx.x;
-    const uint32_t wg   = blockIdx.x;
     const uint32_t pch  = wg * PATCH_P1_BLOCK + tid;
-    const bool     act  = pch < a.n_patches;
-    const uint32_t p0   = a.uniq_ptr[wg];
-    const int      nu   = (int)(a.uniq_ptr[wg + 1] - p0);
-    const uint4    lw   = reinterpret_cast<const uint4 *>(a.loc)[act ? pch : 0];
-    const uint32_t mask = act ? a.coarse_mask[pch] : 0u;
+    const bool     act  = pch < g.n_patches;
+    const uint32_t p0   = g.uniq_ptr[wg];
+    const int      nu   = (int)(g.uniq_ptr[wg + 1] - p0);
+    const uint4    lw   = reinterpret_cast<const uint4 *>(g.loc)[act ? pch : 0];
+    const uint32_t mask = act ? g.coarse_mask[pch] : 0u;
     uint32_t       fi[27];
 #pragma unroll
     for (int t = 0; t < 27; ++t)
-      fi[t] = act ? a.fine_idx_t[(size_t)t * a.n_patches + pch] : DEV_INVALID;
+      fi[t] = act ? g.fine_idx_t[(size_t)t * g.n_patches + pch] : DEV_INVALID;
     T gv[PATCH_P1_ITERS];
 #pragma unroll
     for (int k = 0; k < PATCH_P1_ITERS; ++k)
       {
         const int j = tid + k * PATCH_P1_BLOCK;
-        gv[k]       = nu > 0 ? a.src[a.uniq_idx[p0 + (j < nu ? j : nu - 1)]] : T(0);
+        gv[k]       = nu > 0 ? a.src[g.uniq_idx[p0 + (j < nu ? j : nu - 1)]] : T(0);
       }
 #pragma unroll
     for (int k = 0; k < PATCH_P1_ITERS; ++k)
@@ -377,24 +363,22 @@
       }
   }
 
-  template <typename T>
-  __global__ void
-  __launch_bounds__(PATCH_P1_BLOCK) patch_p1_restrict_kernel(const PatchP1Args<T> a)
-  {
-    extern __shared__ __align__(16) unsigned char smem_raw[];
+  template <typename T, typename A>
+  __device__ __forceinline__ void
+  patch_p1_restrict_body(const A &a, const PatchP1Tables &g, const uint32_t wg, unsigned char *smem_raw)
+  {
     T             *Acc  = reinterpret_cast<T *>(smem_raw);
     const int      tid  = threadIdx.x;
-    const uint32_t wg   = blockIdx.x;
     const uint32_t pch  = wg * PATCH_P1_BLOCK + tid;
-    const bool     act  = pch < a.n_patches;
-    const uint32_t p0   = a.uniq_ptr[wg];
-    const int      nu   = (int)(a.uniq_ptr[wg + 1] - p0);
-    const uint4    lw   = reinterpret_cast<const uint4 *>(a.loc)[act ? pch : 0];
-    const uint32_t mask = act ? a.coarse_mask[pch] : 0u;
+    const bool     act  = pch < g.n_patches;
+    const uint32_t p0   = g.uniq_ptr[wg];
+    const int      nu   = (int)(g.uniq_ptr[wg + 1] - p0);
+    const uint4    lw   = reinterpret_cast<const uint4 *>(g.loc)[act ? pch : 0];
+    const uint32_t mask = act ? g.coarse_mask[pch] : 0u;
     uint32_t       fi[27];
 #pragma unroll
     for (int t = 0; t < 27; ++t)
-      fi[t] = act ? a.fine_idx_t[(size_t)t * a.n_patches + pch] : DEV_INVALID;
+      fi[t] = act ? g.fine_idx_t[(size_t)t * g.n_patches + pch] : DEV_INVALID;
     T r[27];
 #pragma unroll
     for (int t = 0; t < 27; ++t)
@@ -443,7 +427,7 @@
       }
     __syncthreads();
     for (int j = tid; j < nu; j += PATCH_P1_BLOCK)
-      atomic_add(&a.dst[a.uniq_idx[p0 + j]], Acc[j]);
+      atomic_add(&a.dst[g.uniq_idx[p0 + j]], Acc[j]);
   }
 
   template <int P, int B>
@@ -473,24 +457,32 @@
   };
   static_assert(sizeof(BrickTransferArgs<double, MAX_KERNEL_DEGREE>) <= KERNARG_LIMIT, "BrickTransferArgs exceeds the kernel-argument segment");
 
-  template <typename T, int P, int B>
-  __global__ void
-  __launch_bounds__(256, 4) brick_prolongate_kernel(const BrickTransferArgs<T, P> args)
+  struct BrickTables
+  {
+    const uint32_t *slot, *interior_base;
+    const uint16_t *shell_pos;
+    const uint32_t *coarse_idx, *own_shell;
+    uint32_t        n_bricks;
+    uint32_t        B;
+  };
+
+  template <typename T, int P, int B, typename A>
+  __device__ __forceinline__ void
+  brick_prolongate_body(const A &args, const BrickTables &t, const uint32_t block, const uint32_t nblocks, unsigned char *smem_raw)
   {
     using G  = BrickTransferGeo<P, B>;
     using LG = Geo<P, B>;
-    extern __shared__ __align__(16) unsigned char smem_raw[];
     T *buf = reinterpret_cast<T *>(smem_raw);
     constexpr int NC = G::NC, NF = G::NF, BLOCK = G::BLOCK;
     const int      tid   = threadIdx.x;
-    const uint32_t brick = xcd_contiguous(blockIdx.x, gridDim.x);
-    const uint32_t slot  = args.slot[brick];
+    const uint32_t brick = xcd_contiguous(block, nblocks);
+    const uint32_t slot  = t.slot[brick];
 
     constexpr int  NI_P  = LG::NI > 0 ? LG::NI : 1;
     constexpr int  NIN_P = LG::N_INT > 0 ? LG::N_INT : 1;
     constexpr int  ITI_P = (NIN_P + BLOCK - 1) / BLOCK;
     constexpr int  ITS_P = (LG::N_SHELL + BLOCK - 1) / BLOCK;
-    const uint32_t ibase = LG::N_INT > 0 ? args.interior_base[slot] : 0u;
+    const uint32_t ibase = LG::N_INT > 0 ? t.interior_base[slot] : 0u;
     T              ival[ITI_P];
     uint32_t       sgi_p[ITS_P];
     T              sval_p[ITS_P];
@@ -507,7 +499,7 @@
     for (int it = 0; it < ITS_P; ++it)
       {
         const int s = tid + it * BLOCK;
-        sgi_p[it]   = s < LG::N_SHELL ? NT_LOAD(&args.own_shell[(size_t)brick * LG::N_SHELL + s]) : DEV_INVALID;
+        sgi_p[it]   = s < LG::N_SHELL ? NT_LOAD(&t.own_shell[(size_t)brick * LG::N_SHELL + s]) : DEV_INVALID;
       }
 #pragma unroll
     for (int it = 0; it < ITS_P; ++it)
@@ -521,7 +513,7 @@
       for (int it = 0; it < ITC; ++it)
         {
           const int idx = tid + it * BLOCK;
-          gi[it]        = idx < G::NC3 ? NT_LOAD(&args.coarse_idx[(size_t)brick * G::NC3 + idx]) : DEV_INVALID;
+          gi[it]        = idx < G::NC3 ? NT_LOAD(&t.coarse_idx[(size_t)brick * G::NC3 + idx]) : DEV_INVALID;
         }
 #pragma unroll
       for (int it = 0; it < ITC; ++it)
@@ -591,28 +583,27 @@
 #pragma unroll
     for (int it = 0; it < ITS_P; ++it)
       if (sgi_p[it] != DEV_INVALID)
-        args.dst[sgi_p[it]] = sval_p[it] + buf[args.shell_pos[tid + it * BLOCK]];
-  }
-
-  template <typename T, int P, int B>
-  __global__ void
-  __launch_bounds__(256) brick_restrict_kernel(const BrickTransferArgs<T, P> args)
+        args.dst[sgi_p[it]] = sval_p[it] + buf[t.shell_pos[tid + it * BLOCK]];
+  }
+
+  template <typename T, int P, int B, typename A>
+  __device__ __forceinline__ void
+  brick_restrict_body(const A &args, const BrickTables &t, const uint32_t block, const uint32_t nblocks, unsigned char *smem_raw)
   {
     using G  = BrickTransferGeo<P, B>;
     using LG = Geo<P, B>;
-    extern __shared__ __align__(16) unsigned char smem_raw[];
     T *buf = reinterpret_cast<T *>(smem_raw);
     constexpr int NC = G::NC, NF = G::NF, BLOCK = G::BLOCK;
     const int      tid   = threadIdx.x;
-    const uint32_t brick = xcd_contiguous(blockIdx.x, gridDim.x);
-    const uint32_t slot  = args.slot[brick];
+    const uint32_t brick = xcd_contiguous(block, nblocks);
+    const uint32_t slot  = t.slot[brick];
 
     if (LG::N_INT > 0)
       {
         constexpr int  NI_  = LG::NI > 0 ? LG::NI : 1;
         constexpr int  NIN_ = LG::N_INT > 0 ? LG::N_INT : 1;
         constexpr int  ITI  = (NIN_ + BLOCK - 1) / BLOCK;
-        const uint32_t base = args.interior_base[slot];
+        const uint32_t base = t.interior_base[slot];
         T              val[ITI];
 #pragma unroll
         for (int it = 0; it < ITI; ++it)
@@ -639,7 +630,7 @@
       for (int it = 0; it < ITS; ++it)
         {
           const int s = tid + it * BLOCK;
-          gi[it]      = s < LG::N_SHELL ? NT_LOAD(&args.own_shell[(size_t)brick * LG::N_SHELL + s]) : DEV_INVALID;
+          gi[it]      = s < LG::N_SHELL ? NT_LOAD(&t.own_shell[(size_t)brick * LG::N_SHELL + s]) : DEV_INVALID;
         }
 #pragma unroll
       for (int it = 0; it < ITS; ++it)
@@ -647,7 +638,7 @@
 #pragma unroll
       for (int it = 0; it < ITS; ++it)
         if (tid + it * BLOCK < LG::N_SHELL)
-          buf[args.shell_pos[tid + it * BLOCK]] = gi[it] != DEV_INVALID ? val[it] : T(0);
+          buf[t.shell_pos[tid + it * BLOCK]] = gi[it] != DEV_INVALID ? val[it] : T(0);
     }
     constexpr int ITC_R = (G::NC3 + BLOCK - 1) / BLOCK;
     uint32_t      cgi[ITC_R];
@@ -657,7 +648,7 @@
     for (int it = 0; it < ITC_R; ++it)
       {
         const int idx = tid + it * BLOCK;
-        cgi[it]       = idx < G::NC3 ? NT_LOAD(&args.coarse_idx[(size_t)brick * G::NC3 + idx]) : DEV_INVALID;
+        cgi[it]       = idx < G::NC3 ? NT_LOAD(&t.coarse_idx[(size_t)brick * G::NC3 + idx]) : DEV_INVALID;
         const int x = idx % NC, y = (idx / NC) % NC, z = idx / (NC * NC);
         cinner[it] = x > 0 && y > 0 && z > 0 && x < NC - 1 && y < NC - 1 && z < NC - 1;
       }
@@ -878,4 +869,139 @@
       }
   }
 
+  constexpr int TM_PATCH   = 1;
+  constexpr int TM_IDENT   = 2;
+  constexpr int TM_P1      = 4;
+  constexpr int TM_BRICKS  = 8;
+  constexpr int TM_BRICK17 = 16;
+  constexpr int MAX_STAGE_BRICK_GROUPS = 4;
+
+  template <typename T, int PC, int NF>
+  struct TransferStageArgs
+  {
+    uint32_t      end_patch, end_p1, end_brick[MAX_STAGE_BRICK_GROUPS];
+    PatchTables   patch, ident;
+    PatchP1Tables p1;
+    BrickTables   brick[MAX_STAGE_BRICK_GROUPS];
+    Mats<PC, T>   m;
+    T             E[NF * (PC + 1)];
+    const T      *src;
+    T            *dst;
+  };
+  static_assert(sizeof(TransferStageArgs<double, MAX_KERNEL_DEGREE, 2 * MAX_KERNEL_DEGREE + 1>) <= KERNARG_LIMIT,
+                "TransferStageArgs exceeds the kernel-argument segment");
+
+  template <int PC, int B>
+  constexpr bool
+  stage_has_brick(int members)
+  {
+    return PC * B + 1 <= 17 && (members & (PC * B + 1 == 17 ? TM_BRICK17 : TM_BRICKS)) != 0;
+  }
+
+  template <typename A>
+  __device__ __forceinline__ BrickTables
+  stage_brick_group(const A &a, const uint32_t b, uint32_t &lo, uint32_t &hi)
+  {
+    BrickTables t = a.brick[0];
+    lo            = a.end_p1;
+    hi            = a.end_brick[0];
+#pragma unroll
+    for (int k = 1; k < MAX_STAGE_BRICK_GROUPS; ++k)
+      if (b >= a.end_brick[k - 1])
+        {
+          t  = a.brick[k];
+          lo = a.end_brick[k - 1];
+          hi = a.end_brick[k];
+        }
+    return t;
+  }
+
+  template <typename T, int PC, int B, int MEMBERS, bool PROLONGATE, typename A>
+  __device__ __forceinline__ void
+  stage_brick_size(const A &a, const BrickTables &t, const uint32_t block, const uint32_t nblocks, unsigned char *smem_raw)
+  {
+    if constexpr (stage_has_brick<PC, B>(MEMBERS))
+      if (t.B == B)
+        {
+          if constexpr (PROLONGATE)
+            brick_prolongate_body<T, PC, B>(a, t, block, nblocks, smem_raw);
+          else
+            brick_restrict_body<T, PC, B>(a, t, block, nblocks, smem_raw);
+        }
+  }
+  template <typename T, int PC, int MEMBERS, bool PROLONGATE, typename A>
+  __device__ __forceinline__ void
+  stage_brick_body(const A &a, const BrickTables &t, const uint32_t block, const uint32_t nblocks, unsigned char *smem_raw)
+  {
+    stage_brick_size<T, PC, 2, MEMBERS, PROLONGATE>(a, t, block, nblocks, smem_raw);
+    stage_brick_size<T, PC, 4, MEMBERS, PROLONGATE>(a, t, block, nblocks, smem_raw);
+    stage_brick_size<T, PC, 8, MEMBERS, PROLONGATE>(a, t, block, nblocks, smem_raw);
+    stage_brick_size<T, PC, 16, MEMBERS, PROLONGATE>(a, t, block, nblocks, smem_raw);
+  }
+
+  template <typename T, int PC, int NF, int MEMBERS>
+  __global__ void
+  __launch_bounds__(256, (MEMBERS == TM_BRICK17 ? 4 : 1)) prolongate_stage_kernel(const TransferStageArgs<T, PC, NF> a)
+  {
+    static_assert(!(MEMBERS & (TM_BRICKS | TM_BRICK17 | TM_IDENT)) || NF == 2 * PC + 1, "bricks and identity patches: h-transfers");
+    static_assert(!(MEMBERS & TM_P1) || (PC == 1 && NF == 3), "the register patches are the h-patches of p = 1");
+    extern __shared__ __align__(16) unsigned char smem_raw[];
+    const uint32_t b = blockIdx.x;
+    if constexpr ((MEMBERS & TM_PATCH) != 0)
+      if (b < a.end_patch)
+        {
+          prolongate_body<T, PC, NF, false>(a, a.patch, b, smem_raw);
+          return;
+        }
+    if constexpr ((MEMBERS & TM_P1) != 0)
+      if (b < a.end_p1)
+        {
+          patch_p1_prolongate_body<T>(a, a.p1, b - a.end_patch, smem_raw);
+          return;
+        }
+    if constexpr ((MEMBERS & (TM_BRICKS | TM_BRICK17)) != 0)
+      if (b < a.end_brick[MAX_STAGE_BRICK_GROUPS - 1])
+        {
+          uint32_t          lo, hi;
+          const BrickTables t = stage_brick_group(a, b, lo, hi);
+          stage_brick_body<T, PC, MEMBERS, true>(a, t, b - lo, hi - lo, smem_raw);
+          return;
+        }
+    if constexpr ((MEMBERS & TM_IDENT) != 0)
+      prolongate_body<T, PC, PC + 1, true>(a, a.ident, b - a.end_brick[MAX_STAGE_BRICK_GROUPS - 1], smem_raw);
+  }
+
+  template <typename T, int PC, int NF, int MEMBERS>
+  __global__ void
+  __launch_bounds__(256) restrict_stage_kernel(const TransferStageArgs<T, PC, NF> a)
+  {
+    static_assert(!(MEMBERS & (TM_BRICKS | TM_IDENT)) || NF == 2 * PC + 1, "bricks and identity patches: h-transfers");
+    static_assert(!(MEMBERS & TM_P1) || (PC == 1 && NF == 3), "the register patches are the h-patches of p = 1");
+    static_assert(!(MEMBERS & TM_BRICK17), "17-point bricks: the persistent kernel");
+    extern __shared__ __align__(16) unsigned char smem_raw[];
+    const uint32_t b = blockIdx.x;
+    if constexpr ((MEMBERS & TM_PATCH) != 0)
+      if (b < a.end_patch)
+        {
+          restrict_body<T, PC, NF, false>(a, a.patch, b, smem_raw);
+          return;
+        }
+    if constexpr ((MEMBERS & TM_P1) != 0)
+      if (b < a.end_p1)
+        {
+          patch_p1_restrict_body<T>(a, a.p1, b - a.end_patch, smem_raw);
+          return;
+        }
+    if constexpr ((MEMBERS & TM_BRICKS) != 0)
+      if (b < a.end_brick[MAX_STAGE_BRICK_GROUPS - 1])
+        {
+          uint32_t          lo, hi;
+          const BrickTables t = stage_brick_group(a, b, lo, hi);
+          stage_brick_body<T, PC, MEMBERS, false>(a, t, b - lo, hi - lo, smem_raw);
+          return;
+        }
+    if constexpr ((MEMBERS & TM_IDENT) != 0)
+      restrict_body<T, PC, PC + 1, true>(a, a.ident, b - a.end_brick[MAX_STAGE_BRICK_GROUPS - 1], smem_raw);
+  }
+
 }
diff --git a/dealii_multigrid_amd/csrc/runtime.hip b/dealii_multigrid_amd/csrc/runtime.hip
--- a/dealii_multigrid_amd/csrc/runtime.hip
+++ b/dealii_multigrid_amd/csrc/runtime.hip
@@ -751,74 +751,52 @@
             }
           grp[k].E = fec.embedding(k, pf);
         }
-    }
-
-    template <int PC, int NF, bool IDENTITY>
-    void
-    launch(const GroupD &g, const T *src, T *dst, bool prolongate)
-    {
-      using G = TransferGeo<PC, NF>;
-      TransferArgs<T, PC, NF> a;
-      a.coarse_idx  = g.coarse_idx.p;
-      a.coarse_mask = g.coarse_mask.p;
-      a.fine_idx    = (!prolongate && g.fine_idx_restrict.p) ? g.fine_idx_restrict.p : g.fine_idx.p;
-      a.n_patches   = (uint32_t)g.n_patches;
-      const int n   = PC + 1;
-      for (int i = 0; i < n * n; ++i)
-        {
-          a.m.M[i] = a.m.K[i] = 0.0;
-          a.m.I0[i]           = fec.I[0][i];
-          a.m.I1[i]           = fec.I[1][i];
-        }
-      if ((int)g.E.size() != NF * n)
-        throw std::runtime_error("transfer: embedding size mismatch");
-      for (int i = 0; i < NF * n; ++i)
-        a.E[i] = g.E[i];
-      a.src            = src;
-      a.dst            = dst;
-      const size_t lds = 2 * (size_t)G::SPW * G::NF3 * sizeof(T);
-      const int    grid = (int)((g.n_patches + G::SPW - 1) / G::SPW);
-      if (prolongate)
-        launch_lds(ctx, ctx->stream, prolongate_kernel<T, PC, NF, IDENTITY>, grid, G::BLOCK, lds, a);
+      plan_stages();
+    }
+
+    struct StageLaunch
+    {
+      std::function<void(const T *, T *)> launch;
+      uint32_t                            members[MGAMD_TRANSFER_N_MEMBERS] = {};
+    };
+    std::vector<StageLaunch> stages[2][2];
+
+    unsigned
+    launch_plan(bool prolongate, bool skip_fused, uint32_t *members, unsigned max_launches) const override
+    {
+      const std::vector<StageLaunch> &st = stages[prolongate][skip_fused];
+      for (size_t l = 0; l < st.size() && l < max_launches; ++l)
+        std::copy(st[l].members, st[l].members + MGAMD_TRANSFER_N_MEMBERS, members + l * MGAMD_TRANSFER_N_MEMBERS);
+      return (unsigned)st.size();
+    }
+
+    template <int PC, int NF, int MEMBERS, bool prolongate>
+    void
+    add_stage(bool skip_fused, const TransferStageArgs<T, PC, NF> &args, size_t lds, const uint32_t (&members)[MGAMD_TRANSFER_N_MEMBERS])
+    {
+      const int grid = (int)args.end_brick[MAX_STAGE_BRICK_GROUPS - 1] + (int)((args.ident.n_patches + TransferGeo<PC, PC + 1>::SPW - 1) / TransferGeo<PC, PC + 1>::SPW);
+      if (grid == 0)
+        return;
+      StageLaunch s;
+      std::copy(members, members + MGAMD_TRANSFER_N_MEMBERS, s.members);
+      void (*kern)(TransferStageArgs<T, PC, NF>) = nullptr;
+      if constexpr (prolongate)
+        kern = prolongate_stage_kernel<T, PC, NF, MEMBERS>;
       else
-        launch_lds(ctx, ctx->stream, restrict_kernel<T, PC, NF, IDENTITY>, grid, G::BLOCK, lds, a);
-      HIP_CHECK(hipGetLastError());
-    }
-
-    void
-    launch_p1(const GroupD &g, const T *src, T *dst, bool prolongate)
-    {
-      PatchP1Args<T> a;
-      a.uniq_ptr    = g.p1_uniq_ptr.p;
-      a.uniq_idx    = g.p1_uniq_idx.p;
-      a.loc         = g.p1_loc.p;
-      a.coarse_mask = g.coarse_mask.p;
-      a.fine_idx_t  = (!prolongate && g.p1_fine_t_restrict.p) ? g.p1_fine_t_restrict.p : g.p1_fine_t.p;
-      a.n_patches   = (uint32_t)g.n_patches;
-      a.max_uniq    = g.p1_max_uniq;
-      for (int i = 0; i < 4; ++i)
-        {
-          a.m.M[i] = a.m.K[i] = 0.0;
-          a.m.I0[i]           = fec.I[0][i];
-          a.m.I1[i]           = fec.I[1][i];
-        }
-      a.src = src;
-      a.dst = dst;
-      const int    grid = (int)((g.n_patches + PATCH_P1_BLOCK - 1) / PATCH_P1_BLOCK);
-      const size_t lds  = (size_t)std::max<uint32_t>(g.p1_max_uniq, 1) * sizeof(T);
-      if (prolongate)
-        hipLaunchKernelGGL(patch_p1_prolongate_kernel<T>, grid, PATCH_P1_BLOCK, lds, ctx->stream, a);
-      else
-        hipLaunchKernelGGL(patch_p1_restrict_kernel<T>, grid, PATCH_P1_BLOCK, lds, ctx->stream, a);
-      HIP_CHECK(hipGetLastError());
+        kern = restrict_stage_kernel<T, PC, NF, MEMBERS>;
+      s.launch = [this, a = args, kern, grid, lds](const T *src, T *dst) mutable {
+        a.src = src;
+        a.dst = dst;
+        launch_lds(ctx, ctx->stream, kern, grid, 256, lds, a);
+        HIP_CHECK(hipGetLastError());
+      };
+      stages[prolongate][skip_fused].push_back(std::move(s));
     }
 
     template <int P, int B>
     void
-    launch_brick(const BrickD &b, const T *src, T *dst, bool prolongate, size_t n_launch)
-    {
-      if (n_launch == 0)
-        return;
+    add_persistent_restriction(bool skip_fused, const BrickD &b, size_t n, const std::vector<double> &E)
+    {
       using G = BrickTransferGeo<P, B>;
       BrickTransferArgs<T, P> a;
       const GroupDev<T>      &fg = *fop->groups[b.fine_group];
@@ -826,86 +804,229 @@
       a.interior_base = fg.interior_base.p;
       a.shell_pos     = fg.shell_pos.p;
       a.coarse_idx    = b.coarse_idx.p;
-      a.own_shell     = (!prolongate && b.own_shell_restrict.p) ? b.own_shell_restrict.p : b.own_shell.p;
-      a.n_bricks      = (uint32_t)n_launch;
-      const std::vector<double> E = fec.embedding(1, P);
+      a.own_shell     = b.own_shell_restrict.p ? b.own_shell_restrict.p : b.own_shell.p;
+      a.n_bricks      = (uint32_t)n;
       for (int i = 0; i < (2 * P + 1) * (P + 1); ++i)
         a.E[i] = E[i];
-      a.src            = src;
-      a.dst            = dst;
-      const size_t lds = (size_t)G::LDS * sizeof(T);
-      if (prolongate)
-        launch_lds(ctx, ctx->stream, brick_prolongate_kernel<T, P, B>, (int)n_launch, G::BLOCK, lds, a);
-      else if constexpr (persistent_lattice(G::NF))
-        launch_persistent(ctx, ctx->stream, brick_restrict_persistent_kernel<T, P, B>, (int)n_launch, 3, G::BLOCK, lds, a);
-      else
-        launch_lds(ctx, ctx->stream, brick_restrict_kernel<T, P, B>, (int)n_launch, G::BLOCK, lds, a);
-      HIP_CHECK(hipGetLastError());
-    }
-
-    void
-    run(const T *src, T *dst, bool prolongate, bool skip_fused = false)
-    {
-      for (auto &b : bricks)
-        {
-          const size_t nb = skip_fused ? b->n_unfused : b->n_bricks;
-          if (!dispatch_degree(pc, [&](auto P) {
-                if (!dispatch_brick_size<P(), 2, 4, 8, 16>(b->B, [&](auto B) { launch_brick<P(), B()>(*b, src, dst, prolongate, nb); }))
-                  throw std::runtime_error("brick transfer: unsupported brick size");
-              }))
-            throw std::runtime_error("brick transfer: degree not instantiated");
-        }
-      for (int k = 0; k < 3; ++k)
-        {
-          const GroupD &g = grp[k];
-          if (!g.n_patches)
-            continue;
-          const int key = pc * 100 + g.nf;
-          if (k == 0)
+      StageLaunch s;
+      s.members[MGAMD_TRANSFER_MEMBER_BRICKS17] = (uint32_t)n;
+      s.launch = [this, a, n](const T *src, T *dst) mutable {
+        a.src = src;
+        a.dst = dst;
+        launch_persistent(ctx, ctx->stream, brick_restrict_persistent_kernel<T, P, B>, (int)n, 3, G::BLOCK, (size_t)G::LDS * sizeof(T), a);
+        HIP_CHECK(hipGetLastError());
+      };
+      stages[0][skip_fused].push_back(std::move(s));
+    }
+
+    template <int PC, int NF, bool prolongate>
+    void
+    plan_stage(bool skip_fused)
+    {
+      using A = TransferStageArgs<T, PC, NF>;
+      constexpr int n = PC + 1;
+      const bool    h = pf == pc;
+      A             a{};
+      for (int i = 0; i < n * n; ++i)
+        {
+          a.m.M[i] = a.m.K[i] = 0.0;
+          a.m.I0[i]           = fec.I[0][i];
+          a.m.I1[i]           = fec.I[1][i];
+        }
+      const std::vector<double> &E = grp[h ? 1 : 2].E;
+      if ((int)E.size() != NF * n)
+        throw std::runtime_error("transfer: embedding size mismatch");
+      for (int i = 0; i < NF * n; ++i)
+        a.E[i] = E[i];
+      auto patch_tables = [&](const GroupD &g) {
+        return PatchTables{g.coarse_idx.p, g.coarse_mask.p, (!prolongate && g.fine_idx_restrict.p) ? g.fine_idx_restrict.p : g.fine_idx.p, (uint32_t)g.n_patches};
+      };
+      auto set_ends = [](A &s, uint32_t e) {
+        s.end_patch = s.end_p1 = e;
+        for (uint32_t &b : s.end_brick)
+          b = e;
+      };
+      using GP = TransferGeo<PC, NF>;
+      if (!h)
+        {
+          if (grp[0].n_patches || grp[1].n_patches || !bricks.empty())
+            throw std::runtime_error("transfer: h-patches in a p-transfer");
+          if constexpr (NF != 2 * PC + 1 || 2 * PC <= MAX_KERNEL_DEGREE)
             {
-              if (!dispatch_degree(pc, [&](auto P) { launch<P(), P() + 1, true>(g, src, dst, prolongate); }))
-                throw std::runtime_error("transfer: degree not instantiated");
+              uint32_t members[MGAMD_TRANSFER_N_MEMBERS] = {};
+              a.patch                                    = patch_tables(grp[2]);
+              members[MGAMD_TRANSFER_MEMBER_PATCH]       = (uint32_t)((grp[2].n_patches + GP::SPW - 1) / GP::SPW);
+              set_ends(a, members[MGAMD_TRANSFER_MEMBER_PATCH]);
+              add_stage<PC, NF, TM_PATCH, prolongate>(skip_fused, a, 2 * (size_t)GP::SPW * GP::NF3 * sizeof(T), members);
             }
           else
-            switch (key)
+            throw std::runtime_error("transfer: p-transfer not instantiated");
+          return;
+        }
+      if constexpr (NF == 2 * PC + 1)
+        {
+          if (grp[2].n_patches)
+            throw std::runtime_error("transfer: p-patches in an h-transfer");
+          using GI = TransferGeo<PC, PC + 1>;
+          uint32_t members[MGAMD_TRANSFER_N_MEMBERS] = {}, end = 0;
+          size_t   lds                               = 0;
+          const GroupD &g1 = grp[1];
+          if (g1.n_patches && PC > 1)
+            {
+              a.patch = patch_tables(g1);
+              end += members[MGAMD_TRANSFER_MEMBER_PATCH] = (uint32_t)((g1.n_patches + GP::SPW - 1) / GP::SPW);
+              lds = std::max(lds, 2 * (size_t)GP::SPW * GP::NF3 * sizeof(T));
+            }
+          set_ends(a, end);
+          if constexpr (PC == 1)
+            if (g1.n_patches)
               {
-                case 103:
-                  if (g.p1_uniq_ptr.p)
-                    launch_p1(g, src, dst, prolongate);
-                  else
-                    launch<1, 3, false>(g, src, dst, prolongate);
-                  break;
-                case 104:
-                  launch<1, 4, false>(g, src, dst, prolongate);
-                  break;
-                case 205:
-                  launch<2, 5, false>(g, src, dst, prolongate);
-                  break;
-                case 206:
-                  launch<2, 6, false>(g, src, dst, prolongate);
-                  break;
-                case 307:
-                  launch<3, 7, false>(g, src, dst, prolongate);
-                  break;
-                case 308:
-                  launch<3, 8, false>(g, src, dst, prolongate);
-                  break;
-                case 409:
-                  launch<4, 9, false>(g, src, dst, prolongate);
-                  break;
-                case 511:
-                  launch<5, 11, false>(g, src, dst, prolongate);
-                  break;
-                case 613:
-                  launch<6, 13, false>(g, src, dst, prolongate);
-                  break;
-                case 715:
-                  launch<7, 15, false>(g, src, dst, prolongate);
-                  break;
-                default:
-                  throw std::runtime_error("transfer: (coarse degree, fine patch) combination not instantiated");
+                A         own = a;
+                A        &s   = prolongate ? own : a;
+                uint32_t  own_members[MGAMD_TRANSFER_N_MEMBERS] = {};
+                uint32_t *m   = prolongate ? own_members : members;
+                s.p1 = PatchP1Tables{g1.p1_uniq_ptr.p, g1.p1_uniq_idx.p, g1.p1_loc.p, g1.coarse_mask.p,
+                                     (!prolongate && g1.p1_fine_t_restrict.p) ? g1.p1_fine_t_restrict.p : g1.p1_fine_t.p, (uint32_t)g1.n_patches};
+                m[MGAMD_TRANSFER_MEMBER_PATCH_P1] = (uint32_t)((g1.n_patches + PATCH_P1_BLOCK - 1) / PATCH_P1_BLOCK);
+                const size_t lds_p1               = (size_t)std::max<uint32_t>(g1.p1_max_uniq, 1) * sizeof(T);
+                if constexpr (prolongate)
+                  {
+                    set_ends(own, m[MGAMD_TRANSFER_MEMBER_PATCH_P1]);
+                    own.end_patch = 0;
+                    add_stage<PC, NF, TM_P1, true>(skip_fused, own, lds_p1, own_members);
+                  }
+                else
+                  {
+                    end += m[MGAMD_TRANSFER_MEMBER_PATCH_P1];
+                    set_ends(a, end);
+                    a.end_patch = 0;
+                    lds         = std::max(lds, lds_p1);
+                  }
               }
-        }
+          const size_t fills_gpu = (size_t)2 * 8 * ctx->n_cu;
+          A            big       = a;
+          uint32_t     big_members[MGAMD_TRANSFER_N_MEMBERS] = {}, big_end = 0;
+          size_t       big_lds   = 0;
+          int          n_big     = 0;
+          set_ends(big, 0);
+          big.patch = PatchTables{};
+          big.p1    = PatchP1Tables{};
+          int n_groups = 0;
+          for (auto &bp : bricks)
+            {
+              const BrickD &b  = *bp;
+              const size_t  nb = skip_fused ? b.n_unfused : b.n_bricks;
+              if (nb == 0)
+                continue;
+              if (pc * b.B + 1 > 17 || (b.B != 2 && b.B != 4 && b.B != 8 && b.B != 16))
+                throw std::runtime_error("brick transfer: unsupported brick size");
+              const GroupDev<T> &fg = *fop->groups[b.fine_group];
+              const BrickTables  t{b.slot.p, fg.interior_base.p, fg.shell_pos.p, b.coarse_idx.p,
+                                  (!prolongate && b.own_shell_restrict.p) ? b.own_shell_restrict.p : b.own_shell.p, (uint32_t)nb, (uint32_t)b.B};
+              const size_t       N = (size_t)pc * b.B + 1, lds_b = N * N * N * sizeof(T);
+              if (persistent_lattice((int)N))
+                {
+                  if constexpr (persistent_brick(PC) != 0)
+                    {
+                      if constexpr (prolongate)
+                        {
+                          A        own = a;
+                          uint32_t own_members[MGAMD_TRANSFER_N_MEMBERS] = {};
+                          set_ends(own, 0);
+                          own.patch = own.ident = PatchTables{};
+                          own.brick[0]          = t;
+                          for (uint32_t &e : own.end_brick)
+                            e = (uint32_t)nb;
+                          own_members[MGAMD_TRANSFER_MEMBER_BRICKS17] = (uint32_t)nb;
+                          add_stage<PC, NF, TM_BRICK17, true>(skip_fused, own, lds_b, own_members);
+                        }
+                      else
+                        add_persistent_restriction<PC, persistent_brick(PC)>(skip_fused, b, nb, E);
+                    }
+                  continue;
+                }
+              const bool own_launch = nb >= fills_gpu;
+              A         &s          = own_launch ? big : a;
+              int       &ng         = own_launch ? n_big : n_groups;
+              uint32_t  &e          = own_launch ? big_end : end;
+              if (ng == MAX_STAGE_BRICK_GROUPS)
+                throw std::runtime_error("brick transfer: more brick groups than a stage holds");
+              s.brick[ng] = t;
+              e += (uint32_t)nb;
+              for (int k = ng; k < MAX_STAGE_BRICK_GROUPS; ++k)
+                s.end_brick[k] = e;
+              ++ng;
+              (own_launch ? big_members : members)[MGAMD_TRANSFER_MEMBER_BRICKS] += (uint32_t)nb;
+              (own_launch ? big_lds : lds) = std::max(own_launch ? big_lds : lds, lds_b);
+            }
+          add_stage<PC, NF, TM_BRICKS, prolongate>(skip_fused, big, big_lds, big_members);
+          if (grp[0].n_patches)
+            {
+              a.ident                                 = patch_tables(grp[0]);
+              members[MGAMD_TRANSFER_MEMBER_IDENTITY] = (uint32_t)((grp[0].n_patches + GI::SPW - 1) / GI::SPW);
+              lds                                     = std::max(lds, 2 * (size_t)GI::SPW * GI::NF3 * sizeof(T));
+            }
+          constexpr int MERGED = TM_IDENT | TM_BRICKS | (PC > 1 ? TM_PATCH : (prolongate ? 0 : TM_P1));
+          add_stage<PC, NF, MERGED, prolongate>(skip_fused, a, lds, members);
+        }
+      else
+        throw std::runtime_error("transfer: (coarse degree, fine patch) combination not instantiated");
+    }
+
+    void
+    plan_stages()
+    {
+      const int key = pc * 100 + (pf == pc ? 2 * pc + 1 : pf + 1);
+      auto      go  = [&](auto P, auto N) {
+        for (int skip_fused = 0; skip_fused < 2; ++skip_fused)
+          {
+            plan_stage<P(), N(), false>(skip_fused != 0);
+            plan_stage<P(), N(), true>(skip_fused != 0);
+          }
+      };
+      using std::integral_constant;
+      switch (key)
+        {
+          case 103:
+            go(integral_constant<int, 1>(), integral_constant<int, 3>());
+            break;
+          case 104:
+            go(integral_constant<int, 1>(), integral_constant<int, 4>());
+            break;
+          case 205:
+            go(integral_constant<int, 2>(), integral_constant<int, 5>());
+            break;
+          case 206:
+            go(integral_constant<int, 2>(), integral_constant<int, 6>());
+            break;
+          case 307:
+            go(integral_constant<int, 3>(), integral_constant<int, 7>());
+            break;
+          case 308:
+            go(integral_constant<int, 3>(), integral_constant<int, 8>());
+            break;
+          case 409:
+            go(integral_constant<int, 4>(), integral_constant<int, 9>());
+            break;
+          case 511:
+            go(integral_constant<int, 5>(), integral_constant<int, 11>());
+            break;
+          case 613:
+            go(integral_constant<int, 6>(), integral_constant<int, 13>());
+            break;
+          case 715:
+            go(integral_constant<int, 7>(), integral_constant<int, 15>());
+            break;
+          default:
+            throw std::runtime_error("transfer: (coarse degree, fine patch) combination not instantiated");
+        }
+    }
+
+    void
+    run(const T *src, T *dst, bool prolongate, bool skip_fused = false)
+    {
+      for (StageLaunch &s : stages[prolongate][skip_fused])
+        s.launch(src, dst);
     }
 
     void
diff --git a/dealii_multigrid_amd/csrc/runtime.hpp b/dealii_multigrid_amd/csrc/runtime.hpp
--- a/dealii_multigrid_amd/csrc/runtime.hpp
+++ b/dealii_multigrid_amd/csrc/runtime.hpp
@@ -242,6 +242,8 @@
     restrict_and_add(mgamd_vec &dst_coarse, const mgamd_vec &src_fine) = 0;
     virtual uint64_t
     n_fused_bricks_total() const = 0;
+    virtual unsigned
+    launch_plan(bool prolongate, bool skip_fused, uint32_t *members, unsigned max_launches) const = 0;
   };
 
   struct MultigridBase
diff --git a/include/mgamd.h b/include/mgamd.h
--- a/include/mgamd.h
+++ b/include/mgamd.h
@@ -193,6 +193,14 @@
 int mgamd_transfer2_prolongate_and_add(mgamd_transfer2 *t, mgamd_vec *dst_fine, const mgamd_vec *src_coarse);
 int mgamd_transfer2_restrict_and_add(mgamd_transfer2 *t, mgamd_vec *dst_coarse, const mgamd_vec *src_fine);
 int mgamd_transfer2_n_fused_bricks(const mgamd_transfer2 *t, uint64_t *n);
+#define MGAMD_TRANSFER_N_MEMBERS 5
+#define MGAMD_TRANSFER_MEMBER_IDENTITY 0
+#define MGAMD_TRANSFER_MEMBER_PATCH 1
+#define MGAMD_TRANSFER_MEMBER_PATCH_P1 2
+#define MGAMD_TRANSFER_MEMBER_BRICKS 3
+#define MGAMD_TRANSFER_MEMBER_BRICKS17 4
+int mgamd_transfer2_launch_plan(const mgamd_transfer2 *t, int prolongate, int skip_fused, uint32_t *n_launches, uint32_t *members,
+                                uint32_t max_launches);
 
 int mgamd_mg_create(mgamd_ctx *ctx, unsigned n_levels, mgamd_level_op *const *levels, mgamd_transfer2 *const *transfers,
                     mgamd_cheb *const *smoothers, const char *coarse_solver, mgamd_mg **out);
```

After: 15.77 billion DoF/s, median of 6. 1.01x the previous value.
